# barlettacarmen/CrCNN

Measured on NVIDIA B200. Metric: encrypted MNIST images/sec, higher is better.
Workload: dtype u64

## Files before the change

crcnn_b200/csrc/engine.cu:

```cuda
#include <cuda_runtime.h>
#include <dlfcn.h>
#include <algorithm>
#include <cstdlib>
#include <cstring>
#include <map>
#include <unordered_map>
#include <string>
#include <vector>

#include "../../include/crcnn_b200.h"
#include "kernels.cuh"
#include "params.h"
#include "tc_mac.cuh"
#include "tcn_mac.cuh"
#include "relin32.cuh"
#include "reenc.cuh"

using namespace crcnn;

namespace {

enum KernelClass {
    KC_NTT_FWD = 0, KC_NTT_INV, KC_MAC, KC_PLAIN_EXPAND, KC_POOL, KC_BN, KC_PLAIN_OP,
    KC_BEHZ_LIFT, KC_SQ_TENSOR, KC_BEHZ_FLOOR, KC_RELIN, KC_PROBE, KC_TC_SPLIT, KC_TC_MAC, KC_TCN_SPLIT, KC_TCN_MAC, KC_RELIN32, KC_REENC, KC_COUNT
};
const char *kClassNames[KC_COUNT] = {"ntt_forward", "ntt_inverse", "weighted_sum_mac", "plain_expand_ntt", "pool_sum",
                                     "batch_norm", "plain_op", "behz_lift", "square_tensor", "behz_floor_sk",
                                     "relinearize", "imad_probe", "tc_plane_split", "weighted_sum_tc_i8", "tcn_plane_split",
                                     "weighted_sum_tcn_i8", "relinearize_u32", "reencrypt"};

thread_local std::string g_create_error;

}

struct crcnn_tensor {
    long count;
    int size;
    int ntt;
    uint64_t *d;
};

static long next_plain_serial() { static long s = 0; return ++s; }

struct crcnn_plain {
    long serial = next_plain_serial();
    long count;
    bool sparse_shape = false;
    std::vector<uint32_t> off, idx;
    std::vector<uint64_t> val;
    uint32_t *d_off = nullptr, *d_idx = nullptr;
    uint64_t *d_val = nullptr;
    uint64_t *ntt_mul = nullptr;
    uint64_t *ntt_mul_sh = nullptr;
    uint64_t *ntt_add = nullptr;
    uint64_t *coef_add = nullptr;
    int tap_state = 0;
    int tc_state = 0;
    int8_t *tc_A = nullptr;
    int tc_R = 0, tc_Kpad = 0;
    uint8_t *tcn_W = nullptr;
    int tcn_R = 0;
    uint64_t *fused_C = nullptr, *fused_Csh = nullptr, *fused_D = nullptr;
    long fused_scale = 0, fused_mean = 0;
    int add_mult = 1;
    bool dense_only = false;
    crcnn_plain *folded_w = nullptr, *folded_b = nullptr;
    long folded_key[9] = {0, 0, 0, 0, 0, 0, 0, 0, 0};
};

struct crcnn_evk {
    uint64_t *d = nullptr;
    long key_off[MAXK];
    int digits[MAXK];
    int dbc;
    bool has_r32 = false;
    Relin32 r32;
};

struct crcnn_keys {
    uint64_t *sk = nullptr;
    uint64_t *pk = nullptr;
    ReencConsts c;
};

struct crcnn_ctx {
    int device = 0;
    cudaStream_t stream = nullptr;
    HostParams hp;
    DeviceParams *dP = nullptr;
    std::vector<void *> owned;
    int n = 0, logn = 0, K = 0, S = 0;
    int chunk_terms = 1 << 30;
    size_t weight_cache_bytes = 24ull << 30;
    int sm_count = 148;
    int tc_mode = 1;
    int tc_min_fanin = 256;
    int tc_min_outputs = 32;
    int tap_mode = 1;
    int relin_mode = 1;
    int tcn_mode = 1;
    int sq_lean = 1;
    int tcn_fold = 1;
    size_t tc_scratch_bytes = 12ull << 30;
    std::string err;
    std::map<std::vector<int>, int *> index_cache;
    std::unordered_map<void *, size_t> big_size;
    std::multimap<size_t, void *> big_free;
    size_t big_cached = 0, big_cache_cap = 64ull << 30;
    long long st_big_malloc = 0, st_big_hit = 0, st_big_bypass = 0, st_flush = 0, st_small_malloc = 0;
    uint64_t *stage = nullptr;
    size_t stage_bytes = 0;
    bool prof_on = false;
    long launches[KC_COUNT] = {0};
    double ms[KC_COUNT] = {0};
    double work_bytes[KC_COUNT] = {0};
    double work_ops[KC_COUNT] = {0};
    struct Pending { int cls; cudaEvent_t a, b; };
    std::vector<Pending> pending;
    std::vector<cudaEvent_t> event_pool;
};

namespace {

int fail(crcnn_ctx *ctx, int code, const std::string &msg) {
    if (ctx) ctx->err = msg; else g_create_error = msg;
    return code;
}

#define CU(call)                                                                                       \
    do {                                                                                               \
        cudaError_t e__ = (call);                                                                      \
        if (e__ != cudaSuccess) {                                                                      \
            int code__ = (e__ == cudaErrorMemoryAllocation) ? CRCNN_ERR_OUT_OF_MEMORY : CRCNN_ERR_CUDA; \
            return fail(ctx, code__, std::string(#call) + ": " + cudaGetErrorString(e__));            \
        }                                                                                              \
    } while (0)

#define REQUIRE(cond, msg) \
    do { if (!(cond)) return fail(ctx, CRCNN_ERR_INVALID_ARGUMENT, msg); } while (0)

struct ProfScope {
    crcnn_ctx *c; int cls; cudaEvent_t a = nullptr, b = nullptr;
    ProfScope(crcnn_ctx *ctx, int k, double bytes = 0, double ops = 0) : c(ctx), cls(k) {
        c->launches[cls]++;
        c->work_bytes[cls] += bytes;
        c->work_ops[cls] += ops;
        if (!c->prof_on) return;
        auto get = [&]() { cudaEvent_t e; if (!c->event_pool.empty()) { e = c->event_pool.back(); c->event_pool.pop_back(); } else cudaEventCreate(&e); return e; };
        a = get(); b = get();
        cudaEventRecord(a, c->stream);
    }
    ~ProfScope() {
        if (!a) return;
        cudaEventRecord(b, c->stream);
        c->pending.push_back({cls, a, b});
    }
};

void prof_collect(crcnn_ctx *c) {
    for (auto &p : c->pending) {
        cudaEventSynchronize(p.b);
        float t = 0;
        cudaEventElapsedTime(&t, p.a, p.b);
        c->ms[p.cls] += t;
        c->event_pool.push_back(p.a);
        c->event_pool.push_back(p.b);
    }
    c->pending.clear();
}

inline size_t poly_words(const crcnn_ctx *c) { return (size_t)c->K * c->n; }
inline double lp_bytes(const crcnn_ctx *c, double polys) { return polys * c->n * 8.0; }
inline double lp_bfly(const crcnn_ctx *c, double polys) { return polys * (c->n / 2) * c->logn; }

constexpr size_t kBigBlock = 32ull << 20;
void big_cache_flush(crcnn_ctx *ctx) {
    for (auto &kv : ctx->big_free) { ctx->big_size.erase(kv.second); cudaFreeAsync(kv.second, ctx->stream); }
    ctx->big_free.clear();
    ctx->big_cached = 0;
}
int dev_alloc(crcnn_ctx *ctx, size_t bytes, void **out) {
    *out = nullptr;
    if (bytes == 0) return CRCNN_OK;
    if (bytes >= kBigBlock) {
        auto it = ctx->big_free.find(bytes);
        if (it != ctx->big_free.end()) {
            *out = it->second;
            ctx->big_cached -= bytes;
            ctx->big_free.erase(it);
            ctx->st_big_hit++;
            return CRCNN_OK;
        }
        ctx->st_big_malloc++;
    } else {
        ctx->st_small_malloc++;
    }
    cudaError_t e = cudaMallocAsync(out, bytes, ctx->stream);
    if (e == cudaErrorMemoryAllocation && !ctx->big_free.empty()) {
        cudaGetLastError();
        ctx->st_flush++;
        big_cache_flush(ctx);
        e = cudaMallocAsync(out, bytes, ctx->stream);
    }
    CU(e);
    if (bytes >= kBigBlock) ctx->big_size[*out] = bytes;
    return CRCNN_OK;
}
void dev_free(crcnn_ctx *ctx, void *p) {
    if (!p) return;
    auto it = ctx->big_size.find(p);
    if (it != ctx->big_size.end()) {
        if (ctx->big_cached + it->second <= ctx->big_cache_cap) {
            ctx->big_free.insert({it->second, p});
            ctx->big_cached += it->second;
            return;
        }
        ctx->big_size.erase(it);
        ctx->st_big_bypass++;
    }
    cudaFreeAsync(p, ctx->stream);
}

int new_tensor(crcnn_ctx *ctx, long count, int size, int ntt, crcnn_tensor **out) {
    auto *t = new crcnn_tensor{count, size, ntt, nullptr};
    int rc = dev_alloc(ctx, (size_t)count * size * poly_words(ctx) * 8, (void **)&t->d);
    if (rc) { delete t; return rc; }
    *out = t;
    return CRCNN_OK;
}

int ntt_inplace(crcnn_ctx *ctx, uint64_t *d, long npolys, int slot_base, int slot_count, bool inverse) {
    ProfScope ps(ctx, inverse ? KC_NTT_INV : KC_NTT_FWD, 2 * lp_bytes(ctx, npolys), lp_bfly(ctx, npolys));
    CU(launch_ntt(ctx->dP, ctx->logn, d, npolys, slot_base, slot_count, inverse, ctx->stream));
    return CRCNN_OK;
}

int ensure_domain(crcnn_ctx *ctx, crcnn_tensor *t, int want_ntt) {
    if (t->ntt == want_ntt) return CRCNN_OK;
    int rc = ntt_inplace(ctx, t->d, t->count * t->size * ctx->K, 0, ctx->K, !want_ntt);
    if (rc) return rc;
    t->ntt = want_ntt;
    return CRCNN_OK;
}

enum PlainForm { PF_NTT_MUL, PF_NTT_ADD, PF_COEF_ADD };

int expand_range(crcnn_ctx *ctx, crcnn_plain *p, long first, long count, PlainForm f, uint64_t *dst) {
    ProfScope ps(ctx, KC_PLAIN_EXPAND, lp_bytes(ctx, (double)count * ctx->K), f != PF_COEF_ADD ? lp_bfly(ctx, (double)count * ctx->K) : 0);
    CU(launch_plain_expand(ctx->dP, ctx->logn, ctx->K, p->d_off, p->d_idx, p->d_val, first, count,
                           (f == PF_NTT_MUL ? 0 : 1) | (p->sparse_shape ? 2 : 0), f != PF_COEF_ADD, dst, ctx->stream));
    return CRCNN_OK;
}

int ensure_form(crcnn_ctx *ctx, crcnn_plain *p, PlainForm f) {
    uint64_t **slot = f == PF_NTT_MUL ? &p->ntt_mul : (f == PF_NTT_ADD ? &p->ntt_add : &p->coef_add);
    if (*slot) return CRCNN_OK;
    if (p->dense_only) return fail(ctx, CRCNN_ERR_UNSUPPORTED, "this derived plaintext pack has no such form");
    int rc = dev_alloc(ctx, (size_t)p->count * poly_words(ctx) * 8, (void **)slot);
    if (rc) return rc;
    rc = expand_range(ctx, p, 0, p->count, f, *slot);
    if (!rc && f != PF_NTT_MUL && p->add_mult != 1)
        CU(launch_scale_small(ctx->dP, *slot, (long)((size_t)p->count * poly_words(ctx)), p->add_mult, ctx->stream));
    return rc;
}

int make_plain(crcnn_ctx *ctx, std::vector<uint32_t> &&off, std::vector<uint32_t> &&idx, std::vector<uint64_t> &&val,
               crcnn_plain **out) {
    auto *p = new crcnn_plain();
    p->count = (long)off.size() - 1;
    p->off = std::move(off); p->idx = std::move(idx); p->val = std::move(val);
    p->sparse_shape = true;
    for (uint32_t ix : p->idx)
        if (ix >= 64 && ix < (uint32_t)(ctx->n - 32)) { p->sparse_shape = false; break; }
    int rc = dev_alloc(ctx, p->off.size() * 4, (void **)&p->d_off);
    if (!rc) rc = dev_alloc(ctx, std::max<size_t>(p->idx.size(), 1) * 4, (void **)&p->d_idx);
    if (!rc) rc = dev_alloc(ctx, std::max<size_t>(p->val.size(), 1) * 8, (void **)&p->d_val);
    if (rc) { delete p; return rc; }
    CU(cudaMemcpyAsync(p->d_off, p->off.data(), p->off.size() * 4, cudaMemcpyHostToDevice, ctx->stream));
    if (!p->idx.empty()) {
        CU(cudaMemcpyAsync(p->d_idx, p->idx.data(), p->idx.size() * 4, cudaMemcpyHostToDevice, ctx->stream));
        CU(cudaMemcpyAsync(p->d_val, p->val.data(), p->val.size() * 8, cudaMemcpyHostToDevice, ctx->stream));
    }
    CU(cudaStreamSynchronize(ctx->stream));
    *out = p;
    return CRCNN_OK;
}

int ensure_shoup(crcnn_ctx *ctx, crcnn_plain *p) {
    int rc = ensure_form(ctx, p, PF_NTT_MUL);
    if (rc || p->ntt_mul_sh) return rc;
    const size_t words = (size_t)p->count * poly_words(ctx);
    rc = dev_alloc(ctx, words * 8, (void **)&p->ntt_mul_sh);
    if (rc) return rc;
    CU(launch_shoup_companion(ctx->dP, p->ntt_mul, (long)words, p->ntt_mul_sh, ctx->stream));
    return CRCNN_OK;
}

int ensure_pool_bn_consts(crcnn_ctx *ctx, crcnn_plain *scale, crcnn_plain *mean, crcnn_plain *invstd) {
    int rc = scale ? ensure_form(ctx, scale, PF_NTT_MUL) : CRCNN_OK;
    if (!rc) rc = ensure_form(ctx, mean, PF_NTT_ADD);
    if (!rc) rc = ensure_form(ctx, invstd, PF_NTT_MUL);
    if (rc) return rc;
    const long scale_id = scale ? scale->serial : -1;
    if (invstd->fused_C && invstd->fused_scale == scale_id && invstd->fused_mean == mean->serial) return CRCNN_OK;
    const size_t words = (size_t)invstd->count * poly_words(ctx);
    dev_free(ctx, invstd->fused_C); dev_free(ctx, invstd->fused_Csh); dev_free(ctx, invstd->fused_D);
    invstd->fused_C = invstd->fused_Csh = invstd->fused_D = nullptr;
    rc = dev_alloc(ctx, words * 8, (void **)&invstd->fused_C);
    if (!rc) rc = dev_alloc(ctx, words * 8, (void **)&invstd->fused_Csh);
    if (!rc) rc = dev_alloc(ctx, words * 8, (void **)&invstd->fused_D);
    if (rc) return rc;
    CU(launch_pool_bn_consts(ctx->dP, scale ? scale->ntt_mul : nullptr, invstd->ntt_mul, mean->ntt_add, (long)words, invstd->fused_C, invstd->fused_D, ctx->stream));
    CU(launch_shoup_companion(ctx->dP, invstd->fused_C, (long)words, invstd->fused_Csh, ctx->stream));
    invstd->fused_scale = scale_id; invstd->fused_mean = mean->serial;
    return CRCNN_OK;
}

int get_index_table(crcnn_ctx *ctx, const std::vector<int> &key, const std::vector<int> &table, const int **out) {
    auto it = ctx->index_cache.find(key);
    if (it != ctx->index_cache.end()) { *out = it->second; return CRCNN_OK; }
    int *d = nullptr;
    CU(cudaMalloc((void **)&d, std::max<size_t>(table.size(), 1) * sizeof(int)));
    CU(cudaMemcpyAsync(d, table.data(), table.size() * sizeof(int), cudaMemcpyHostToDevice, ctx->stream));
    CU(cudaStreamSynchronize(ctx->stream));
    ctx->index_cache[key] = d;
    *out = d;
    return CRCNN_OK;
}

bool tap_eligible(crcnn_ctx *ctx, crcnn_plain *p) {
    if (p->tap_state == 0) {
        p->tap_state = (p->sparse_shape && tcn_planes_for(ctx->hp.d) == 7 && ctx->n % 1024 == 0) ? 1 : -1;
        const uint64_t t = ctx->hp.d.t;
        for (size_t e = 0; e < p->val.size() && p->tap_state == 1; e++)
            if (p->val[e] != 1 && p->val[e] != t - 1) p->tap_state = -1;
        for (long i = 0; i < p->count && p->tap_state == 1; i++)
            if (p->off[i + 1] - p->off[i] > 96) p->tap_state = -1;
    }
    return p->tap_state == 1;
}

bool sum_fits_64(const crcnn_ctx *ctx, long R) {
    uint64_t maxq = 0;
    for (int j = 0; j < ctx->K; j++) maxq = std::max(maxq, ctx->hp.d.tab[j].mod.q);
    return R > 0 && (uint64_t)R <= UINT64_MAX / maxq;
}

void boundaries(int xd, int yd, int xs, int ys, int xf, int yf, int *xl, int *yl) {
    *xl = (xf > xs) ? xd - xf + 1 : xd - xs + 1;
    *yl = (yf > ys) ? yd - yf + 1 : yd - ys + 1;
}

int ensure_tc_form(crcnn_ctx *ctx, crcnn_plain *w, int R) {
    if (w->tc_state < 0) return CRCNN_OK;
    if (w->tc_state == 1 && w->tc_R == R) return CRCNN_OK;
    const uint32_t n = (uint32_t)ctx->n;
    const uint64_t t = ctx->hp.d.t;
    for (size_t e = 0; e < w->idx.size(); e++)
        if (w->idx[e] < n - TC_TAPS || (w->val[e] != 1 && w->val[e] != t - 1)) { w->tc_state = -1; return CRCNN_OK; }
    if (w->count % R) { w->tc_state = -1; return CRCNN_OK; }
    const long Mall = w->count / R;
    const int Kpad = ((R + 31) / 32 + 3) / 4 * TC_BK;
    const size_t rows = (size_t)Mall * TC_TAPS + TC_BM;
    std::vector<int8_t> A(rows * Kpad, 0);
    for (long wi = 0; wi < w->count; wi++) {
        const long m = wi / R, r = wi % R;
        for (uint32_t e = w->off[wi]; e < w->off[wi + 1]; e++) {
            const int tap = (int)(n - w->idx[e]);
            A[((size_t)m * TC_TAPS + tap - 1) * Kpad + r] = w->val[e] == 1 ? (int8_t)-1 : (int8_t)1;
        }
    }
    if (w->tc_A) { dev_free(ctx, w->tc_A); w->tc_A = nullptr; }
    int rc = dev_alloc(ctx, A.size(), (void **)&w->tc_A);
    if (rc) return rc;
    CU(cudaMemcpyAsync(w->tc_A, A.data(), A.size(), cudaMemcpyHostToDevice, ctx->stream));
    CU(cudaStreamSynchronize(ctx->stream));
    w->tc_state = 1; w->tc_R = R; w->tc_Kpad = Kpad;
    return CRCNN_OK;
}

int run_weighted_sum_tc(crcnn_ctx *ctx, crcnn_tensor *in, crcnn_plain *w, crcnn_plain *b, const int *d_index, int R,
                        int Npos, int Pimg, int m_first, int M, crcnn_tensor *out) {
    int rc = ensure_domain(ctx, in, 0);
    if (!rc) rc = ensure_form(ctx, b, PF_COEF_ADD);
    if (rc) return rc;
    const size_t pw = poly_words(ctx);
    TcMacArgs a{};
    a.A = w->tc_A + (size_t)m_first * TC_TAPS * w->tc_Kpad;
    a.x = in->d; a.bias = b->coef_add + (size_t)m_first * pw; a.out = out->d;
    a.M = M; a.Mpad = (M * TC_TAPS + TC_BM - 1) / TC_BM * TC_BM; a.R = R; a.Kpad = w->tc_Kpad;
    a.planes = tc_planes_for(ctx->hp.d);
    a.Pimg = Pimg; a.Mtotal = M; a.m0 = 0; a.n = ctx->n; a.K = ctx->K;
    a.npos = 1;
    const size_t per_pos = tc_b_bytes(a);
    long chunk = (long)std::max<size_t>(1, ctx->tc_scratch_bytes / per_pos);
    chunk = std::min<long>(std::min<long>(chunk, Npos), 65535 / (2 * ctx->K));
    uint8_t *scratch = nullptr;
    rc = dev_alloc(ctx, (size_t)chunk * per_pos, (void **)&scratch);
    if (rc) return rc;
    a.B = scratch;
    for (long p0 = 0; p0 < Npos && !rc; p0 += chunk) {
        a.npos = (int)std::min<long>(chunk, Npos - p0);
        a.p0 = (int)p0;
        a.in_index = d_index + p0 * R;
        cudaError_t e;
        const double bbytes = (double)a.npos * per_pos;
        { ProfScope ps(ctx, KC_TC_SPLIT, lp_bytes(ctx, (double)a.npos * R * 2 * ctx->K) + bbytes, 0); e = launch_tc_split(ctx->dP, a, ctx->stream); }
        if (e == cudaSuccess) {
            ProfScope ps(ctx, KC_TC_MAC, bbytes + lp_bytes(ctx, (double)a.npos * M * 2 * ctx->K),
                         (double)a.npos * 2 * ctx->K * ctx->n * a.planes * (double)M * TC_TAPS * R);
            e = launch_tc_mac(ctx->dP, a, ctx->sm_count, ctx->stream);
        }
        if (e != cudaSuccess) rc = fail(ctx, CRCNN_ERR_CUDA, std::string("tensor-core weighted sum: ") + cudaGetErrorString(e));
    }
    dev_free(ctx, scratch);
    if (!rc) out->ntt = 0;
    return rc;
}

int ensure_tcn_weights(crcnn_ctx *ctx, crcnn_plain *w, int R) {
    if (w->tcn_W && w->tcn_R == R) return CRCNN_OK;
    int rc = ensure_form(ctx, w, PF_NTT_MUL);
    if (rc) return rc;
    if (w->tcn_W) { dev_free(ctx, w->tcn_W); w->tcn_W = nullptr; }
    const int Mall = (int)(w->count / R), Kpad = tcn_kpad(R);
    rc = dev_alloc(ctx, tcn_w_bytes(7, Mall, Kpad, ctx->K, ctx->n), (void **)&w->tcn_W);
    if (rc) return rc;
    TcnSplitArgs s{};
    s.src = w->ntt_mul; s.index = nullptr; s.dst = w->tcn_W; s.item_polys = 1;
    s.R = R; s.Kpad = Kpad; s.planes = 7; s.ncols = Mall; s.slot0 = 0; s.nslots = ctx->K * ctx->n; s.n = ctx->n; s.K = ctx->K;
    {
        ProfScope ps(ctx, KC_TCN_SPLIT, lp_bytes(ctx, (double)w->count * ctx->K) + (double)tcn_w_bytes(7, Mall, Kpad, ctx->K, ctx->n), 0);
        CU(launch_tcn_split(s, ctx->stream));
    }
    dev_free(ctx, w->ntt_mul); w->ntt_mul = nullptr;
    if (w->ntt_mul_sh) { dev_free(ctx, w->ntt_mul_sh); w->ntt_mul_sh = nullptr; }
    w->tcn_R = R;
    return CRCNN_OK;
}

int run_weighted_sum_tcn(crcnn_ctx *ctx, crcnn_tensor *in, crcnn_plain *w, crcnn_plain *b, const int *d_index, int R,
                         int Npos, int Pimg, int m_first, int M, crcnn_tensor *out) {
    int rc = ensure_domain(ctx, in, 1);
    if (!rc) rc = ensure_form(ctx, b, PF_NTT_ADD);
    if (!rc) rc = ensure_tcn_weights(ctx, w, R);
    if (rc) return rc;
    const size_t pw = poly_words(ctx);
    const int Kpad = tcn_kpad(R), ncols = 2 * Npos, total = ctx->K * ctx->n;
    const size_t per_slot = tcn_x_bytes_per_slot(7, ncols, Kpad);
    long chunk = (long)(ctx->tc_scratch_bytes / per_slot) / 32 * 32;
    chunk = std::max<long>(32, std::min<long>(chunk, total));
    uint8_t *scratch = nullptr;
    rc = dev_alloc(ctx, (size_t)chunk * per_slot, (void **)&scratch);
    if (rc) return rc;
    TcnSplitArgs s{};
    s.src = in->d; s.index = d_index; s.dst = scratch; s.item_polys = 2;
    s.R = R; s.Kpad = Kpad; s.planes = 7; s.ncols = ncols; s.n = ctx->n; s.K = ctx->K;
    TcnMacArgs a{};
    a.W = w->tcn_W; a.X = scratch; a.bias = b->ntt_add + (size_t)m_first * pw; a.out = out->d;
    a.Mall = (int)(w->count / R); a.m_first = m_first; a.M = M;
    a.R = R; a.Kpad = Kpad; a.planes = 7; a.ncols = ncols;
    a.Pimg = Pimg; a.Mtotal = M; a.m0 = 0; a.n = ctx->n; a.K = ctx->K;
    a.variant = ctx->tcn_mode >= 2 ? ctx->tcn_mode - 1 : 0;
    a.use_fold = ctx->tcn_fold;
    for (int j = 0; j < ctx->K; j++) a.fold[j] = tcn_fold_make(ctx->hp.d.tab[j].mod.q);
    for (long s0 = 0; s0 < total && !rc; s0 += chunk) {
        const int ns = (int)std::min<long>(chunk, total - s0);
        s.slot0 = a.slot0 = (int)s0; s.nslots = a.nslots = ns;
        const double xbytes = (double)ns * per_slot;
        cudaError_t e;
        { ProfScope ps(ctx, KC_TCN_SPLIT, (double)ncols * R * ns * 8.0 + xbytes, 0); e = launch_tcn_split(s, ctx->stream); }
        if (e == cudaSuccess) {
            ProfScope ps(ctx, KC_TCN_MAC, xbytes + (double)ns * 7 * M * Kpad + (double)ncols * M * ns * 8.0, (double)ns * ncols * M * R * 49.0);
            e = launch_tcn_mac(ctx->dP, a, ctx->sm_count, ctx->stream);
        }
        if (e != cudaSuccess) rc = fail(ctx, CRCNN_ERR_CUDA, std::string("limb-split tensor-core weighted sum: ") + cudaGetErrorString(e));
    }
    dev_free(ctx, scratch);
    if (!rc) out->ntt = 1;
    return rc;
}

int run_weighted_sum(crcnn_ctx *ctx, crcnn_tensor *in, crcnn_plain *w, crcnn_plain *b, const int *d_index, int R,
                     int Npos, int Pimg, int Mall, int m_first, int M, crcnn_tensor *out) {
    if (ctx->tc_mode && R >= ctx->tc_min_fanin && (ctx->tc_mode == 2 || Mall >= ctx->tc_min_outputs) && w->sparse_shape && tc_mac_available() == cudaSuccess) {
        int rc = ensure_tc_form(ctx, w, R);
        if (rc) return rc;
        if (w->tc_state == 1) return run_weighted_sum_tc(ctx, in, w, b, d_index, R, Npos, Pimg, m_first, M, out);
    }
    if (ctx->tcn_mode && tcn_planes_for(ctx->hp.d) == 7 && R <= TCN_MAX_R && w->count % R == 0 && tc_mac_available() == cudaSuccess &&
        (w->tcn_W || tcn_w_bytes(7, (int)(w->count / R), tcn_kpad(R), ctx->K, ctx->n) <= ctx->weight_cache_bytes))
        return run_weighted_sum_tcn(ctx, in, w, b, d_index, R, Npos, Pimg, m_first, M, out);
    int rc = ensure_domain(ctx, in, 1);
    if (rc) return rc;
    rc = ensure_form(ctx, b, PF_NTT_ADD);
    if (rc) return rc;
    MacArgs a{};
    a.x = in->d; a.in_index = d_index; a.out = out->d;
    a.R = R; a.Npos = Npos; a.Pimg = Pimg; a.Mtotal = M; a.K = ctx->K; a.n = ctx->n;
    a.chunk_terms = ctx->chunk_terms;
    const size_t pw = poly_words(ctx);
    const size_t all_bytes = (size_t)w->count * pw * 8;
    if (w->ntt_mul || all_bytes <= ctx->weight_cache_bytes) {
        rc = ensure_form(ctx, w, PF_NTT_MUL);
        if (rc) return rc;
        a.w = w->ntt_mul + (size_t)m_first * R * pw;
        a.bias = b->ntt_add + (size_t)m_first * pw;
        a.M = M; a.m0 = 0;
        ProfScope ps(ctx, KC_MAC, lp_bytes(ctx, ((double)in->count + (double)M * Npos) * 2 * ctx->K + (double)M * R * ctx->K),
                     (double)M * Npos * R * 2 * ctx->K * ctx->n);
        CU(launch_mac(ctx->dP, a, ctx->stream));
        return CRCNN_OK;
    }
    long rows = (long)std::max<size_t>(1, ctx->weight_cache_bytes / ((size_t)R * pw * 8));
    rows = std::min<long>(rows, M);
    uint64_t *scratch = nullptr;
    rc = dev_alloc(ctx, (size_t)rows * R * pw * 8, (void **)&scratch);
    if (rc) return rc;
    for (long m0 = 0; m0 < M; m0 += rows) {
        long cur = std::min<long>(rows, M - m0);
        rc = expand_range(ctx, w, (long)(m_first + m0) * R, cur * R, PF_NTT_MUL, scratch);
        if (rc) break;
        a.w = scratch; a.bias = b->ntt_add + (size_t)(m_first + m0) * pw;
        a.M = (int)cur; a.m0 = (int)m0;
        ProfScope ps(ctx, KC_MAC, lp_bytes(ctx, ((double)in->count + (double)cur * Npos) * 2 * ctx->K + (double)cur * R * ctx->K),
                     (double)cur * Npos * R * 2 * ctx->K * ctx->n);
        cudaError_t e = launch_mac(ctx->dP, a, ctx->stream);
        if (e != cudaSuccess) { rc = fail(ctx, CRCNN_ERR_CUDA, cudaGetErrorString(e)); break; }
    }
    dev_free(ctx, scratch);
    return rc;
}

int upload_rows(crcnn_ctx *ctx, const uint64_t *host, size_t rows, uint64_t *dst, cudaStream_t s) {
    const size_t n = ctx->n;
    if (rows * n * 8 < (8u << 20)) {
        CU(cudaMemcpy2DAsync(dst, n * 8, host, (n + 1) * 8, n * 8, rows, cudaMemcpyHostToDevice, s));
        return CRCNN_OK;
    }
    uint64_t *stage = nullptr;
    CU(cudaMallocAsync((void **)&stage, rows * (n + 1) * 8, s));
    cudaError_t e = cudaMemcpyAsync(stage, host, rows * (n + 1) * 8, cudaMemcpyHostToDevice, s);
    if (e == cudaSuccess) e = launch_strip_pad(stage, dst, (long)rows, (int)n, s);
    cudaFreeAsync(stage, s);
    if (e != cudaSuccess) return fail(ctx, CRCNN_ERR_CUDA, std::string("upload: ") + cudaGetErrorString(e));
    return CRCNN_OK;
}

}

extern "C" {

const char *crcnn_last_error(const crcnn_ctx *ctx) { return ctx ? ctx->err.c_str() : g_create_error.c_str(); }

int crcnn_ctx_create(int n, int K, const uint64_t *q, uint64_t t, int device, crcnn_ctx **out) {
    crcnn_ctx *ctx = nullptr;
    if (!out || !q) return fail(nullptr, CRCNN_ERR_INVALID_ARGUMENT, "null argument");
    *out = nullptr;
    int ndev = 0;
    if (cudaGetDeviceCount(&ndev) != cudaSuccess || ndev == 0)
        return fail(nullptr, CRCNN_ERR_NO_DEVICE, "no CUDA device: crcnn_b200 has no CPU fallback");
    if (device < 0 || device >= ndev) return fail(nullptr, CRCNN_ERR_INVALID_ARGUMENT, "bad device ordinal");
    HostParams hp;
    try {
        hp = derive_params(n, K, q, t);
    } catch (const std::exception &e) {
        return fail(nullptr, CRCNN_ERR_INVALID_ARGUMENT, e.what());
    }
    CU(cudaSetDevice(device));
    auto *c = new crcnn_ctx();
    c->device = device; c->n = n; c->K = K; c->S = hp.d.S; c->logn = hp.d.logn;
    int maxbits = 0;
    for (int i = 0; i < K; i++) { int b = 0; for (uint64_t v = q[i]; v; v >>= 1) b++; maxbits = std::max(maxbits, b); }
    int spare = 128 - 2 * maxbits;
    c->chunk_terms = spare >= 30 ? (1 << 30) : (1 << spare);
    cudaDeviceGetAttribute(&c->sm_count, cudaDevAttrMultiProcessorCount, device);
    if (const char *e = getenv("CRCNN_TC")) c->tc_mode = atoi(e);
    if (const char *e = getenv("CRCNN_TCN")) c->tcn_mode = atoi(e);
    if (const char *e = getenv("CRCNN_TAP")) c->tap_mode = atoi(e);
    if (const char *e = getenv("CRCNN_TCN_FOLD")) c->tcn_fold = atoi(e);
    if (const char *e = getenv("CRCNN_SQ_LEAN")) c->sq_lean = atoi(e);
    cudaMemPool_t pool;
    if (cudaDeviceGetDefaultMemPool(&pool, device) == cudaSuccess) {
        uint64_t thr = UINT64_MAX;
        cudaMemPoolSetAttribute(pool, cudaMemPoolAttrReleaseThreshold, &thr);
    }
    {
        size_t fr = 0, tot = 0;
        if (cudaMemGetInfo(&fr, &tot) == cudaSuccess && tot) c->big_cache_cap = tot / 4 * 3;
    }
    int slots = K + hp.d.S;
    auto up = [&](const std::vector<uint64_t> &v, const uint64_t **dst) -> cudaError_t {
        void *d = nullptr;
        cudaError_t e = cudaMalloc(&d, v.size() * 8);
        if (e != cudaSuccess) return e;
        c->owned.push_back(d);
        *dst = (const uint64_t *)d;
        return cudaMemcpy(d, v.data(), v.size() * 8, cudaMemcpyHostToDevice);
    };
    cudaError_t e = cudaSuccess;
    for (int s = 0; s < slots && e == cudaSuccess; s++) {
        std::vector<uint64_t> fw(2 * (size_t)n), bw(2 * (size_t)n);
        for (int i = 0; i < n; i++) {
            fw[2 * i] = hp.w[s][i]; fw[2 * i + 1] = hp.wp[s][i];
            bw[2 * i] = hp.iwf[s][i]; bw[2 * i + 1] = hp.iwfp[s][i];
        }
        e = up(fw, &hp.d.tab[s].w);
        if (e == cudaSuccess) e = up(bw, &hp.d.tab[s].iw);
        const int NG = n >> 4;
        std::vector<uint64_t> fl(2 * (size_t)16 * NG, 0), bl(2 * (size_t)16 * NG, 0);
        for (int G = 0; G < NG; G++)
            for (int st = 0; st < 4; st++) {
                for (int lb = 0; lb < (1 << st); lb++) {
                    const size_t at = 2 * ((size_t)((1 << st) - 1 + lb) * NG + G), from = 2 * ((((size_t)NG + G) << st) + lb);
                    fl[at] = fw[from]; fl[at + 1] = fw[from + 1];
                }
                for (int lb = 0; lb < (1 << (3 - st)); lb++) {
                    const size_t at = 2 * ((size_t)(16 - (16 >> st) + lb) * NG + G);
                    const size_t from = 2 * ((size_t)((n >> 1) >> st) + ((size_t)G << (3 - st)) + lb);
                    bl[at] = bw[from]; bl[at + 1] = bw[from + 1];
                }
            }
        if (e == cudaSuccess) e = up(fl, &hp.d.tab[s].wl);
        if (e == cudaSuccess) e = up(bl, &hp.d.tab[s].iwl);
        hp.d.tab[s].tf = nullptr;
        if (e == cudaSuccess && s < K) e = up(hp.tf[s], &hp.d.tab[s].tf);
    }
    if (e == cudaSuccess) e = cudaMalloc((void **)&c->dP, sizeof(DeviceParams));
    if (e == cudaSuccess) e = cudaMemcpy(c->dP, &hp.d, sizeof(DeviceParams), cudaMemcpyHostToDevice);
    if (e != cudaSuccess) {
        std::string m = cudaGetErrorString(e);
        for (void *p : c->owned) cudaFree(p);
        if (c->dP) cudaFree(c->dP);
        delete c;
        return fail(nullptr, CRCNN_ERR_CUDA, "context setup: " + m);
    }
    c->hp = std::move(hp);
    *out = c;
    return CRCNN_OK;
}

int crcnn_ctx_destroy(crcnn_ctx *ctx) {
    if (!ctx) return CRCNN_OK;
    cudaSetDevice(ctx->device);
    big_cache_flush(ctx);
    cudaStreamSynchronize(ctx->stream);
    prof_collect(ctx);
    for (auto e : ctx->event_pool) cudaEventDestroy(e);
    for (auto &kv : ctx->index_cache) cudaFree(kv.second);
    if (ctx->stage) cudaFree(ctx->stage);
    for (void *p : ctx->owned) cudaFree(p);
    cudaFree(ctx->dP);
    delete ctx;
    return CRCNN_OK;
}

int crcnn_ctx_set_stream(crcnn_ctx *ctx, void *cuda_stream) {
    if (!ctx) return CRCNN_ERR_INVALID_ARGUMENT;
    CU(cudaStreamSynchronize(ctx->stream));
    ctx->stream = (cudaStream_t)cuda_stream;
    return CRCNN_OK;
}

int crcnn_ctx_sync(crcnn_ctx *ctx) {
    if (!ctx) return CRCNN_ERR_INVALID_ARGUMENT;
    CU(cudaStreamSynchronize(ctx->stream));
    prof_collect(ctx);
    return CRCNN_OK;
}

int crcnn_ctx_alloc_stats(crcnn_ctx *ctx, long long out[6]) {
    if (!ctx || !out) return CRCNN_ERR_INVALID_ARGUMENT;
    out[0] = ctx->st_big_malloc; out[1] = ctx->st_big_hit; out[2] = ctx->st_big_bypass; out[3] = ctx->st_flush;
    out[4] = ctx->st_small_malloc; out[5] = (long long)ctx->big_cached;
    return CRCNN_OK;
}

int crcnn_ctx_set_weight_cache_bytes(crcnn_ctx *ctx, size_t bytes) {
    if (!ctx) return CRCNN_ERR_INVALID_ARGUMENT;
    ctx->weight_cache_bytes = bytes;
    return CRCNN_OK;
}

int crcnn_ctx_set_tensor_core_mode(crcnn_ctx *ctx, int mode, int min_fanin, size_t scratch_bytes) {
    if (!ctx) return CRCNN_ERR_INVALID_ARGUMENT;
    REQUIRE(mode >= 0 && mode <= 2, "tensor-core mode must be 0, 1 or 2");
    ctx->tc_mode = mode;
    if (min_fanin > 0) ctx->tc_min_fanin = min_fanin;
    if (scratch_bytes > 0) ctx->tc_scratch_bytes = scratch_bytes;
    return CRCNN_OK;
}

int crcnn_ctx_set_limb_split_mode(crcnn_ctx *ctx, int mode) {
    if (!ctx) return CRCNN_ERR_INVALID_ARGUMENT;
    REQUIRE(mode >= 0 && mode <= 3, "limb-split mode must be 0 (off), 1 (on), 2 (row-major kernel) or 3 (column-major kernel)");
    ctx->tcn_mode = mode;
    return CRCNN_OK;
}

int crcnn_ctx_set_limb_split_reduction(crcnn_ctx *ctx, int mode) {
    if (!ctx) return CRCNN_ERR_INVALID_ARGUMENT;
    REQUIRE(mode == 0 || mode == 1, "limb-split reduction must be 0 (128-bit recombination + Barrett) or 1 (folded through 2^k - delta)");
    ctx->tcn_fold = mode;
    return CRCNN_OK;
}

int crcnn_ctx_set_relin_mode(crcnn_ctx *ctx, int mode) {
    if (!ctx) return CRCNN_ERR_INVALID_ARGUMENT;
    REQUIRE(mode == 0 || mode == 1, "relinearize mode must be 0 (64-bit transforms) or 1 (word-size auxiliary primes)");
    ctx->relin_mode = mode;
    return CRCNN_OK;
}

int crcnn_ctx_ntt_table(const crcnn_ctx *ctx_c, int slot, int which, uint64_t *out) {
    crcnn_ctx *ctx = const_cast<crcnn_ctx *>(ctx_c);
    if (!ctx) return CRCNN_ERR_INVALID_ARGUMENT;
    REQUIRE(out && slot >= 0 && slot < ctx->K + ctx->S && which >= 0 && which < 4, "bad table selector");
    const auto &v = which == 0 ? ctx->hp.w[slot] : which == 1 ? ctx->hp.wp[slot] : which == 2 ? ctx->hp.iw[slot] : ctx->hp.iwp[slot];
    memcpy(out, v.data(), v.size() * 8);
    return CRCNN_OK;
}

int crcnn_ctx_bsk_count(const crcnn_ctx *ctx) { return ctx ? ctx->S : CRCNN_ERR_INVALID_ARGUMENT; }

int crcnn_tensor_upload_ex(crcnn_ctx *ctx, const uint64_t *host, long count, int size, int ntt_form, crcnn_tensor **out) {
    if (!ctx) return CRCNN_ERR_INVALID_ARGUMENT;
    REQUIRE(host && out && count >= 0 && size >= 2 && size <= 3, "bad tensor upload arguments");
    CU(cudaSetDevice(ctx->device));
    crcnn_tensor *t = nullptr;
    int rc = new_tensor(ctx, count, size, ntt_form ? 1 : 0, &t);
    if (rc) return rc;
    const size_t n = ctx->n, rows = (size_t)count * size * ctx->K;
    if (rows) {
        int rc2 = upload_rows(ctx, host, rows, t->d, ctx->stream);
        if (rc2) { crcnn_tensor_free(ctx, t); return rc2; }
    }
    (void)n;
    *out = t;
    return CRCNN_OK;
}
int crcnn_tensor_upload_on(crcnn_ctx *ctx, const uint64_t *host, long count, int size, int ntt_form, void *copy_stream,
                           crcnn_tensor **out) {
    if (!ctx) return CRCNN_ERR_INVALID_ARGUMENT;
    REQUIRE(host && out && count >= 0 && size >= 2 && size <= 3, "bad tensor upload arguments");
    CU(cudaSetDevice(ctx->device));
    cudaStream_t cs = (cudaStream_t)copy_stream;
    auto *t = new crcnn_tensor{count, size, ntt_form ? 1 : 0, nullptr};
    const size_t n = ctx->n, rows = (size_t)count * size * ctx->K;
    if (rows) {
        cudaError_t e = cudaMallocAsync((void **)&t->d, rows * n * 8, cs);
        if (e != cudaSuccess) { delete t; return fail(ctx, e == cudaErrorMemoryAllocation ? CRCNN_ERR_OUT_OF_MEMORY : CRCNN_ERR_CUDA, cudaGetErrorString(e)); }
        int rc2 = upload_rows(ctx, host, rows, t->d, cs);
        if (rc2) { cudaFreeAsync(t->d, cs); delete t; return rc2; }
    }
    *out = t;
    return CRCNN_OK;
}

int crcnn_tensor_upload_into(crcnn_ctx *ctx, const uint64_t *host, crcnn_tensor *t, int ntt_form, void *copy_stream) {
    if (!ctx) return CRCNN_ERR_INVALID_ARGUMENT;
    REQUIRE(host && t, "null argument");
    CU(cudaSetDevice(ctx->device));
    cudaStream_t cs = copy_stream ? (cudaStream_t)copy_stream : ctx->stream;
    const size_t n = ctx->n, rows = (size_t)t->count * t->size * ctx->K;
    const size_t need = rows * (n + 1) * 8;
    if (need > ctx->stage_bytes) {
        if (ctx->stage) { CU(cudaStreamSynchronize(cs)); CU(cudaFree(ctx->stage)); ctx->stage = nullptr; ctx->stage_bytes = 0; }
        CU(cudaMalloc((void **)&ctx->stage, need));
        ctx->stage_bytes = need;
    }
    if (rows) {
        CU(cudaMemcpyAsync(ctx->stage, host, need, cudaMemcpyHostToDevice, cs));
        CU(launch_strip_pad(ctx->stage, t->d, (long)rows, (int)n, cs));
    }
    t->ntt = ntt_form ? 1 : 0;
    return CRCNN_OK;
}

int crcnn_ctx_wait_stream(crcnn_ctx *ctx, void *other_stream) {
    if (!ctx) return CRCNN_ERR_INVALID_ARGUMENT;
    cudaEvent_t ev;
    CU(cudaEventCreateWithFlags(&ev, cudaEventDisableTiming));
    CU(cudaEventRecord(ev, (cudaStream_t)other_stream));
    CU(cudaStreamWaitEvent(ctx->stream, ev, 0));
    CU(cudaEventDestroy(ev));
    return CRCNN_OK;
}

int crcnn_tensor_upload(crcnn_ctx *ctx, const uint64_t *host, long count, int size, crcnn_tensor **out) {
    return crcnn_tensor_upload_ex(ctx, host, count, size, 0, out);
}

int crcnn_tensor_download_ex(crcnn_ctx *ctx, crcnn_tensor *t, int want_ntt, uint64_t *host) {
    if (!ctx) return CRCNN_ERR_INVALID_ARGUMENT;
    REQUIRE(t && host, "null argument");
    CU(cudaSetDevice(ctx->device));
    const size_t n = ctx->n, rows = (size_t)t->count * t->size * ctx->K;
    const uint64_t *src = t->d;
    uint64_t *tmp = nullptr;
    if ((t->ntt != 0) != (want_ntt != 0)) {
        int rc = dev_alloc(ctx, rows * n * 8, (void **)&tmp);
        if (rc) return rc;
        CU(cudaMemcpyAsync(tmp, t->d, rows * n * 8, cudaMemcpyDeviceToDevice, ctx->stream));
        rc = ntt_inplace(ctx, tmp, (long)rows, 0, ctx->K, want_ntt == 0);
        if (rc) return rc;
        src = tmp;
    }
    if (rows) CU(cudaMemcpy2DAsync(host, (n + 1) * 8, src, n * 8, n * 8, rows, cudaMemcpyDeviceToHost, ctx->stream));
    CU(cudaStreamSynchronize(ctx->stream));
    dev_free(ctx, tmp);
    for (size_t r = 0; r < rows; r++) host[r * (n + 1) + n] = 0;
    prof_collect(ctx);
    return CRCNN_OK;
}
int crcnn_tensor_download(crcnn_ctx *ctx, crcnn_tensor *t, uint64_t *host) { return crcnn_tensor_download_ex(ctx, t, 0, host); }

int crcnn_tensor_free(crcnn_ctx *ctx, crcnn_tensor *t) {
    if (!ctx) return CRCNN_ERR_INVALID_ARGUMENT;
    if (!t) return CRCNN_OK;
    dev_free(ctx, t->d);
    delete t;
    return CRCNN_OK;
}
long crcnn_tensor_count(const crcnn_tensor *t) { return t ? t->count : -1; }
int crcnn_tensor_ct_size(const crcnn_tensor *t) { return t ? t->size : -1; }

int crcnn_tensor_slice(crcnn_ctx *ctx, crcnn_tensor *t, long first, long count, crcnn_tensor **out) {
    if (!ctx) return CRCNN_ERR_INVALID_ARGUMENT;
    REQUIRE(t && out && first >= 0 && count >= 0 && first + count <= t->count, "slice out of range");
    crcnn_tensor *s = nullptr;
    int rc = new_tensor(ctx, count, t->size, t->ntt, &s);
    if (rc) return rc;
    size_t ctw = (size_t)t->size * poly_words(ctx);
    if (count) CU(cudaMemcpyAsync(s->d, t->d + first * ctw, count * ctw * 8, cudaMemcpyDeviceToDevice, ctx->stream));
    *out = s;
    return CRCNN_OK;
}

int crcnn_tensor_device_ptr(crcnn_tensor *t, void **dev_ptr, int *ntt_form) {
    if (!t || !dev_ptr) return CRCNN_ERR_INVALID_ARGUMENT;
    *dev_ptr = t->d;
    if (ntt_form) *ntt_form = t->ntt;
    return CRCNN_OK;
}

int crcnn_tensor_wrap_alloc(crcnn_ctx *ctx, long count, int size, int ntt_form, crcnn_tensor **out) {
    if (!ctx) return CRCNN_ERR_INVALID_ARGUMENT;
    REQUIRE(out && count >= 0 && size >= 2 && size <= 3, "bad tensor shape");
    return new_tensor(ctx, count, size, ntt_form ? 1 : 0, out);
}

int crcnn_plain_upload(crcnn_ctx *ctx, const uint64_t *host, long count, int coeff_count, long stride, crcnn_plain **out) {
    if (!ctx) return CRCNN_ERR_INVALID_ARGUMENT;
    REQUIRE(host && out && count >= 0 && coeff_count >= 0 && stride >= coeff_count, "bad plaintext upload arguments");
    REQUIRE(coeff_count <= ctx->n + 1, "plain is not valid for encryption parameters");
    std::vector<uint32_t> off(count + 1, 0), idx;
    std::vector<uint64_t> val;
    for (long i = 0; i < count; i++) {
        const uint64_t *p = host + i * stride;
        for (int c = 0; c < coeff_count; c++)
            if (p[c]) {
                REQUIRE(c < ctx->n, "plain is not valid for encryption parameters");
                REQUIRE(p[c] < ctx->hp.d.t, "plaintext coefficient not below the plain modulus");
                idx.push_back((uint32_t)c); val.push_back(p[c]);
            }
        off[i + 1] = (uint32_t)idx.size();
    }
    return make_plain(ctx, std::move(off), std::move(idx), std::move(val), out);
}

int crcnn_plain_upload_sparse(crcnn_ctx *ctx, const uint32_t *idx, const uint64_t *val, const uint32_t *offsets, long count,
                              crcnn_plain **out) {
    if (!ctx) return CRCNN_ERR_INVALID_ARGUMENT;
    REQUIRE(offsets && out && count >= 0, "bad sparse plaintext arguments");
    std::vector<uint32_t> off(offsets, offsets + count + 1);
    size_t nnz = off[count];
    REQUIRE(nnz == 0 || (idx && val), "null sparse arrays");
    std::vector<uint32_t> vi(idx, idx + nnz);
    std::vector<uint64_t> vv(val, val + nnz);
    for (size_t e = 0; e < nnz; e++) {
        REQUIRE(vi[e] < (uint32_t)ctx->n, "plain is not valid for encryption parameters");
        REQUIRE(vv[e] < ctx->hp.d.t, "plaintext coefficient not below the plain modulus");
    }
    return make_plain(ctx, std::move(off), std::move(vi), std::move(vv), out);
}

int crcnn_plain_encode(crcnn_ctx *ctx, const float *values, long count, crcnn_plain **out) {
    if (!ctx) return CRCNN_ERR_INVALID_ARGUMENT;
    REQUIRE(values && out && count >= 0, "bad encode arguments");
    std::vector<uint32_t> off(count + 1, 0), idx;
    std::vector<uint64_t> val;
    idx.reserve(count * 24); val.reserve(count * 24);
    for (long i = 0; i < count; i++) {
        encode_fractional_sparse((double)values[i], ctx->n, ctx->hp.d.t, idx, val);
        off[i + 1] = (uint32_t)idx.size();
    }
    return make_plain(ctx, std::move(off), std::move(idx), std::move(val), out);
}

int crcnn_plain_encode_f64(crcnn_ctx *ctx, const double *values, long count, crcnn_plain **out) {
    if (!ctx) return CRCNN_ERR_INVALID_ARGUMENT;
    REQUIRE(values && out && count >= 0, "bad encode arguments");
    std::vector<uint32_t> off(count + 1, 0), idx;
    std::vector<uint64_t> val;
    for (long i = 0; i < count; i++) {
        encode_fractional_sparse(values[i], ctx->n, ctx->hp.d.t, idx, val);
        off[i + 1] = (uint32_t)idx.size();
    }
    return make_plain(ctx, std::move(off), std::move(idx), std::move(val), out);
}

int crcnn_plain_get(crcnn_ctx *ctx, const crcnn_plain *p, long index, uint64_t *out_words) {
    if (!ctx) return CRCNN_ERR_INVALID_ARGUMENT;
    REQUIRE(p && out_words && index >= 0 && index < p->count, "plaintext index out of range");
    REQUIRE(!p->dense_only, "derived plaintext pack: no host form");
    memset(out_words, 0, (size_t)(ctx->n + 1) * 8);
    for (uint32_t e = p->off[index]; e < p->off[index + 1]; e++) out_words[p->idx[e]] = p->val[e];
    return CRCNN_OK;
}

int crcnn_plain_get_ntt(crcnn_ctx *ctx, crcnn_plain *p, long index, uint64_t *out_words) {
    if (!ctx) return CRCNN_ERR_INVALID_ARGUMENT;
    REQUIRE(p && out_words && index >= 0 && index < p->count, "plaintext index out of range");
    REQUIRE(!p->dense_only, "derived plaintext pack: no host form");
    uint64_t *tmp = nullptr;
    int rc = dev_alloc(ctx, poly_words(ctx) * 8, (void **)&tmp);
    if (rc) return rc;
    rc = expand_range(ctx, p, index, 1, PF_NTT_MUL, tmp);
    if (rc) return rc;
    const size_t n = ctx->n;
    CU(cudaMemcpy2DAsync(out_words, (n + 1) * 8, tmp, n * 8, n * 8, ctx->K, cudaMemcpyDeviceToHost, ctx->stream));
    CU(cudaStreamSynchronize(ctx->stream));
    dev_free(ctx, tmp);
    for (int j = 0; j < ctx->K; j++) out_words[j * (n + 1) + n] = 0;
    return CRCNN_OK;
}

int crcnn_plain_free(crcnn_ctx *ctx, crcnn_plain *p) {
    if (!ctx) return CRCNN_ERR_INVALID_ARGUMENT;
    if (!p) return CRCNN_OK;
    dev_free(ctx, p->d_off); dev_free(ctx, p->d_idx); dev_free(ctx, p->d_val);
    dev_free(ctx, p->ntt_mul); dev_free(ctx, p->ntt_mul_sh); dev_free(ctx, p->ntt_add); dev_free(ctx, p->coef_add); dev_free(ctx, p->tc_A); dev_free(ctx, p->tcn_W);
    dev_free(ctx, p->fused_C); dev_free(ctx, p->fused_Csh); dev_free(ctx, p->fused_D);
    if (p->folded_w) crcnn_plain_free(ctx, p->folded_w);
    if (p->folded_b) crcnn_plain_free(ctx, p->folded_b);
    delete p;
    return CRCNN_OK;
}
long crcnn_plain_count(const crcnn_plain *p) { return p ? p->count : -1; }

int crcnn_evk_upload(crcnn_ctx *ctx, const uint64_t *host, int dbc, const int *sizes, crcnn_evk **out) {
    if (!ctx) return CRCNN_ERR_INVALID_ARGUMENT;
    REQUIRE(host && sizes && out && dbc >= 1 && dbc <= 60, "bad evaluation key arguments");
    CU(cudaSetDevice(ctx->device));
    auto *k = new crcnn_evk();
    k->dbc = dbc;
    long polys = 0;
    const size_t pw = poly_words(ctx);
    for (int i = 0; i < MAXK; i++) { k->key_off[i] = 0; k->digits[i] = 0; }
    for (int i = 0; i < ctx->K; i++) {
        if (sizes[i] < 2 || (sizes[i] & 1)) { delete k; return fail(ctx, CRCNN_ERR_INVALID_ARGUMENT, "evaluation key sizes must be even and >= 2"); }
        k->key_off[i] = polys * (long)pw;
        k->digits[i] = sizes[i] / 2;
        polys += sizes[i];
    }
    int rc = dev_alloc(ctx, (size_t)polys * pw * 8, (void **)&k->d);
    if (rc) { delete k; return rc; }
    const size_t n = ctx->n, rows = (size_t)polys * ctx->K;
    CU(cudaMemcpy2DAsync(k->d, n * 8, host, (n + 1) * 8, n * 8, rows, cudaMemcpyHostToDevice, ctx->stream));
    CU(launch_canonicalize(ctx->dP, k->d, (long)(rows * n), ctx->stream));
    {
        uint64_t q[MAXK];
        for (int i = 0; i < ctx->K; i++) q[i] = ctx->hp.d.tab[i].mod.q;
        if (relin32_applicable(ctx->n, ctx->K, q, k->digits, dbc, k->r32.c)) {
            cudaError_t e = relin32_build(ctx->dP, ctx->logn, ctx->K, q, k->d, k->key_off, polys, k->r32, ctx->stream);
            if (e != cudaSuccess) { relin32_free(k->r32); dev_free(ctx, k->d); delete k; return fail(ctx, CRCNN_ERR_CUDA, cudaGetErrorString(e)); }
            k->has_r32 = true;
        }
    }
    *out = k;
    return CRCNN_OK;
}
int crcnn_evk_free(crcnn_ctx *ctx, crcnn_evk *k) {
    if (!ctx) return CRCNN_ERR_INVALID_ARGUMENT;
    if (!k) return CRCNN_OK;
    CU(cudaSetDevice(ctx->device));
    CU(cudaStreamSynchronize(ctx->stream));
    relin32_free(k->r32);
    dev_free(ctx, k->d);
    delete k;
    return CRCNN_OK;
}

int crcnn_conv_forward_shard(crcnn_ctx *ctx, crcnn_tensor *in, crcnn_plain *w, crcnn_plain *b, int batch, int xd, int yd,
                             int zd, int xs, int ys, int xf, int yf, int nf, int k0, int kc, crcnn_tensor **out) {
    if (!ctx) return CRCNN_ERR_INVALID_ARGUMENT;
    REQUIRE(in && w && b && out, "null argument");
    REQUIRE(batch > 0 && xd > 0 && yd > 0 && zd > 0 && xs > 0 && ys > 0 && xf > 0 && yf > 0 && nf > 0 && xf <= xd && yf <= yd,
            "bad convolution geometry");
    REQUIRE(k0 >= 0 && kc >= 0 && k0 + kc <= nf, "bad output-channel shard");
    REQUIRE(in->size == 2 && in->count == (long)batch * zd * xd * yd, "input tensor does not match the layer geometry");
    const int R = zd * xf * yf;
    REQUIRE(w->count == (long)nf * R && b->count == nf, "kernel/bias count does not match the layer geometry");
    CU(cudaSetDevice(ctx->device));
    const int xo = (xd - xf) / xs + 1, yo = (yd - yf) / ys + 1;
    int xl, yl;
    boundaries(xd, yd, xs, ys, xf, yf, &xl, &yl);
    if ((xl + xs - 1) / xs != xo || (yl + ys - 1) / ys != yo)
        return fail(ctx, CRCNN_ERR_UNSUPPORTED, "stride larger than the filter leaves outputs the reference never computes");
    const int P = xo * yo, Npos = batch * P, nin = zd * xd * yd;
    std::vector<int> key = {1, batch, xd, yd, zd, xs, ys, xf, yf};
    const int *d_index = nullptr;
    if (ctx->index_cache.find(key) == ctx->index_cache.end()) {
        std::vector<int> table((size_t)Npos * R);
        for (int bi = 0; bi < batch; bi++)
            for (int i = 0; i < xo; i++)
                for (int j = 0; j < yo; j++) {
                    int *row = &table[((size_t)bi * P + i * yo + j) * R];
                    int r = 0;
                    for (int z = 0; z < zd; z++)
                        for (int kx = 0; kx < xf; kx++)
                            for (int ky = 0; ky < yf; ky++) row[r++] = bi * nin + (z * xd + i * xs + kx) * yd + j * ys + ky;
                }
        int rc = get_index_table(ctx, key, table, &d_index);
        if (rc) return rc;
    } else {
        d_index = ctx->index_cache[key];
    }
    crcnn_tensor *o = nullptr;
    int rc = new_tensor(ctx, (long)batch * kc * P, 2, 1, &o);
    if (rc) return rc;
    rc = run_weighted_sum(ctx, in, w, b, d_index, R, Npos, P, nf, k0, kc, o);
    if (rc) { crcnn_tensor_free(ctx, o); return rc; }
    *out = o;
    return CRCNN_OK;
}

int crcnn_conv_forward(crcnn_ctx *ctx, crcnn_tensor *in, crcnn_plain *w, crcnn_plain *b, int batch, int xd, int yd, int zd,
                       int xs, int ys, int xf, int yf, int nf, crcnn_tensor **out) {
    return crcnn_conv_forward_shard(ctx, in, w, b, batch, xd, yd, zd, xs, ys, xf, yf, nf, 0, nf, out);
}

int crcnn_fc_forward_shard(crcnn_ctx *ctx, crcnn_tensor *in, crcnn_plain *w, crcnn_plain *b, int batch, int in_dim,
                           int out_dim, int o0, int oc, crcnn_tensor **out) {
    if (!ctx) return CRCNN_ERR_INVALID_ARGUMENT;
    REQUIRE(in && w && b && out, "null argument");
    REQUIRE(batch > 0 && in_dim > 0 && out_dim > 0, "bad fully-connected geometry");
    REQUIRE(o0 >= 0 && oc >= 0 && o0 + oc <= out_dim, "bad output-row shard");
    REQUIRE(in->size == 2 && in->count == (long)batch * in_dim, "input tensor does not match the layer geometry");
    REQUIRE(w->count == (long)out_dim * in_dim && b->count == out_dim, "weight/bias count does not match the layer geometry");
    CU(cudaSetDevice(ctx->device));
    std::vector<int> key = {2, batch, in_dim};
    const int *d_index = nullptr;
    if (ctx->index_cache.find(key) == ctx->index_cache.end()) {
        std::vector<int> table((size_t)batch * in_dim);
        for (size_t i = 0; i < table.size(); i++) table[i] = (int)i;
        int rc = get_index_table(ctx, key, table, &d_index);
        if (rc) return rc;
    } else {
        d_index = ctx->index_cache[key];
    }
    crcnn_tensor *o = nullptr;
    int rc = new_tensor(ctx, (long)batch * oc, 2, 1, &o);
    if (rc) return rc;
    rc = run_weighted_sum(ctx, in, w, b, d_index, in_dim, batch, 1, out_dim, o0, oc, o);
    if (rc) { crcnn_tensor_free(ctx, o); return rc; }
    *out = o;
    return CRCNN_OK;
}

int crcnn_fc_forward(crcnn_ctx *ctx, crcnn_tensor *in, crcnn_plain *w, crcnn_plain *b, int batch, int in_dim, int out_dim,
                     crcnn_tensor **out) {
    return crcnn_fc_forward_shard(ctx, in, w, b, batch, in_dim, out_dim, 0, out_dim, out);
}

static int compose_fc(crcnn_ctx *ctx, crcnn_plain *w1, crcnn_plain *b1, crcnn_plain *w2, crcnn_plain *b2, int in_dim, int mid_dim, int out_dim,
                      const uint64_t *C = nullptr, const uint64_t *D = nullptr, int per_channel = 1) {
    const size_t pw = poly_words(ctx);
    const int saved_tc = ctx->tc_mode;
    const bool saved_prof = ctx->prof_on;
    ctx->tc_mode = 0;
    ctx->prof_on = false;
    crcnn_plain *zero = nullptr, *W = nullptr, *B = nullptr;
    crcnn_tensor *T = nullptr, *O = nullptr;
    uint64_t *dense = nullptr;
    int rc = CRCNN_OK;
    auto done = [&](int code) {
        if (T) crcnn_tensor_free(ctx, T);
        if (O) crcnn_tensor_free(ctx, O);
        if (zero) crcnn_plain_free(ctx, zero);
        dev_free(ctx, dense);
        if (code) { if (W) crcnn_plain_free(ctx, W); if (B) crcnn_plain_free(ctx, B); }
        ctx->tc_mode = saved_tc; ctx->prof_on = saved_prof;
        return code;
    };
    rc = make_plain(ctx, std::vector<uint32_t>((size_t)out_dim + 1, 0), {}, {}, &zero);
    if (rc) return done(rc);
    rc = dev_alloc(ctx, (size_t)out_dim * in_dim * pw * 8, (void **)&dense);
    if (rc) return done(rc);
    const int pairs_all = (in_dim + 1) / 2;
    int Bc = (int)std::max<size_t>(1, std::min<size_t>((size_t)pairs_all, (8ull << 30) / ((size_t)mid_dim * 2 * pw * 8)));
    if (const char *e = getenv("CRCNN_FC_COMPOSE_PAIRS")) Bc = std::max(1, std::min(Bc, atoi(e)));
    std::vector<int> table((size_t)Bc * mid_dim);
    for (int bi = 0; bi < Bc; bi++)
        for (int o = 0; o < mid_dim; o++) table[(size_t)bi * mid_dim + o] = o * Bc + bi;
    const int *d_index = nullptr;
    rc = get_index_table(ctx, {5, Bc, mid_dim}, table, &d_index);
    if (rc) return done(rc);
    rc = new_tensor(ctx, (long)mid_dim * Bc, 2, 1, &T);
    if (!rc) rc = new_tensor(ctx, (long)Bc * out_dim, 2, 1, &O);
    if (rc) return done(rc);
    CU(cudaMemsetAsync(T->d, 0, (size_t)T->count * 2 * pw * 8, ctx->stream));
    for (int r0 = 0; r0 < in_dim && !rc; r0 += 2 * Bc) {
        const int cols = std::min(2 * Bc, in_dim - r0);
        for (int o = 0; o < mid_dim && !rc; o++)
            rc = expand_range(ctx, w1, (long)o * in_dim + r0, cols, PF_NTT_MUL, T->d + (size_t)o * Bc * 2 * pw);
        if (rc) break;
        rc = run_weighted_sum(ctx, T, w2, zero, d_index, mid_dim, Bc, 1, out_dim, 0, out_dim, O);
        if (rc) break;
        for (int bi = 0; 2 * bi < cols; bi++) {
            const int polys = std::min(2, cols - 2 * bi);
            cudaError_t e = cudaMemcpy2DAsync(dense + ((size_t)r0 + 2 * bi) * pw, (size_t)in_dim * pw * 8, O->d + (size_t)bi * out_dim * 2 * pw,
                                              2 * pw * 8, (size_t)polys * pw * 8, out_dim, cudaMemcpyDeviceToDevice, ctx->stream);
            if (e != cudaSuccess) { rc = fail(ctx, CRCNN_ERR_CUDA, cudaGetErrorString(e)); break; }
        }
    }
    if (rc) return done(rc);
    W = new crcnn_plain();
    W->count = (long)out_dim * in_dim; W->dense_only = true; W->sparse_shape = false; W->tc_state = -1; W->tap_state = -1;
    W->ntt_mul = dense; dense = nullptr;
    rc = ensure_form(ctx, b1, PF_NTT_ADD);
    if (rc) return done(rc);
    crcnn_tensor_free(ctx, T); T = nullptr;
    crcnn_tensor_free(ctx, O); O = nullptr;
    rc = new_tensor(ctx, mid_dim, 2, 1, &T);
    if (!rc) rc = new_tensor(ctx, out_dim, 2, 1, &O);
    if (rc) return done(rc);
    CU(cudaMemsetAsync(T->d, 0, (size_t)mid_dim * 2 * pw * 8, ctx->stream));
    CU(cudaMemcpy2DAsync(T->d, 2 * pw * 8, b1->ntt_add, pw * 8, pw * 8, mid_dim, cudaMemcpyDeviceToDevice, ctx->stream));
    std::vector<int> ident(mid_dim);
    for (int o = 0; o < mid_dim; o++) ident[o] = o;
    rc = get_index_table(ctx, {2, 1, mid_dim}, ident, &d_index);
    if (!rc) rc = run_weighted_sum(ctx, T, w2, b2, d_index, mid_dim, 1, 1, out_dim, 0, out_dim, O);
    if (rc) return done(rc);
    B = new crcnn_plain();
    B->count = out_dim; B->dense_only = true; B->sparse_shape = false; B->tc_state = -1; B->tap_state = -1;
    rc = dev_alloc(ctx, (size_t)out_dim * pw * 8, (void **)&B->ntt_add);
    if (rc) return done(rc);
    CU(cudaMemcpy2DAsync(B->ntt_add, pw * 8, O->d, 2 * pw * 8, pw * 8, out_dim, cudaMemcpyDeviceToDevice, ctx->stream));
    if (C) CU(launch_fold_fc_input_affine(ctx->dP, W->ntt_mul, out_dim, in_dim, (long)pw, per_channel, C, D, B->ntt_add, ctx->stream));
    rc = ensure_tcn_weights(ctx, W, in_dim);
    if (rc) return done(rc);
    w1->folded_w = W; w1->folded_b = B;
    return done(CRCNN_OK);
}

int crcnn_fc_fc_forward(crcnn_ctx *ctx, crcnn_tensor *in, crcnn_plain *w1, crcnn_plain *b1, crcnn_plain *w2, crcnn_plain *b2, int batch,
                        int in_dim, int mid_dim, int out_dim, crcnn_tensor **out) {
    if (!ctx) return CRCNN_ERR_INVALID_ARGUMENT;
    REQUIRE(in && w1 && b1 && w2 && b2 && out, "null argument");
    REQUIRE(batch > 0 && in_dim > 0 && mid_dim > 0 && out_dim > 0, "bad fully-connected geometry");
    REQUIRE(in->size == 2 && in->count == (long)batch * in_dim, "input tensor does not match the layer geometry");
    REQUIRE(w1->count == (long)mid_dim * in_dim && b1->count == mid_dim && w2->count == (long)out_dim * mid_dim && b2->count == out_dim,
            "weight/bias count does not match the layer geometry");
    CU(cudaSetDevice(ctx->device));
    const bool composed = (double)out_dim * in_dim < (double)mid_dim * (in_dim + out_dim) && !w1->dense_only && !w2->dense_only &&
                          ctx->tcn_mode && tcn_planes_for(ctx->hp.d) == 7 && in_dim <= TCN_MAX_R && mid_dim <= TCN_MAX_R &&
                          tc_mac_available() == cudaSuccess && tcn_w_bytes(7, out_dim, tcn_kpad(in_dim), ctx->K, ctx->n) <= ctx->weight_cache_bytes &&
                          !getenv("CRCNN_NO_FC_COMPOSE");
    if (!composed) {
        crcnn_tensor *mid = nullptr;
        int rc = crcnn_fc_forward(ctx, in, w1, b1, batch, in_dim, mid_dim, &mid);
        if (rc) return rc;
        rc = crcnn_fc_forward(ctx, mid, w2, b2, batch, mid_dim, out_dim, out);
        crcnn_tensor_free(ctx, mid);
        return rc;
    }
    const long key[9] = {b1->serial, w2->serial, b2->serial, (long)mid_dim, (long)out_dim, 0, 0, 0, 0};
    if (!w1->folded_w || memcmp(key, w1->folded_key, sizeof(key)) != 0) {
        if (w1->folded_w) { crcnn_plain_free(ctx, w1->folded_w); w1->folded_w = nullptr; }
        if (w1->folded_b) { crcnn_plain_free(ctx, w1->folded_b); w1->folded_b = nullptr; }
        int rc = compose_fc(ctx, w1, b1, w2, b2, in_dim, mid_dim, out_dim);
        if (rc) return rc;
        memcpy(w1->folded_key, key, sizeof(key));
    }
    return crcnn_fc_forward(ctx, in, w1->folded_w, w1->folded_b, batch, in_dim, out_dim, out);
}

int crcnn_pool_bn_fc_fc_forward(crcnn_ctx *ctx, crcnn_tensor *in, int batch, int xd, int yd, int zd, int pxs, int pys, int pxf, int pyf,
                                crcnn_plain *scale, crcnn_plain *mean, crcnn_plain *invstd, crcnn_plain *w1, crcnn_plain *b1,
                                crcnn_plain *w2, crcnn_plain *b2, int mid_dim, int out_dim, crcnn_tensor **out) {
    if (!ctx) return CRCNN_ERR_INVALID_ARGUMENT;
    REQUIRE(in && mean && invstd && w1 && b1 && w2 && b2 && out, "null argument");
    REQUIRE(batch > 0 && xd > 0 && yd > 0 && zd > 0 && pxs > 0 && pys > 0 && pxf > 0 && pyf > 0 && pxf <= xd && pyf <= yd, "bad pooling geometry");
    REQUIRE(mid_dim > 0 && out_dim > 0, "bad fully-connected geometry");
    const int pxo = (xd - pxf) / pxs + 1, pyo = (yd - pyf) / pys + 1, Rp = pxf * pyf;
    const int in_dim = zd * pxo * pyo;
    REQUIRE(in->size == 2 && in->count == (long)batch * zd * xd * yd, "input tensor does not match the layer geometry");
    REQUIRE((!scale || scale->count >= 1) && mean->count == zd && invstd->count == zd, "mean/var count does not match the channel count");
    REQUIRE(w1->count == (long)mid_dim * in_dim && b1->count == mid_dim && w2->count == (long)out_dim * mid_dim && b2->count == out_dim,
            "weight/bias count does not match the layer geometry");
    CU(cudaSetDevice(ctx->device));
    const bool composed = pxs <= pxf && pys <= pyf && sum_fits_64(ctx, Rp) &&
                          (double)out_dim * in_dim < (double)mid_dim * (in_dim + out_dim) && !w1->dense_only && !w2->dense_only &&
                          ctx->tcn_mode && tcn_planes_for(ctx->hp.d) == 7 && in_dim <= TCN_MAX_R && mid_dim <= TCN_MAX_R &&
                          tc_mac_available() == cudaSuccess && tcn_w_bytes(7, out_dim, tcn_kpad(in_dim), ctx->K, ctx->n) <= ctx->weight_cache_bytes &&
                          !getenv("CRCNN_NO_FC_COMPOSE");
    if (!composed) {
        crcnn_tensor *mid = nullptr;
        int rc = crcnn_pool_bn_forward(ctx, in, batch, xd, yd, zd, pxs, pys, pxf, pyf, scale, mean, invstd, &mid);
        if (rc) return rc;
        rc = crcnn_fc_fc_forward(ctx, mid, w1, b1, w2, b2, batch, in_dim, mid_dim, out_dim, out);
        crcnn_tensor_free(ctx, mid);
        return rc;
    }
    int rc = ensure_pool_bn_consts(ctx, scale, mean, invstd);
    if (rc) return rc;
    const long key[9] = {b1->serial, w2->serial, b2->serial, (long)mid_dim, (long)out_dim, scale ? scale->serial : -1, mean->serial, invstd->serial, (long)(pxo * pyo)};
    if (!w1->folded_w || memcmp(key, w1->folded_key, sizeof(key)) != 0) {
        if (w1->folded_w) { crcnn_plain_free(ctx, w1->folded_w); w1->folded_w = nullptr; }
        if (w1->folded_b) { crcnn_plain_free(ctx, w1->folded_b); w1->folded_b = nullptr; }
        rc = compose_fc(ctx, w1, b1, w2, b2, in_dim, mid_dim, out_dim, invstd->fused_C, invstd->fused_D, pxo * pyo);
        if (rc) return rc;
        memcpy(w1->folded_key, key, sizeof(key));
    }
    crcnn_tensor *sums = nullptr;
    rc = crcnn_pool_forward(ctx, in, batch, xd, yd, zd, pxs, pys, pxf, pyf, nullptr, &sums);
    if (rc) return rc;
    rc = crcnn_fc_forward(ctx, sums, w1->folded_w, w1->folded_b, batch, in_dim, out_dim, out);
    crcnn_tensor_free(ctx, sums);
    return rc;
}

int crcnn_pool_forward(crcnn_ctx *ctx, crcnn_tensor *in, int batch, int xd, int yd, int zd, int xs, int ys, int xf, int yf,
                       crcnn_plain *scale, crcnn_tensor **out) {
    if (!ctx) return CRCNN_ERR_INVALID_ARGUMENT;
    REQUIRE(in && out, "null argument");
    REQUIRE(batch > 0 && xd > 0 && yd > 0 && zd > 0 && xs > 0 && ys > 0 && xf > 0 && yf > 0 && xf <= xd && yf <= yd, "bad pooling geometry");
    REQUIRE(in->size == 2 && in->count == (long)batch * zd * xd * yd, "input tensor does not match the layer geometry");
    REQUIRE(!scale || scale->count >= 1, "empty scale pack");
    CU(cudaSetDevice(ctx->device));
    const int xo = (xd - xf) / xs + 1, yo = (yd - yf) / ys + 1;
    int xl, yl;
    boundaries(xd, yd, xs, ys, xf, yf, &xl, &yl);
    if ((xl + xs - 1) / xs != xo || (yl + ys - 1) / ys != yo)
        return fail(ctx, CRCNN_ERR_UNSUPPORTED, "stride larger than the window leaves outputs the reference never computes");
    const int R = xf * yf, Nout = batch * zd * xo * yo;
    std::vector<int> key = {3, batch, xd, yd, zd, xs, ys, xf, yf};
    const int *d_index = nullptr;
    if (ctx->index_cache.find(key) == ctx->index_cache.end()) {
        std::vector<int> table((size_t)Nout * R);
        size_t o = 0;
        for (int bz = 0; bz < batch * zd; bz++)
            for (int i = 0; i < xo; i++)
                for (int j = 0; j < yo; j++)
                    for (int kx = 0; kx < xf; kx++)
                        for (int ky = 0; ky < yf; ky++) table[o++] = (bz * xd + i * xs + kx) * yd + j * ys + ky;
        int rc = get_index_table(ctx, key, table, &d_index);
        if (rc) return rc;
    } else {
        d_index = ctx->index_cache[key];
    }
    int rc = CRCNN_OK;
    if (scale && !in->ntt && ctx->tap_mode && tap_eligible(ctx, scale) && sum_fits_64(ctx, R)) {
        crcnn_tensor *o = nullptr;
        rc = new_tensor(ctx, Nout, 2, 0, &o);
        if (rc) return rc;
        TapMulArgs a{};
        a.in = in->d; a.in_index = d_index; a.R = R; a.sub = nullptr;
        a.t_off = scale->d_off; a.t_idx = scale->d_idx; a.t_val = scale->d_val; a.per_channel = 1; a.channels = 1;
        a.out = o->d; a.nout = Nout;
        ProfScope ps(ctx, KC_POOL, lp_bytes(ctx, ((double)in->count + Nout) * 2 * ctx->K), (double)Nout * R * 2 * ctx->K * ctx->n);
        cudaError_t e = launch_tapmul(ctx->dP, ctx->n, ctx->K, a, ctx->stream);
        if (e != cudaSuccess) { crcnn_tensor_free(ctx, o); return fail(ctx, CRCNN_ERR_CUDA, cudaGetErrorString(e)); }
        *out = o;
        return CRCNN_OK;
    }
    if (scale) {
        rc = ensure_domain(ctx, in, 1);
        if (!rc) rc = ensure_shoup(ctx, scale);
        if (rc) return rc;
    }
    crcnn_tensor *o = nullptr;
    rc = new_tensor(ctx, Nout, 2, in->ntt, &o);
    if (rc) return rc;
    {
        ProfScope ps(ctx, KC_POOL, lp_bytes(ctx, ((double)in->count + Nout) * 2 * ctx->K), (double)Nout * R * 2 * ctx->K * ctx->n);
        cudaError_t e = launch_pool(ctx->dP, ctx->n, ctx->K, in->d, d_index, Nout, R, scale ? scale->ntt_mul : nullptr,
                                    scale ? scale->ntt_mul_sh : nullptr, sum_fits_64(ctx, R), o->d, ctx->stream);
        if (e != cudaSuccess) { crcnn_tensor_free(ctx, o); return fail(ctx, CRCNN_ERR_CUDA, cudaGetErrorString(e)); }
    }
    *out = o;
    return CRCNN_OK;
}

int crcnn_pool_bn_forward(crcnn_ctx *ctx, crcnn_tensor *in, int batch, int xd, int yd, int zd, int xs, int ys, int xf, int yf,
                          crcnn_plain *scale, crcnn_plain *mean, crcnn_plain *invstd, crcnn_tensor **out) {
    if (!ctx) return CRCNN_ERR_INVALID_ARGUMENT;
    REQUIRE(in && mean && invstd && out, "null argument");
    REQUIRE((!scale || scale->count >= 1) && mean->count == zd && invstd->count == zd, "mean/var count does not match the channel count");
    const int xo = (xd - xf) / xs + 1, yo = (yd - yf) / ys + 1;
    const int R = xf * yf;
    if (!in->ntt || !sum_fits_64(ctx, R)) {
        crcnn_tensor *mid = nullptr;
        int rc = crcnn_pool_forward(ctx, in, batch, xd, yd, zd, xs, ys, xf, yf, scale, &mid);
        if (rc) return rc;
        rc = crcnn_bn_forward(ctx, mid, batch, zd, xo, yo, mean, invstd, out);
        crcnn_tensor_free(ctx, mid);
        return rc;
    }
    REQUIRE(batch > 0 && xd > 0 && yd > 0 && zd > 0 && xs > 0 && ys > 0 && xf > 0 && yf > 0 && xf <= xd && yf <= yd, "bad pooling geometry");
    REQUIRE(in->size == 2 && in->count == (long)batch * zd * xd * yd, "input tensor does not match the layer geometry");
    CU(cudaSetDevice(ctx->device));
    int xl, yl;
    boundaries(xd, yd, xs, ys, xf, yf, &xl, &yl);
    if ((xl + xs - 1) / xs != xo || (yl + ys - 1) / ys != yo)
        return fail(ctx, CRCNN_ERR_UNSUPPORTED, "stride larger than the window leaves outputs the reference never computes");
    const int Nout = batch * zd * xo * yo;
    std::vector<int> key = {3, batch, xd, yd, zd, xs, ys, xf, yf};
    const int *d_index = nullptr;
    if (ctx->index_cache.find(key) == ctx->index_cache.end()) {
        std::vector<int> table((size_t)Nout * R);
        size_t o = 0;
        for (int bz = 0; bz < batch * zd; bz++)
            for (int i = 0; i < xo; i++)
                for (int j = 0; j < yo; j++)
                    for (int kx = 0; kx < xf; kx++)
                        for (int ky = 0; ky < yf; ky++) table[o++] = (bz * xd + i * xs + kx) * yd + j * ys + ky;
        int rc = get_index_table(ctx, key, table, &d_index);
        if (rc) return rc;
    } else {
        d_index = ctx->index_cache[key];
    }
    int rc = ensure_pool_bn_consts(ctx, scale, mean, invstd);
    if (rc) return rc;
    crcnn_tensor *o = nullptr;
    rc = new_tensor(ctx, Nout, 2, 1, &o);
    if (rc) return rc;
    {
        ProfScope ps(ctx, KC_POOL, lp_bytes(ctx, ((double)in->count + Nout) * 2 * ctx->K), (double)Nout * (R + 1) * 2 * ctx->K * ctx->n);
        cudaError_t e = launch_pool(ctx->dP, ctx->n, ctx->K, in->d, d_index, Nout, R, invstd->fused_C, invstd->fused_Csh, true, o->d, ctx->stream,
                                    xo * yo, zd, invstd->fused_D);
        if (e != cudaSuccess) { crcnn_tensor_free(ctx, o); return fail(ctx, CRCNN_ERR_CUDA, cudaGetErrorString(e)); }
    }
    *out = o;
    return CRCNN_OK;
}

int crcnn_conv_pool_bn_forward_shard(crcnn_ctx *ctx, crcnn_tensor *in, crcnn_plain *w, crcnn_plain *b, int batch, int xd, int yd, int zd,
                                     int xs, int ys, int xf, int yf, int nf, int pxs, int pys, int pxf, int pyf, crcnn_plain *scale,
                                     crcnn_plain *mean, crcnn_plain *invstd, int k0, int kc, crcnn_tensor **out) {
    if (!ctx) return CRCNN_ERR_INVALID_ARGUMENT;
    REQUIRE(k0 >= 0 && kc >= 0 && k0 + kc <= nf, "bad output-channel shard");
    REQUIRE(in && w && b && mean && invstd && out, "null argument");
    REQUIRE(batch > 0 && xd > 0 && yd > 0 && zd > 0 && xs > 0 && ys > 0 && xf > 0 && yf > 0 && nf > 0 && xf <= xd && yf <= yd,
            "bad convolution geometry");
    const int cxo = (xd - xf) / xs + 1, cyo = (yd - yf) / ys + 1;
    REQUIRE(pxs > 0 && pys > 0 && pxf > 0 && pyf > 0 && pxf <= cxo && pyf <= cyo, "bad pooling geometry");
    const int pxo = (cxo - pxf) / pxs + 1, pyo = (cyo - pyf) / pys + 1;
    const int Rp = pxf * pyf, R = zd * xf * yf;
    REQUIRE(in->size == 2 && in->count == (long)batch * zd * xd * yd, "input tensor does not match the layer geometry");
    REQUIRE(w->count == (long)nf * R && b->count == nf, "kernel/bias count does not match the layer geometry");
    REQUIRE((!scale || scale->count >= 1) && mean->count == nf && invstd->count == nf, "mean/var count does not match the channel count");
    CU(cudaSetDevice(ctx->device));
    const bool pooled_grid = pxs <= pxf && pys <= pyf && xs <= xf && ys <= yf && pxs * xs <= xf && pys * ys <= yf && Rp <= 64 && sum_fits_64(ctx, Rp) &&
                             ctx->tcn_mode && tcn_planes_for(ctx->hp.d) == 7 && R <= TCN_MAX_R && tc_mac_available() == cudaSuccess &&
                             tcn_w_bytes(7, nf, tcn_kpad(R), ctx->K, ctx->n) <= ctx->weight_cache_bytes && !getenv("CRCNN_NO_POOLED_CONV");
    if (!pooled_grid) {
        if (k0 != 0 || kc != nf)
            return fail(ctx, CRCNN_ERR_UNSUPPORTED, "channel shards of conv + pool + batch-norm need the pooled-grid path");
        crcnn_tensor *mid = nullptr;
        int rc = crcnn_conv_forward(ctx, in, w, b, batch, xd, yd, zd, xs, ys, xf, yf, nf, &mid);
        if (rc) return rc;
        rc = crcnn_pool_bn_forward(ctx, mid, batch, cxo, cyo, nf, pxs, pys, pxf, pyf, scale, mean, invstd, out);
        crcnn_tensor_free(ctx, mid);
        return rc;
    }
    int rc = ensure_pool_bn_consts(ctx, scale, mean, invstd);
    if (rc) return rc;
    const long key[9] = {b->serial, scale ? scale->serial : -1, mean->serial, invstd->serial, (long)Rp, 0, 0, 0, 0};
    if (!w->folded_w || memcmp(key, w->folded_key, sizeof(key)) != 0) {
        if (w->folded_w) { crcnn_plain_free(ctx, w->folded_w); w->folded_w = nullptr; }
        if (w->folded_b) { crcnn_plain_free(ctx, w->folded_b); w->folded_b = nullptr; }
        const size_t pw = poly_words(ctx);
        rc = make_plain(ctx, std::vector<uint32_t>(w->off), std::vector<uint32_t>(w->idx), std::vector<uint64_t>(w->val), &w->folded_w);
        if (rc) return rc;
        w->folded_w->sparse_shape = false;
        w->folded_w->tc_state = -1; w->folded_w->tap_state = -1;
        rc = ensure_form(ctx, w->folded_w, PF_NTT_MUL);
        if (rc) return rc;
        CU(launch_fold_affine(ctx->dP, w->folded_w->ntt_mul, (long)nf * R, (long)pw, R, invstd->fused_C, nullptr, ctx->stream));
        rc = ensure_tcn_weights(ctx, w->folded_w, R);
        if (rc) return rc;
        rc = make_plain(ctx, std::vector<uint32_t>(b->off), std::vector<uint32_t>(b->idx), std::vector<uint64_t>(b->val), &w->folded_b);
        if (rc) return rc;
        w->folded_b->add_mult = Rp;
        rc = ensure_form(ctx, w->folded_b, PF_NTT_ADD);
        if (rc) return rc;
        CU(launch_fold_affine(ctx->dP, w->folded_b->ntt_add, (long)nf, (long)pw, 1, invstd->fused_C, invstd->fused_D, ctx->stream));
        memcpy(w->folded_key, key, sizeof(key));
    }
    const int sxd = xd - (pxf - 1) * xs, syd = yd - (pyf - 1) * ys;
    const int Nsum = batch * zd * sxd * syd;
    std::vector<int> skey = {4, batch, xd, yd, zd, xs, ys, pxf, pyf};
    const int *d_index = nullptr;
    if (ctx->index_cache.find(skey) == ctx->index_cache.end()) {
        std::vector<int> table((size_t)Nsum * Rp);
        size_t o = 0;
        for (int bz = 0; bz < batch * zd; bz++)
            for (int u = 0; u < sxd; u++)
                for (int v = 0; v < syd; v++)
                    for (int a = 0; a < pxf; a++)
                        for (int c = 0; c < pyf; c++) table[o++] = (bz * xd + u + a * xs) * yd + v + c * ys;
        rc = get_index_table(ctx, skey, table, &d_index);
        if (rc) return rc;
    } else {
        d_index = ctx->index_cache[skey];
    }
    crcnn_tensor *sums = nullptr, *pooled = nullptr;
    rc = new_tensor(ctx, Nsum, 2, in->ntt, &sums);
    if (rc) return rc;
    {
        ProfScope ps(ctx, KC_POOL, lp_bytes(ctx, ((double)in->count + Nsum) * 2 * ctx->K), (double)Nsum * Rp * 2 * ctx->K * ctx->n);
        cudaError_t e = launch_pool(ctx->dP, ctx->n, ctx->K, in->d, d_index, Nsum, Rp, nullptr, nullptr, true, sums->d, ctx->stream);
        if (e != cudaSuccess) { crcnn_tensor_free(ctx, sums); return fail(ctx, CRCNN_ERR_CUDA, cudaGetErrorString(e)); }
    }
    rc = crcnn_conv_forward_shard(ctx, sums, w->folded_w, w->folded_b, batch, sxd, syd, zd, pxs * xs, pys * ys, xf, yf, nf, k0, kc, &pooled);
    crcnn_tensor_free(ctx, sums);
    if (rc) return rc;
    if (pooled->count != (long)batch * kc * pxo * pyo || !pooled->ntt) {
        crcnn_tensor_free(ctx, pooled);
        return fail(ctx, CRCNN_ERR_UNSUPPORTED, "pooled-grid convolution produced an unexpected shape");
    }
    *out = pooled;
    return CRCNN_OK;
}

int crcnn_conv_pool_bn_forward(crcnn_ctx *ctx, crcnn_tensor *in, crcnn_plain *w, crcnn_plain *b, int batch, int xd, int yd, int zd,
                               int xs, int ys, int xf, int yf, int nf, int pxs, int pys, int pxf, int pyf, crcnn_plain *scale,
                               crcnn_plain *mean, crcnn_plain *invstd, crcnn_tensor **out) {
    return crcnn_conv_pool_bn_forward_shard(ctx, in, w, b, batch, xd, yd, zd, xs, ys, xf, yf, nf, pxs, pys, pxf, pyf, scale, mean, invstd, 0, nf, out);
}

int crcnn_bn_forward(crcnn_ctx *ctx, crcnn_tensor *in, int batch, int zd, int xd, int yd, crcnn_plain *mean,
                     crcnn_plain *invstd, crcnn_tensor **out) {
    if (!ctx) return CRCNN_ERR_INVALID_ARGUMENT;
    REQUIRE(in && mean && invstd && out, "null argument");
    REQUIRE(batch > 0 && zd > 0 && xd > 0 && yd > 0, "bad batch-norm geometry");
    REQUIRE(in->size == 2 && in->count == (long)batch * zd * xd * yd, "input tensor does not match the layer geometry");
    REQUIRE(mean->count == zd && invstd->count == zd, "mean/var count does not match the channel count");
    CU(cudaSetDevice(ctx->device));
    if (!in->ntt && ctx->tap_mode && tap_eligible(ctx, invstd)) {
        int rc = ensure_form(ctx, mean, PF_COEF_ADD);
        if (rc) return rc;
        crcnn_tensor *o = nullptr;
        rc = new_tensor(ctx, in->count, 2, 0, &o);
        if (rc) return rc;
        TapMulArgs a{};
        a.in = in->d; a.in_index = nullptr; a.R = 1; a.sub = mean->coef_add;
        a.t_off = invstd->d_off; a.t_idx = invstd->d_idx; a.t_val = invstd->d_val; a.per_channel = xd * yd; a.channels = zd;
        a.out = o->d; a.nout = in->count;
        ProfScope ps(ctx, KC_BN, lp_bytes(ctx, (double)in->count * 4 * ctx->K), (double)in->count * 2 * ctx->K * ctx->n);
        cudaError_t e = launch_tapmul(ctx->dP, ctx->n, ctx->K, a, ctx->stream);
        if (e != cudaSuccess) { crcnn_tensor_free(ctx, o); return fail(ctx, CRCNN_ERR_CUDA, cudaGetErrorString(e)); }
        *out = o;
        return CRCNN_OK;
    }
    int rc = ensure_domain(ctx, in, 1);
    if (!rc) rc = ensure_form(ctx, mean, PF_NTT_ADD);
    if (!rc) rc = ensure_shoup(ctx, invstd);
    if (rc) return rc;
    crcnn_tensor *o = nullptr;
    rc = new_tensor(ctx, in->count, 2, 1, &o);
    if (rc) return rc;
    {
        ProfScope ps(ctx, KC_BN, lp_bytes(ctx, (double)in->count * 4 * ctx->K), (double)in->count * 2 * ctx->K * ctx->n);
        cudaError_t e = launch_bn(ctx->dP, ctx->n, ctx->K, in->d, in->count, xd * yd, zd, mean->ntt_add, invstd->ntt_mul, invstd->ntt_mul_sh, o->d, ctx->stream);
        if (e != cudaSuccess) { crcnn_tensor_free(ctx, o); return fail(ctx, CRCNN_ERR_CUDA, cudaGetErrorString(e)); }
    }
    *out = o;
    return CRCNN_OK;
}

int crcnn_square(crcnn_ctx *ctx, crcnn_tensor *in, crcnn_tensor **out3) {
    if (!ctx) return CRCNN_ERR_INVALID_ARGUMENT;
    REQUIRE(in && out3, "null argument");
    REQUIRE(in->size == 2, "square expects size-2 ciphertexts");
    CU(cudaSetDevice(ctx->device));
    const bool have_ntt = in->ntt != 0;
    const bool lean = ctx->sq_lean != 0, fold = lean && behz_fold_ok(ctx->hp.d), copy_ninv = !(lean && have_ntt);
    crcnn_tensor *o = nullptr;
    int rc = new_tensor(ctx, in->count, 3, 0, &o);
    if (rc) return rc;
    const int KS = ctx->K + ctx->S;
    const size_t n = ctx->n, pw = poly_words(ctx);
    const long step = std::max<long>(1, std::min<long>(in->count, (long)((2ull << 30) / (5 * (size_t)KS * n * 8))));
    uint64_t *ext = nullptr, *prod = nullptr, *coef = nullptr;
    rc = dev_alloc(ctx, (size_t)step * 2 * KS * n * 8, (void **)&ext);
    if (!rc) rc = dev_alloc(ctx, (size_t)step * 3 * KS * n * 8, (void **)&prod);
    if (!rc && have_ntt) rc = dev_alloc(ctx, (size_t)step * 2 * pw * 8, (void **)&coef);
    if (rc) { crcnn_tensor_free(ctx, o); return rc; }
    for (long c0 = 0; c0 < in->count && !rc; c0 += step) {
        const long cur = std::min<long>(step, in->count - c0);
        const uint64_t *src = in->d + c0 * 2 * pw;
        cudaError_t e = cudaSuccess;
        if (have_ntt) {
            ProfScope ps(ctx, KC_NTT_INV, 2 * lp_bytes(ctx, (double)cur * 2 * ctx->K), lp_bfly(ctx, (double)cur * 2 * ctx->K));
            e = launch_ntt_grouped(ctx->dP, ctx->logn, coef, cur * 2 * ctx->K, 0, ctx->K, true, ctx->K, 0, ctx->stream, src,
                                   nullptr, 1, 1, copy_ninv);
        }
        if (e == cudaSuccess) { ProfScope ps(ctx, KC_BEHZ_LIFT, lp_bytes(ctx, (double)cur * 2 * (ctx->K + (have_ntt ? ctx->S : KS))), (double)cur * 2 * n * ctx->S * (ctx->K + 1)); e = launch_behz_lift(ctx->hp.d, ctx->n, have_ntt ? coef : src, have_ntt ? src : nullptr, cur, ext, ctx->stream, copy_ninv); }
        if (e == cudaSuccess) {
            if (have_ntt) {
                ProfScope ps(ctx, KC_NTT_FWD, 2 * lp_bytes(ctx, (double)cur * 2 * ctx->S), lp_bfly(ctx, (double)cur * 2 * ctx->S));
                e = launch_ntt_grouped(ctx->dP, ctx->logn, ext, cur * 2 * ctx->S, ctx->K, ctx->S, false, KS, ctx->K, ctx->stream);
            } else {
                ProfScope ps(ctx, KC_NTT_FWD, 2 * lp_bytes(ctx, (double)cur * 2 * KS), lp_bfly(ctx, (double)cur * 2 * KS));
                e = launch_ntt(ctx->dP, ctx->logn, ext, cur * 2 * KS, 0, KS, false, ctx->stream);
            }
        }
        if (e == cudaSuccess) {
            ProfScope ps(ctx, KC_SQ_TENSOR, lp_bytes(ctx, (double)cur * 5 * KS), lp_bfly(ctx, (double)cur * 3 * KS));
            e = launch_ntt_inv_tensor(ctx->dP, ctx->logn, ext, have_ntt ? src : nullptr, cur, KS, prod, fold, !lean, ctx->stream);
        }
        if (e == cudaSuccess) { ProfScope ps(ctx, KC_BEHZ_FLOOR, lp_bytes(ctx, (double)cur * 3 * (KS + ctx->K)),
                                                     (double)cur * 3 * n * (ctx->S * (ctx->K + 1) + ctx->S + ctx->K * ctx->S)); e = launch_behz_floor(ctx->hp.d, ctx->n, prod, cur, o->d + c0 * 3 * pw, ctx->stream, !lean); }
        if (e != cudaSuccess) rc = fail(ctx, CRCNN_ERR_CUDA, cudaGetErrorString(e));
    }
    dev_free(ctx, coef);
    dev_free(ctx, ext); dev_free(ctx, prod);
    if (rc) { crcnn_tensor_free(ctx, o); return rc; }
    *out3 = o;
    return CRCNN_OK;
}

int crcnn_relinearize(crcnn_ctx *ctx, crcnn_tensor *in3, crcnn_evk *evk, crcnn_tensor **out2) {
    if (!ctx) return CRCNN_ERR_INVALID_ARGUMENT;
    REQUIRE(in3 && evk && out2, "null argument");
    REQUIRE(in3->size == 3, "relinearize expects size-3 ciphertexts");
    int total_digits = 0;
    for (int i = 0; i < ctx->K; i++) {
        int bits = 0; for (uint64_t v = ctx->hp.d.tab[i].mod.q; v; v >>= 1) bits++;
        REQUIRE(evk->digits[i] * evk->dbc >= bits, "not enough evaluation keys");
        total_digits += evk->digits[i];
    }
    REQUIRE(total_digits <= 63, "too many key digits for 128-bit lazy accumulation");
    CU(cudaSetDevice(ctx->device));
    int rc = ensure_domain(ctx, in3, 0);
    if (rc) return rc;
    crcnn_tensor *o = nullptr;
    rc = new_tensor(ctx, in3->count, 2, 0, &o);
    if (rc) return rc;
    const size_t pw = poly_words(ctx);
    if (evk->has_r32 && ctx->relin_mode == 1) {
        const Relin32Consts &c = evk->r32.c;
        const size_t per_ct = relin32_scratch_bytes(ctx->n, ctx->K, c);
        const long step = std::max<long>(1, std::min<long>(std::min<long>(in3->count, 200000), (long)((2ull << 30) / per_ct)));
        void *scratch = nullptr;
        rc = dev_alloc(ctx, (size_t)step * per_ct, &scratch);
        if (rc) { crcnn_tensor_free(ctx, o); return rc; }
        for (long c0 = 0; c0 < in3->count && !rc; c0 += step) {
            const long cnt = std::min<long>(step, in3->count - c0);
            ProfScope ps(ctx, KC_RELIN32, lp_bytes(ctx, (double)cnt * 5 * ctx->K),
                         lp_bfly(ctx, (double)cnt * (c.D + 2 * ctx->K) * c.S3));
            cudaError_t e = relin32_run(ctx->dP, ctx->logn, ctx->K, evk->r32, in3->d + c0 * 3 * pw, o->d + c0 * 2 * pw, cnt, scratch, ctx->stream);
            if (e != cudaSuccess) rc = fail(ctx, CRCNN_ERR_CUDA, cudaGetErrorString(e));
        }
        dev_free(ctx, scratch);
        if (rc) { crcnn_tensor_free(ctx, o); return rc; }
        *out2 = o;
        return CRCNN_OK;
    }
    RelinArgs a{};
    a.evk = evk->d; a.dbc = evk->dbc;
    for (int i = 0; i < MAXK; i++) { a.key_off[i] = evk->key_off[i]; a.digits[i] = evk->digits[i]; }
    const size_t per_ct = (size_t)(1 + total_digits + 2) * pw * 8;
    const long step = std::max<long>(1, std::min<long>(in3->count, (long)((2ull << 30) / per_ct)));
    uint64_t *scratch = nullptr;
    rc = dev_alloc(ctx, (size_t)step * per_ct, (void **)&scratch);
    if (rc) { crcnn_tensor_free(ctx, o); return rc; }
    a.dsc = scratch;
    a.dig = scratch + (size_t)step * pw;
    a.acc = a.dig + (size_t)step * total_digits * pw;
    for (long c0 = 0; c0 < in3->count && !rc; c0 += step) {
        a.count = std::min<long>(step, in3->count - c0);
        a.in3 = in3->d + c0 * 3 * pw;
        a.out = o->d + c0 * 2 * pw;
        cudaError_t e;
        { ProfScope ps(ctx, KC_RELIN, lp_bytes(ctx, (double)a.count * 3 * ctx->K), lp_bfly(ctx, (double)a.count * total_digits * ctx->K)); e = launch_relin(ctx->dP, ctx->logn, ctx->K, a, ctx->stream); }
        if (e == cudaSuccess) {
            ProfScope ps(ctx, KC_NTT_INV, 2 * lp_bytes(ctx, (double)a.count * 2 * ctx->K) + lp_bytes(ctx, (double)a.count * 2 * ctx->K), lp_bfly(ctx, (double)a.count * 2 * ctx->K));
            e = launch_ntt_grouped(ctx->dP, ctx->logn, a.out, a.count * 2 * ctx->K, 0, ctx->K, true, ctx->K, 0, ctx->stream, a.acc, a.in3,
                                   2 * ctx->K, 3 * ctx->K);
        }
        if (e != cudaSuccess) rc = fail(ctx, CRCNN_ERR_CUDA, cudaGetErrorString(e));
    }
    dev_free(ctx, scratch);
    if (rc) { crcnn_tensor_free(ctx, o); return rc; }
    *out2 = o;
    return CRCNN_OK;
}

int crcnn_square_forward(crcnn_ctx *ctx, crcnn_tensor *in, crcnn_evk *evk, crcnn_tensor **out) {
    if (!ctx) return CRCNN_ERR_INVALID_ARGUMENT;
    crcnn_tensor *t3 = nullptr;
    int rc = crcnn_square(ctx, in, &t3);
    if (rc) return rc;
    rc = crcnn_relinearize(ctx, t3, evk, out);
    crcnn_tensor_free(ctx, t3);
    return rc;
}

int crcnn_transform_to_ntt(crcnn_ctx *ctx, crcnn_tensor *t) {
    if (!ctx) return CRCNN_ERR_INVALID_ARGUMENT;
    REQUIRE(t, "null argument");
    REQUIRE(!t->ntt, "tensor is already in NTT form");
    CU(cudaSetDevice(ctx->device));
    return ensure_domain(ctx, t, 1);
}
int crcnn_transform_from_ntt(crcnn_ctx *ctx, crcnn_tensor *t) {
    if (!ctx) return CRCNN_ERR_INVALID_ARGUMENT;
    REQUIRE(t, "null argument");
    REQUIRE(t->ntt, "tensor is not in NTT form");
    CU(cudaSetDevice(ctx->device));
    return ensure_domain(ctx, t, 0);
}

int crcnn_plain_op(crcnn_ctx *ctx, crcnn_tensor *t, crcnn_plain *p, long index, int op) {
    if (!ctx) return CRCNN_ERR_INVALID_ARGUMENT;
    REQUIRE(t && p && index >= 0 && index < p->count && op >= 0 && op <= 2, "bad plain_op arguments");
    CU(cudaSetDevice(ctx->device));
    int rc;
    const uint64_t *pl, *pl_sh = nullptr;
    if (op == 0) {
        rc = ensure_domain(ctx, t, 1);
        if (!rc) rc = ensure_shoup(ctx, p);
        if (rc) return rc;
        pl = p->ntt_mul + index * poly_words(ctx);
        pl_sh = p->ntt_mul_sh + index * poly_words(ctx);
    } else {
        rc = ensure_form(ctx, p, t->ntt ? PF_NTT_ADD : PF_COEF_ADD);
        if (rc) return rc;
        pl = (t->ntt ? p->ntt_add : p->coef_add) + index * poly_words(ctx);
    }
    ProfScope ps(ctx, KC_PLAIN_OP, lp_bytes(ctx, (double)t->count * (op == 0 ? t->size : 1) * 2 * ctx->K), (double)t->count * (op == 0 ? t->size : 1) * ctx->K * ctx->n);
    CU(launch_plain_op(ctx->dP, ctx->n, ctx->K, t->d, t->count, t->size, pl, pl_sh, op, ctx->stream));
    return CRCNN_OK;
}

int crcnn_add_many(crcnn_ctx *ctx, crcnn_tensor *t, crcnn_tensor **out) {
    if (!ctx) return CRCNN_ERR_INVALID_ARGUMENT;
    REQUIRE(t && out, "null argument");
    REQUIRE(t->count >= 1, "encrypteds cannot be empty");
    REQUIRE(t->size == 2, "add_many is implemented for size-2 ciphertexts");
    CU(cudaSetDevice(ctx->device));
    auto pass = [&](const uint64_t *src, long first, int nout, int g, uint64_t *dst) -> int {
        std::vector<int> key = {4, (int)first, nout, g};
        const int *d_index = nullptr;
        auto it = ctx->index_cache.find(key);
        if (it == ctx->index_cache.end()) {
            std::vector<int> table((size_t)nout * g);
            for (size_t i = 0; i < table.size(); i++) table[i] = (int)(first + (long)i);
            int rc = get_index_table(ctx, key, table, &d_index);
            if (rc) return rc;
        } else d_index = it->second;
        ProfScope ps(ctx, KC_POOL, lp_bytes(ctx, ((double)nout * g + nout) * 2 * ctx->K), (double)nout * g * 2 * ctx->K * ctx->n);
        CU(launch_pool(ctx->dP, ctx->n, ctx->K, src, d_index, nout, g, nullptr, nullptr, sum_fits_64(ctx, g), dst, ctx->stream));
        return CRCNN_OK;
    };
    crcnn_tensor *o = nullptr;
    int rc = new_tensor(ctx, 1, 2, t->ntt, &o);
    if (rc) return rc;
    if (t->count <= 128) {
        rc = pass(t->d, 0, 1, (int)t->count, o->d);
    } else {
        int g = 1;
        while ((long)g * g < t->count) g++;
        const long full = t->count / g, tail = t->count % g, groups = full + (tail ? 1 : 0);
        crcnn_tensor *part = nullptr;
        rc = new_tensor(ctx, groups, 2, t->ntt, &part);
        if (!rc) rc = pass(t->d, 0, (int)full, g, part->d);
        if (!rc && tail) rc = pass(t->d, full * g, 1, (int)tail, part->d + full * 2 * poly_words(ctx));
        if (!rc) rc = pass(part->d, 0, 1, (int)groups, o->d);
        crcnn_tensor_free(ctx, part);
    }
    if (rc) { crcnn_tensor_free(ctx, o); return rc; }
    *out = o;
    return CRCNN_OK;
}

int crcnn_prof_enable(crcnn_ctx *ctx, int on) {
    if (!ctx) return CRCNN_ERR_INVALID_ARGUMENT;
    ctx->prof_on = on != 0;
    return CRCNN_OK;
}
int crcnn_prof_reset(crcnn_ctx *ctx) {
// ... 378 lines not shown
```

crcnn_b200/csrc/host_selftest.cpp:

```cpp
#include <cinttypes>
#include <cstdio>
#include <cstdlib>
#include <vector>
#include "params.h"

using namespace crcnn;

static uint64_t fnv(const std::vector<uint64_t> &v) {
    uint64_t h = 1469598103934665603ULL;
    for (uint64_t x : v) { h ^= x; h *= 1099511628211ULL; }
    return h;
}

int main(int argc, char **argv) {
    if (argc < 4) { fprintf(stderr, "usage: host_selftest n t q...\n"); return 2; }
    int n = atoi(argv[1]);
    uint64_t t = strtoull(argv[2], nullptr, 0);
    std::vector<uint64_t> q;
    for (int i = 3; i < argc; i++) q.push_back(strtoull(argv[i], nullptr, 0));
    try {
        HostParams hp = derive_params(n, (int)q.size(), q.data(), t);
        const DeviceParams &d = hp.d;
        printf("K %d L %d S %d half %" PRIu64 "\n", d.K, d.L, d.S, d.half);
        for (int s = 0; s < d.K + d.S; s++) {
            printf("slot %d q %" PRIu64 " r0 %" PRIu64 " r1 %" PRIu64 " root %" PRIu64 " w %" PRIu64 " wp %" PRIu64 " iw %" PRIu64 " iwp %" PRIu64 "\n",
                   s, d.tab[s].mod.q, d.tab[s].mod.r0, d.tab[s].mod.r1, hp.roots[s], fnv(hp.w[s]), fnv(hp.wp[s]), fnv(hp.iw[s]), fnv(hp.iwp[s]));
        }
        for (int j = 0; j < d.K; j++)
            printf("prime %d delta %" PRIu64 " rho %" PRIu64 " lift %" PRIu64 "\n", j, d.delta[j], d.rho[j], d.lift_inc[j]);
        uint64_t x = 0x123456789abcdef1ULL, y = 0xfedcba9876543211ULL;
        for (int s = 0; s < d.K + d.S; s++) {
            const Mod &m = d.tab[s].mod;
            for (int it = 0; it < 1000; it++) {
                x = x * 6364136223846793005ULL + 1442695040888963407ULL;
                y = y * 2862933555777941757ULL + 3037000493ULL;
                uint64_t a = x % (4 * m.q), b = y % m.q;
                uint64_t want = (uint64_t)(((unsigned __int128)a * b) % m.q);
                if (mulmod(a, b, m) != want) { printf("MULMOD MISMATCH\n"); return 1; }
                uint64_t wp = (uint64_t)((((unsigned __int128)b) << 64) / m.q);
                uint64_t lazy = mulshoup_lazy(a, b, wp, m.q);
                if (lazy >= 2 * m.q || lazy % m.q != want) { printf("SHOUP MISMATCH\n"); return 1; }
            }
        }
        for (int j = 0; j < d.K; j++) {
            const Mod &m = d.tab[j].mod;
            const TcnFold f = tcn_fold_make(m.q);
            printf("fold %d ok %u T %u delta %u\n", j, f.ok, f.T, f.delta);
            if (!f.ok) continue;
            for (int it = 0; it < 200000; it++) {
                uint32_t s[13];
                const int mode = it % 8;
                for (int w = 0; w < 13; w++) {
                    x = x * 6364136223846793005ULL + 1442695040888963407ULL;
                    const uint32_t r = (uint32_t)(x >> 33);
                    s[w] = mode == 0 ? 0x7fffffffu : mode == 1 ? 0u : mode == 2 ? ((x >> 20) & 1 ? 0x7fffffffu : 0u)
                         : mode == 3 ? 7u * 4096u * 255u * 255u - (r & 3) : mode == 4 ? (r >> (x & 31)) : r;
                }
                y = y * 2862933555777941757ULL + 3037000493ULL;
                const uint64_t bias = mode == 0 ? m.q - 1 : (it & 1) ? y % m.q : 0;
                unsigned __int128 z = 0;
                for (int w = 12; w >= 0; w--) z = (z << 8) + s[w];
                const uint64_t want = (uint64_t)((z + bias) % m.q);
                if (tcn_fold_reduce(s, bias, f, m.q) != want) { printf("FOLD MISMATCH\n"); return 1; }
            }
        }
        for (int sidx = 0; sidx < d.K + d.S; sidx++) {
            const Mod &m = d.tab[sidx].mod;
            const Fold128 f = fold128_make(m.q);
            printf("fold128 %d ok %u delta %u\n", sidx, f.ok, f.delta);
            if (!f.ok) continue;
            for (int it = 0; it < 200000; it++) {
                x = x * 6364136223846793005ULL + 1442695040888963407ULL;
                y = y * 2862933555777941757ULL + 3037000493ULL;
                U128 z;
                const int mode = it % 8;
                z.lo = mode == 0 ? ~0ull : mode == 1 ? 0 : mode == 2 ? m.q - 1 : mode == 3 ? m.q : x;
                z.hi = mode == 0 ? ~0ull : mode == 1 ? 0 : mode == 2 ? 0 : mode == 3 ? (y >> (y & 63)) : mode == 4 ? (y >> 40) : y;
                const uint64_t want = (uint64_t)(((((unsigned __int128)z.hi) << 64) | z.lo) % m.q);
                if (reduce128_fold(z, f) != want || barrett128(z, m) != want) { printf("FOLD128 MISMATCH\n"); return 1; }
            }
        }
        typedef unsigned __int128 u128;
        for (int s = 0; s < d.K + d.S; s++) {
            const uint64_t q = d.tab[s].mod.q;
            const bool ok_ninv = (u128)d.tab[s].ninv * (uint64_t)n % q == 1;
            bool ok = ok_ninv;
            if (s < d.K) {
                ok = ok && d.mt_inv_qhat_n[s] < q && (u128)d.mt_inv_qhat_n[s] * (uint64_t)n % q == d.mt_inv_qhat[s];
                ok = ok && d.fl_c_n[s] < q && (u128)d.fl_c_n[s] * (uint64_t)n % q == d.fl_c[s];
            } else {
                ok = ok && d.fl_T_n[s - d.K] < q && (u128)d.fl_T_n[s - d.K] * (uint64_t)n % q == d.fl_T[s - d.K];
            }
            printf("ninv %d ok %d\n", s, ok ? 1 : 0);
            if (!ok) { printf("NINV CONSTANT MISMATCH\n"); return 1; }
        }
        for (int s = 0; s < d.K + d.S; s++) {
            const uint64_t q = d.tab[s].mod.q, nq = 0 - q;
            const uint64_t ws[] = {0, 1, q - 1, q / 2, 0x5555555555555555ULL % q, 0};
            long checked = 0;
            for (int wi = 0; wi < 6; wi++) {
                uint64_t w = ws[wi];
                for (int it = 0; it < 20000; it++) {
                    x = x * 6364136223846793005ULL + 1442695040888963407ULL;
                    y = y * 2862933555777941757ULL + 3037000493ULL;
                    if (wi == 5) w = y % q;
                    const uint64_t wp = (uint64_t)(((u128)w << 64) / q);
                    const int mode = it % 8;
                    const uint64_t yv = mode == 0 ? 0 : mode == 1 ? ~0ull : mode == 2 ? (x % (~0ull / q + 1)) * q
                                      : mode == 3 ? (~0ull / q) * q : mode == 4 ? q - 1 : mode == 5 ? 8 * q - 1 - (x & 7) : x;
                    const uint64_t r = mulshoup_lazy4(yv, w, wp, nq);
                    if (r >= 4 * q || r % q != (uint64_t)((u128)w * yv % q)) { printf("SHOUP4 MISMATCH\n"); return 1; }
                    const uint64_t a = x % q;
                    const U128 z = sqr128(a);
                    if (((u128)z.hi << 64 | z.lo) != (u128)a * a) { printf("SQR128 MISMATCH\n"); return 1; }
                    checked++;
                }
            }
            printf("shoup4 %d checked %ld\n", s, checked);
            const int k = reduce64_shape_k(q);
            if (k) {
                for (int it = 0; it < 200000; it++) {
                    x = x * 6364136223846793005ULL + 1442695040888963407ULL;
                    const int mode = it % 6;
                    const uint64_t v = mode == 0 ? ~0ull : mode == 1 ? 0 : mode == 2 ? q : mode == 3 ? q - 1 : mode == 4 ? (x % 16) * q + (x >> 60) : x;
                    if (reduce64_shape(v, q, k) != v % q || reduce64(v, d.tab[s].mod) != v % q) { printf("REDUCE64 MISMATCH\n"); return 1; }
                }
            }
            printf("reduce64_shape %d k %d\n", s, k);
        }
        for (int i = 4; i >= 0; i--) {
            double vals[] = {0.0867, -3.25, 0.0, 1.0, 2.8215};
            std::vector<uint32_t> idx; std::vector<uint64_t> val;
            encode_fractional_sparse(vals[i], n, t, idx, val);
            printf("enc %.4f nnz %zu", vals[i], idx.size());
            for (size_t e = 0; e < idx.size(); e++) printf(" %u:%" PRIu64, idx[e], val[e]);
            printf("\n");
        }
        printf("OK\n");
    } catch (const std::exception &e) {
        printf("ERROR %s\n", e.what());
        return 1;
    }
    return 0;
}
```

crcnn_b200/csrc/modarith.cuh:

```cuda
#pragma once
#include <cstdint>

#if defined(__CUDACC__)
#define CRCNN_HD __host__ __device__ __forceinline__
#else
#define CRCNN_HD inline
#endif

namespace crcnn {

struct Mod {
    uint64_t q;
    uint64_t r0;
    uint64_t r1;
};

CRCNN_HD uint64_t mulhi64(uint64_t a, uint64_t b) {
#if defined(__CUDA_ARCH__)
    return __umul64hi(a, b);
#else
    return (uint64_t)(((unsigned __int128)a * b) >> 64);
#endif
}

struct U128 {
    uint64_t lo, hi;
};

CRCNN_HD U128 mul128(uint64_t a, uint64_t b) {
    U128 r;
    r.lo = a * b;
    r.hi = mulhi64(a, b);
    return r;
}

CRCNN_HD U128 sqr128(uint64_t a) {
    const uint64_t a0 = (uint32_t)a, a1 = a >> 32;
    const uint64_t lo = a0 * a0, mid = (a0 * a1) << 1, hi = a1 * a1;
    U128 r;
    r.lo = lo + (mid << 32);
    r.hi = hi + (mid >> 32) + (r.lo < lo);
    return r;
}

CRCNN_HD void mac128(U128 &acc, uint64_t a, uint64_t b) {
    uint64_t lo = a * b;
    uint64_t hi = mulhi64(a, b);
    acc.lo += lo;
    acc.hi += hi + (acc.lo < lo);
}

struct Acc7 {
    uint32_t a0, a1, a2, a3;
    uint32_t b0, b1, b2;
};

CRCNN_HD Acc7 acc7_zero() { return Acc7{0, 0, 0, 0, 0, 0, 0}; }

CRCNN_HD void mac7(Acc7 &c, uint64_t x, uint64_t w) {
#if defined(__CUDA_ARCH__)
    uint32_t x0 = (uint32_t)x, x1 = (uint32_t)(x >> 32), w0 = (uint32_t)w, w1 = (uint32_t)(w >> 32);
    asm("mad.lo.cc.u32 %0, %7, %9, %0;\n\t"
        "madc.hi.cc.u32 %1, %7, %9, %1;\n\t"
        "madc.lo.cc.u32 %2, %8, %10, %2;\n\t"
        "madc.hi.u32 %3, %8, %10, %3;\n\t"
        "mad.lo.cc.u32 %4, %7, %10, %4;\n\t"
        "madc.hi.cc.u32 %5, %7, %10, %5;\n\t"
        "addc.u32 %6, %6, 0;\n\t"
        "mad.lo.cc.u32 %4, %8, %9, %4;\n\t"
        "madc.hi.cc.u32 %5, %8, %9, %5;\n\t"
        "addc.u32 %6, %6, 0;\n\t"
        : "+r"(c.a0), "+r"(c.a1), "+r"(c.a2), "+r"(c.a3), "+r"(c.b0), "+r"(c.b1), "+r"(c.b2)
        : "r"(x0), "r"(x1), "r"(w0), "r"(w1));
#else
    typedef unsigned __int128 u128;
    uint64_t x0 = (uint32_t)x, x1 = x >> 32, w0 = (uint32_t)w, w1 = w >> 32;
    u128 even = ((u128)(((uint64_t)c.a3 << 32) | c.a2) << 64) | (((uint64_t)c.a1 << 32) | c.a0);
    even += (u128)(x0 * w0) + ((u128)(x1 * w1) << 64);
    u128 odd = ((u128)c.b2 << 64) | (((uint64_t)c.b1 << 32) | c.b0);
    odd += (u128)(x0 * w1) + (u128)(x1 * w0);
    c.a0 = (uint32_t)even; c.a1 = (uint32_t)(even >> 32); c.a2 = (uint32_t)(even >> 64); c.a3 = (uint32_t)(even >> 96);
    c.b0 = (uint32_t)odd; c.b1 = (uint32_t)(odd >> 32); c.b2 = (uint32_t)(odd >> 64);
#endif
}

CRCNN_HD U128 acc7_value(const Acc7 &c) {
    uint64_t lo = ((uint64_t)c.a1 << 32) | c.a0, hi = ((uint64_t)c.a3 << 32) | c.a2;
    uint64_t add_lo = (uint64_t)c.b0 << 32, add_hi = ((uint64_t)c.b2 << 32) | c.b1;
    U128 r;
    r.lo = lo + add_lo;
    r.hi = hi + add_hi + (r.lo < lo);
    return r;
}

CRCNN_HD Acc7 acc7_from(uint64_t v) { return Acc7{(uint32_t)v, (uint32_t)(v >> 32), 0, 0, 0, 0, 0}; }

CRCNN_HD void add128_64(U128 &acc, uint64_t v) {
    acc.lo += v;
    acc.hi += (acc.lo < v);
}

CRCNN_HD uint64_t barrett128(U128 z, const Mod &m) {
    uint64_t carry = mulhi64(z.lo, m.r0);
    uint64_t t_lo = z.lo * m.r1;
    uint64_t t_hi = mulhi64(z.lo, m.r1);
    uint64_t s1 = t_lo + carry;
    uint64_t c1 = t_hi + (s1 < carry);
    uint64_t u_lo = z.hi * m.r0;
    uint64_t u_hi = mulhi64(z.hi, m.r0);
    uint64_t s2 = s1 + u_lo;
    uint64_t c2 = u_hi + (s2 < u_lo);
    uint64_t qest = z.hi * m.r1 + c1 + c2;
    uint64_t r = z.lo - qest * m.q;
    return r >= m.q ? r - m.q : r;
}

CRCNN_HD uint64_t reduce64(uint64_t x, const Mod &m) {
    uint64_t r = x - mulhi64(x, m.r1) * m.q;
    return r >= m.q ? r - m.q : r;
}

CRCNN_HD int reduce64_shape_k(uint64_t q) {
    int k = 0;
    for (uint64_t v = q; v; v >>= 1) k++;
    return (k >= 48 && k <= 63 && ((1ull << k) - q) < (1ull << 27)) ? k : 0;
}
CRCNN_HD uint64_t reduce64_shape(uint64_t x, uint64_t q, int k) {
    const uint32_t delta = (uint32_t)((1ull << k) - q), hi = (uint32_t)(x >> k);
    const uint64_t r = (x & ((1ull << k) - 1)) + (uint64_t)hi * delta;
    return r >= q ? r - q : r;
}

CRCNN_HD uint64_t mulmod(uint64_t a, uint64_t b, const Mod &m) { return barrett128(mul128(a, b), m); }

CRCNN_HD uint64_t addmod(uint64_t a, uint64_t b, uint64_t q) {
    uint64_t s = a + b;
    return s >= q ? s - q : s;
}
CRCNN_HD uint64_t submod(uint64_t a, uint64_t b, uint64_t q) { return a >= b ? a - b : a + q - b; }
CRCNN_HD uint64_t negmod(uint64_t a, uint64_t q) { return a ? q - a : 0; }

CRCNN_HD uint64_t mulshoup_lazy(uint64_t y, uint64_t w, uint64_t wp, uint64_t q) {
    uint64_t h = mulhi64(wp, y);
    return y * w - h * q;
}

CRCNN_HD uint64_t mulshoup_lazy4(uint64_t y, uint64_t w, uint64_t wp, uint64_t nq) {
#if defined(__CUDA_ARCH__)
    uint32_t y0 = (uint32_t)y, y1 = (uint32_t)(y >> 32), p0 = (uint32_t)wp, p1 = (uint32_t)(wp >> 32);
    uint32_t w0 = (uint32_t)w, w1 = (uint32_t)(w >> 32), n0 = (uint32_t)nq, n1 = (uint32_t)(nq >> 32);
    uint32_t a, b, h0, h1, r0, r1;
    uint64_t wa, wb;
    asm("mul.wide.u32 %0, %2, %3;\n\t"
        "mul.wide.u32 %1, %4, %5;\n\t"
        : "=l"(wa), "=l"(wb) : "r"(p1), "r"(y0), "r"(p0), "r"(y1));
    a = (uint32_t)(wa >> 32);
    b = (uint32_t)(wb >> 32);
    asm("mad.lo.cc.u32 %0, %2, %3, %4;\n\t"
        "madc.hi.u32 %1, %2, %3, 0;\n\t"
        "add.cc.u32 %0, %0, %5;\n\t"
        "addc.u32 %1, %1, 0;\n\t"
        : "=r"(h0), "=r"(h1) : "r"(p1), "r"(y1), "r"(a), "r"(b));
    asm("mul.lo.u32 %0, %2, %3;\n\t"
        "mul.hi.u32 %1, %2, %3;\n\t"
        "mad.lo.cc.u32 %0, %4, %5, %0;\n\t"
        "madc.hi.u32 %1, %4, %5, %1;\n\t"
        "mad.lo.u32 %1, %2, %6, %1;\n\t"
        "mad.lo.u32 %1, %7, %3, %1;\n\t"
        "mad.lo.u32 %1, %4, %8, %1;\n\t"
        "mad.lo.u32 %1, %9, %5, %1;\n\t"
        : "=&r"(r0), "=&r"(r1) : "r"(y0), "r"(w0), "r"(h0), "r"(n0), "r"(w1), "r"(y1), "r"(n1), "r"(h1));
    return ((uint64_t)r1 << 32) | r0;
#else
    uint64_t y0 = (uint32_t)y, y1 = y >> 32, p0 = (uint32_t)wp, p1 = wp >> 32;
    uint64_t h = p1 * y1 + ((p1 * y0) >> 32) + ((p0 * y1) >> 32);
    return y * w + h * nq;
#endif
}

struct TcnFold {
    uint32_t T;
    uint32_t delta;
    uint32_t sh, mask;
    uint32_t c8, c16, c24;
    uint32_t ok;
};

inline TcnFold tcn_fold_make(uint64_t q) {
    typedef unsigned __int128 u128;
    TcnFold f{};
    int k = 0;
    for (uint64_t v = q; v; v >>= 1) k++;
    if (k < 48 || k > 56) return f;
    const uint64_t delta = (1ull << k) - q;
    if (delta == 0 || delta >> 28) return f;
    const u128 T = (u128)delta << (56 - k);
    if (T >> 32 || T >= q) return f;
    const u128 one = 1, smax = 0x7fffffffu, w32 = 0xffffffffu;
    const u128 La = smax * (1 + (one << 8) + (one << 16) + (one << 24)), Lb = smax * (1 + (one << 8) + (one << 16));
    const u128 Ha = La, Hb = smax * (1 + (one << 8));
    const u128 a = w32 * T + La, b = (Ha >> 32) * T + Lb + w32 * T, e = (Hb >> 32) * T;
    if (a >> 64 || b >> 64 || e >> 60) return f;
    const u128 y = a + (b << 32) + (e << 64);
    const u128 h1 = (y >> k) >> 32;
    const u128 v = w32 * delta + ((one << k) - 1) + (q - 1), w = h1 * delta;
    if (h1 >> 32 || v >> 64 || w >> 62) return f;
    const u128 V = v + (w << 32);
    const u128 g = V >> k;
    if (V >> 96 || g >> 32) return f;
    if (g * delta + ((one << k) - 1) >= 2 * (u128)q) return f;
    f.T = (uint32_t)T; f.delta = (uint32_t)delta; f.sh = (uint32_t)(k - 32); f.mask = (1u << (k - 32)) - 1;
    f.c8 = 1u << 8; f.c16 = 1u << 16; f.c24 = 1u << 24; f.ok = 1;
    return f;
}

CRCNN_HD uint32_t tcn_shr64(uint32_t lo, uint32_t hi, uint32_t sh) {
#if defined(__CUDA_ARCH__)
    return __funnelshift_r(lo, hi, sh);
#else
    return (lo >> sh) | (hi << (32 - sh));
#endif
}

CRCNN_HD uint64_t tcn_fold_reduce(const uint32_t (&s)[13], uint64_t bias, const TcnFold &f, uint64_t q) {
    const uint64_t La = (uint64_t)s[3] * f.c24 + ((uint64_t)s[2] * f.c16 + ((uint64_t)s[1] * f.c8 + s[0]));
    const uint64_t Lb = (uint64_t)s[6] * f.c16 + ((uint64_t)s[5] * f.c8 + s[4]);
    const uint64_t Ha = (uint64_t)s[10] * f.c24 + ((uint64_t)s[9] * f.c16 + ((uint64_t)s[8] * f.c8 + s[7]));
    const uint64_t Hb = (uint64_t)s[12] * f.c8 + s[11];
    const uint64_t a = (uint64_t)(uint32_t)Ha * f.T + La;
    const uint64_t b = (uint64_t)(uint32_t)Hb * f.T + ((Ha >> 32) * f.T + Lb);
    const uint64_t e = (Hb >> 32) * f.T;
    const uint32_t y0 = (uint32_t)a;
    const uint64_t m1 = (a >> 32) + (uint32_t)b;
    const uint32_t y1 = (uint32_t)m1;
    const uint64_t m2 = (b >> 32) + (uint64_t)(uint32_t)e + (m1 >> 32);
    const uint32_t y2 = (uint32_t)m2;
    const uint32_t y3 = (uint32_t)(e >> 32) + (uint32_t)(m2 >> 32);
    const uint32_t h0 = tcn_shr64(y1, y2, f.sh), h1 = tcn_shr64(y2, y3, f.sh);
    const uint64_t l = ((uint64_t)(y1 & f.mask) << 32) | y0;
    const uint64_t v = (uint64_t)h0 * f.delta + l + bias;
    const uint64_t w = (uint64_t)h1 * f.delta;
    const uint64_t m3 = (v >> 32) + (uint32_t)w;
    const uint32_t V1 = (uint32_t)m3, V2 = (uint32_t)(w >> 32) + (uint32_t)(m3 >> 32);
    const uint32_t g = tcn_shr64(V1, V2, f.sh);
    const uint64_t lo = ((uint64_t)(V1 & f.mask) << 32) | (uint32_t)v;
    const uint64_t r = (uint64_t)g * f.delta + lo;
    return r >= q ? r - q : r;
}

struct Fold128 {
    uint64_t q;
    uint32_t delta, sh, mask, ok;
};

inline Fold128 fold128_make(uint64_t q) {
    typedef unsigned __int128 u128;
    Fold128 f{};
    f.q = q;
    int k = 0;
    for (uint64_t v = q; v; v >>= 1) k++;
    if (k < 54 || k > 61) return f;
    const uint64_t delta = (1ull << k) - q;
    if (delta == 0 || delta >> 27) return f;
    const u128 one = 1, zmax = ~(u128)0;
    const u128 y = ((one << k) - 1) + (zmax >> k) * delta;
    const u128 V = ((one << k) - 1) + (y >> k) * delta;
    const u128 g = V >> k;
    if (y >> 112 || (y >> k) >> 64 || V >> 96 || g >> 32) return f;
    if (g * delta + ((one << k) - 1) >= 2 * (u128)q) return f;
    f.delta = (uint32_t)delta; f.sh = (uint32_t)(k - 32); f.mask = (1u << (k - 32)) - 1; f.ok = 1;
    return f;
}

CRCNN_HD uint64_t reduce128_fold(U128 z, const Fold128 &f) {
    const uint32_t z0 = (uint32_t)z.lo, z1 = (uint32_t)(z.lo >> 32), z2 = (uint32_t)z.hi, z3 = (uint32_t)(z.hi >> 32);
    const uint32_t h0 = tcn_shr64(z1, z2, f.sh), h1 = tcn_shr64(z2, z3, f.sh), h2 = z3 >> f.sh;
    const uint64_t l = ((uint64_t)(z1 & f.mask) << 32) | z0;
    const uint64_t t0 = (uint64_t)h0 * f.delta + l;
    const uint64_t u = (uint64_t)h1 * f.delta + (t0 >> 32);
    const uint64_t u2 = (uint64_t)h2 * f.delta + (u >> 32);
    const uint32_t y0 = (uint32_t)t0, y1 = (uint32_t)u, y2 = (uint32_t)u2, y3 = (uint32_t)(u2 >> 32);
    const uint32_t g0 = tcn_shr64(y1, y2, f.sh), g1 = tcn_shr64(y2, y3, f.sh);
    const uint64_t l2 = ((uint64_t)(y1 & f.mask) << 32) | y0;
    const uint64_t v = (uint64_t)g0 * f.delta + l2;
    const uint64_t w = (uint64_t)g1 * f.delta + (v >> 32);
    const uint32_t V0 = (uint32_t)v, V1 = (uint32_t)w, V2 = (uint32_t)(w >> 32);
    const uint32_t g = tcn_shr64(V1, V2, f.sh);
    const uint64_t l3 = ((uint64_t)(V1 & f.mask) << 32) | V0;
    const uint64_t r = (uint64_t)g * f.delta + l3;
    return r >= f.q ? r - f.q : r;
}

}
```

crcnn_b200/csrc/tc_ptx.cuh:

```cuda
#pragma once
#include <cuda.h>
#include <cuda_runtime.h>
#include <cstdint>
#include <cstdio>

namespace crcnn {
namespace tcptx {

__device__ __forceinline__ uint32_t smem_u32(const void *p) { return (uint32_t)__cvta_generic_to_shared(p); }

__device__ __forceinline__ void mbar_init(uint32_t bar, uint32_t count) {
    asm volatile("mbarrier.init.shared::cta.b64 [%0], %1;" ::"r"(bar), "r"(count));
}
__device__ __forceinline__ void mbar_expect_tx(uint32_t bar, uint32_t bytes) {
    asm volatile("mbarrier.arrive.expect_tx.shared::cta.b64 _, [%0], %1;" ::"r"(bar), "r"(bytes) : "memory");
}
__device__ __forceinline__ void mbar_arrive(uint32_t bar) {
    asm volatile("mbarrier.arrive.shared::cta.b64 _, [%0];" ::"r"(bar) : "memory");
}
__device__ __forceinline__ bool mbar_try_wait(uint32_t bar, uint32_t parity) {
    uint32_t ok;
    asm volatile(
        "{\n\t.reg .pred p;\n\t"
        "mbarrier.try_wait.parity.shared::cta.b64 p, [%1], %2;\n\t"
        "selp.u32 %0, 1, 0, p;\n\t}"
        : "=r"(ok)
        : "r"(bar), "r"(parity)
        : "memory");
    return ok != 0;
}
__device__ __forceinline__ void mbar_wait(uint32_t bar, uint32_t parity) {
    uint32_t spins = 0;
    while (!mbar_try_wait(bar, parity)) {
        if (++spins > (1u << 28)) {
            printf("tcgen05 kernel: mbarrier wait timed out (block %d thread %d)\n", blockIdx.x, threadIdx.x);
            __trap();
        }
    }
}
__device__ __forceinline__ void fence_barrier_init() { asm volatile("fence.mbarrier_init.release.cluster;" ::: "memory"); }
__device__ __forceinline__ void fence_proxy_async() { asm volatile("fence.proxy.async.shared::cta;" ::: "memory"); }

__device__ __forceinline__ void tma_load_2d(uint32_t dst, const CUtensorMap *map, uint32_t bar, int c0, int c1) {
    asm volatile(
        "cp.async.bulk.tensor.2d.shared::cluster.global.tile.mbarrier::complete_tx::bytes [%0], [%1, {%3, %4}], [%2];" ::"r"(dst),
        "l"(map), "r"(bar), "r"(c0), "r"(c1)
        : "memory");
}
__device__ __forceinline__ void tma_load_4d(uint32_t dst, const CUtensorMap *map, uint32_t bar, int c0, int c1, int c2, int c3) {
    asm volatile(
        "cp.async.bulk.tensor.4d.shared::cluster.global.tile.mbarrier::complete_tx::bytes [%0], [%1, {%3, %4, %5, %6}], [%2];" ::"r"(dst),
        "l"(map), "r"(bar), "r"(c0), "r"(c1), "r"(c2), "r"(c3)
        : "memory");
}
__device__ __forceinline__ void prefetch_tmap(const CUtensorMap *map) {
    asm volatile("prefetch.tensormap [%0];" ::"l"(map) : "memory");
}

__device__ __forceinline__ void tc_fence_before() { asm volatile("tcgen05.fence::before_thread_sync;" ::: "memory"); }
__device__ __forceinline__ void tc_fence_after() { asm volatile("tcgen05.fence::after_thread_sync;" ::: "memory"); }
__device__ __forceinline__ void tmem_alloc(uint32_t dst_smem, uint32_t cols) {
    asm volatile("tcgen05.alloc.cta_group::1.sync.aligned.shared::cta.b32 [%0], %1;" ::"r"(dst_smem), "r"(cols) : "memory");
    asm volatile("tcgen05.relinquish_alloc_permit.cta_group::1.sync.aligned;" ::: "memory");
}
__device__ __forceinline__ void tmem_dealloc(uint32_t taddr, uint32_t cols) {
    asm volatile("tcgen05.dealloc.cta_group::1.sync.aligned.b32 %0, %1;" ::"r"(taddr), "r"(cols) : "memory");
}
__device__ __forceinline__ void umma_i8(uint32_t tmem_d, uint64_t desc_a, uint64_t desc_b, uint32_t idesc, uint32_t accumulate) {
    asm volatile(
        "{\n\t.reg .pred p;\n\t"
        "setp.ne.b32 p, %4, 0;\n\t"
        "tcgen05.mma.cta_group::1.kind::i8 [%0], %1, %2, %3, p;\n\t}" ::"r"(tmem_d),
        "l"(desc_a), "l"(desc_b), "r"(idesc), "r"(accumulate)
        : "memory");
}
__device__ __forceinline__ void umma_commit(uint32_t bar) {
    asm volatile("tcgen05.commit.cta_group::1.mbarrier::arrive::one.shared::cluster.b64 [%0];" ::"r"(bar) : "memory");
}
__device__ __forceinline__ void tmem_ld32(uint32_t taddr, int (&v)[32]) {
    asm volatile(
        "tcgen05.ld.sync.aligned.32x32b.x32.b32 "
        "{%0, %1, %2, %3, %4, %5, %6, %7, %8, %9, %10, %11, %12, %13, %14, %15, "
        "%16, %17, %18, %19, %20, %21, %22, %23, %24, %25, %26, %27, %28, %29, %30, %31}, [%32];"
        : "=r"(v[0]), "=r"(v[1]), "=r"(v[2]), "=r"(v[3]), "=r"(v[4]), "=r"(v[5]), "=r"(v[6]), "=r"(v[7]), "=r"(v[8]),
          "=r"(v[9]), "=r"(v[10]), "=r"(v[11]), "=r"(v[12]), "=r"(v[13]), "=r"(v[14]), "=r"(v[15]), "=r"(v[16]),
          "=r"(v[17]), "=r"(v[18]), "=r"(v[19]), "=r"(v[20]), "=r"(v[21]), "=r"(v[22]), "=r"(v[23]), "=r"(v[24]),
          "=r"(v[25]), "=r"(v[26]), "=r"(v[27]), "=r"(v[28]), "=r"(v[29]), "=r"(v[30]), "=r"(v[31])
        : "r"(taddr)
        : "memory");
    asm volatile("tcgen05.wait::ld.sync.aligned;" ::: "memory");
}


__device__ __forceinline__ void tmem_ld16_nowait(uint32_t taddr, int *v) {
    asm volatile(
        "tcgen05.ld.sync.aligned.32x32b.x16.b32 "
        "{%0, %1, %2, %3, %4, %5, %6, %7, %8, %9, %10, %11, %12, %13, %14, %15}, [%16];"
        : "=r"(v[0]), "=r"(v[1]), "=r"(v[2]), "=r"(v[3]), "=r"(v[4]), "=r"(v[5]), "=r"(v[6]), "=r"(v[7]), "=r"(v[8]),
          "=r"(v[9]), "=r"(v[10]), "=r"(v[11]), "=r"(v[12]), "=r"(v[13]), "=r"(v[14]), "=r"(v[15])
        : "r"(taddr)
        : "memory");
}

__device__ __forceinline__ uint32_t cluster_ctarank() {
    uint32_t r;
    asm volatile("mov.u32 %0, %%cluster_ctarank;" : "=r"(r));
    return r;
}
__device__ __forceinline__ void cluster_sync_all() {
    asm volatile("barrier.cluster.arrive.release.aligned;" ::: "memory");
    asm volatile("barrier.cluster.wait.acquire.aligned;" ::: "memory");
}
constexpr uint32_t PAIR_LEADER_MASK = 0xFEFFFFFFu;
__device__ __forceinline__ void tma_load_2d_pair(uint32_t dst, const CUtensorMap *map, uint32_t bar, int c0, int c1) {
    asm volatile(
        "cp.async.bulk.tensor.2d.cta_group::2.shared::cluster.global.mbarrier::complete_tx::bytes [%0], [%1, {%3, %4}], [%2];" ::"r"(dst),
        "l"(map), "r"(bar & PAIR_LEADER_MASK), "r"(c0), "r"(c1)
        : "memory");
}
__device__ __forceinline__ void tma_load_4d_pair(uint32_t dst, const CUtensorMap *map, uint32_t bar, int c0, int c1, int c2, int c3) {
    asm volatile(
        "cp.async.bulk.tensor.4d.cta_group::2.shared::cluster.global.mbarrier::complete_tx::bytes [%0], [%1, {%3, %4, %5, %6}], [%2];" ::"r"(dst),
        "l"(map), "r"(bar & PAIR_LEADER_MASK), "r"(c0), "r"(c1), "r"(c2), "r"(c3)
        : "memory");
}
__device__ __forceinline__ void tmem_alloc_pair(uint32_t dst_smem, uint32_t cols) {
    asm volatile("tcgen05.alloc.cta_group::2.sync.aligned.shared::cta.b32 [%0], %1;" ::"r"(dst_smem), "r"(cols) : "memory");
    asm volatile("tcgen05.relinquish_alloc_permit.cta_group::2.sync.aligned;" ::: "memory");
}
__device__ __forceinline__ void tmem_dealloc_pair(uint32_t taddr, uint32_t cols) {
    asm volatile("tcgen05.dealloc.cta_group::2.sync.aligned.b32 %0, %1;" ::"r"(taddr), "r"(cols) : "memory");
}
__device__ __forceinline__ void umma_i8_pair(uint32_t tmem_d, uint64_t desc_a, uint64_t desc_b, uint32_t idesc, uint32_t accumulate) {
    asm volatile(
        "{\n\t.reg .pred p;\n\t"
        "setp.ne.b32 p, %4, 0;\n\t"
        "tcgen05.mma.cta_group::2.kind::i8 [%0], %1, %2, %3, p;\n\t}" ::"r"(tmem_d),
        "l"(desc_a), "l"(desc_b), "r"(idesc), "r"(accumulate)
        : "memory");
}
__device__ __forceinline__ void umma_commit_pair(uint32_t bar) {
    asm volatile("tcgen05.commit.cta_group::2.mbarrier::arrive::one.shared::cluster.multicast::cluster.b64 [%0], %1;" ::"r"(bar),
                 "h"((uint16_t)3)
                 : "memory");
}
__device__ __forceinline__ void mbar_arrive_remote(uint32_t bar, uint32_t rank) {
    asm volatile(
        "{\n\t.reg .b32 ra;\n\t"
        "mapa.shared::cluster.u32 ra, %0, %1;\n\t"
        "mbarrier.arrive.release.cluster.shared::cluster.b64 _, [ra];\n\t}" ::"r"(bar),
        "r"(rank)
        : "memory");
}

__device__ __forceinline__ void tmem_ld4(uint32_t taddr, uint32_t (&v)[4]) {
    asm volatile("tcgen05.ld.sync.aligned.32x32b.x4.b32 {%0, %1, %2, %3}, [%4];"
                 : "=r"(v[0]), "=r"(v[1]), "=r"(v[2]), "=r"(v[3])
                 : "r"(taddr)
                 : "memory");
}
__device__ __forceinline__ void tmem_ld_wait() { asm volatile("tcgen05.wait::ld.sync.aligned;" ::: "memory"); }

__device__ __forceinline__ uint64_t umma_desc_sw128(uint32_t smem_addr) {
    return (uint64_t)((smem_addr & 0x3FFFF) >> 4) | (1ull << 16) | (64ull << 32) | (1ull << 46) | (2ull << 61);
}
__device__ __forceinline__ uint64_t umma_desc_sw64(uint32_t smem_addr) {
    return (uint64_t)((smem_addr & 0x3FFFF) >> 4) | (1ull << 16) | (32ull << 32) | (1ull << 46) | (4ull << 61);
}
__device__ __forceinline__ uint64_t umma_desc_sw32(uint32_t smem_addr) {
    return (uint64_t)((smem_addr & 0x3FFFF) >> 4) | (1ull << 16) | (16ull << 32) | (1ull << 46) | (6ull << 61);
}

typedef CUresult (*EncodeTiledFn)(CUtensorMap *, CUtensorMapDataType, cuuint32_t, void *, const cuuint64_t *, const cuuint64_t *,
                                  const cuuint32_t *, const cuuint32_t *, CUtensorMapInterleave, CUtensorMapSwizzle,
                                  CUtensorMapL2promotion, CUtensorMapFloatOOBfill);

inline EncodeTiledFn encode_tiled() {
    static EncodeTiledFn fn = [] {
        void *p = nullptr;
        cudaDriverEntryPointQueryResult qres;
        if (cudaGetDriverEntryPoint("cuTensorMapEncodeTiled", &p, cudaEnableDefault, &qres) != cudaSuccess ||
            qres != cudaDriverEntryPointSuccess)
            p = nullptr;
        return (EncodeTiledFn)p;
    }();
    return fn;
}

}
}
```

crcnn_b200/csrc/tcn_mac.cu:

```cuda
#include <cuda.h>
#include <cuda_runtime.h>
#include <cstdio>
#include <cstdlib>
#include "devcfg.cuh"
#include "modarith.cuh"
#include "tc_ptx.cuh"
#include "tcn_mac.cuh"

namespace crcnn {

namespace {

using namespace tcptx;

constexpr int TCN_PLANES = 7;
constexpr int TCN_CLASSES = 2 * TCN_PLANES - 1;
constexpr int TCN_EPI_WARPS = 8;
constexpr int TCN_THREADS = 32 * (2 + TCN_EPI_WARPS);
constexpr int TCN_TMEM_COLS = 512;

__device__ __forceinline__ U128 tcn_combine(const uint32_t (&S)[TCN_CLASSES][4], int i) {
    uint32_t z0 = S[0][i], z1 = S[4][i], z2 = S[8][i], z3 = S[12][i];
#define CRCNN_ADD4(a0, a1, a2, a3)                                                                                     \
    asm("add.cc.u32 %0, %0, %4;\n\taddc.cc.u32 %1, %1, %5;\n\taddc.cc.u32 %2, %2, %6;\n\taddc.u32 %3, %3, %7;"          \
        : "+r"(z0), "+r"(z1), "+r"(z2), "+r"(z3)                                                                       \
        : "r"(a0), "r"(a1), "r"(a2), "r"(a3))
    CRCNN_ADD4(S[1][i] << 8, __funnelshift_l(S[1][i], S[5][i], 8), __funnelshift_l(S[5][i], S[9][i], 8), S[9][i] >> 24);
    CRCNN_ADD4(S[2][i] << 16, __funnelshift_l(S[2][i], S[6][i], 16), __funnelshift_l(S[6][i], S[10][i], 16), S[10][i] >> 16);
    CRCNN_ADD4(S[3][i] << 24, __funnelshift_l(S[3][i], S[7][i], 24), __funnelshift_l(S[7][i], S[11][i], 24), S[11][i] >> 8);
#undef CRCNN_ADD4
    U128 z;
    z.lo = ((uint64_t)z1 << 32) | z0;
    z.hi = ((uint64_t)z3 << 32) | z2;
    return z;
}

__device__ __forceinline__ uint64_t tcn_fold_out(const uint32_t (&S)[TCN_CLASSES][4], int i, uint64_t bias, const TcnFold &f, uint64_t q) {
    uint32_t s[TCN_CLASSES];
#pragma unroll
    for (int w = 0; w < TCN_CLASSES; w++) s[w] = S[w][i];
    return tcn_fold_reduce(s, bias, f, q);
}

template <int BK> struct TcnCfg {
    static constexpr int A_STAGE = TCN_PLANES * TCN_BM * BK;
    static constexpr int B_STAGE = TCN_PLANES * TCN_NB * BK;
    static constexpr int STAGES = BK == 128 ? 2 : 4;
    static constexpr size_t SMEM = 1024 + (size_t)STAGES * (A_STAGE + B_STAGE) + 8 * (2 * STAGES + 2) + 16;
};

template <int BK, bool FOLD>
__global__ void __launch_bounds__(TCN_THREADS, 1)
tcn_mac_kernel(const __grid_constant__ CUtensorMap tmW, const __grid_constant__ CUtensorMap tmX,
               const DeviceParams *__restrict__ P, TcnMacArgs a) {
    using Cfg = TcnCfg<BK>;
    constexpr int STAGES = Cfg::STAGES, A_STAGE = Cfg::A_STAGE, B_STAGE = Cfg::B_STAGE;
    constexpr uint32_t IDESC_BASE = (2u << 4)
                                    | ((uint32_t)(TCN_BM >> 4) << 24);

    extern __shared__ uint8_t smem_raw[];
    const uint32_t base = (smem_u32(smem_raw) + 1023u) & ~1023u;
    uint8_t *base_ptr = smem_raw + (base - smem_u32(smem_raw));
    const uint32_t sA = base, sB = base + STAGES * A_STAGE;
    const uint32_t off_bar = STAGES * (A_STAGE + B_STAGE);
    const uint32_t bar_full = base + off_bar, bar_empty = bar_full + 8 * STAGES;
    const uint32_t bar_tfull = bar_empty + 8 * STAGES, bar_tempty = bar_tfull + 8;
    const uint32_t tmem_slot = bar_tempty + 8;
    volatile uint32_t *tmem_slot_ptr = reinterpret_cast<volatile uint32_t *>(base_ptr + off_bar + 8 * (2 * STAGES + 2));

    const int warp = threadIdx.x >> 5, lane = threadIdx.x & 31;
    const int n = a.n;
    const int m_tiles = (a.M + TCN_BM - 1) / TCN_BM;
    const long items = (long)a.nslots * m_tiles;
    const int chunks = (a.ncols + TCN_NB - 1) / TCN_NB;
    const int ksteps = (a.R + 31) / 32;
    const int KB = (ksteps * 32 + BK - 1) / BK;

    if (threadIdx.x == 0) {
        for (int s = 0; s < STAGES; s++) { mbar_init(bar_full + 8 * s, 1); mbar_init(bar_empty + 8 * s, 1); }
        mbar_init(bar_tfull, 1);
        mbar_init(bar_tempty, TCN_EPI_WARPS);
        fence_barrier_init();
        prefetch_tmap(&tmW);
        prefetch_tmap(&tmX);
    }
    if (warp == 0) tmem_alloc(tmem_slot, TCN_TMEM_COLS);
    tc_fence_before();
    __syncthreads();
    tc_fence_after();
    const uint32_t tmem_base = *tmem_slot_ptr;

    if (warp == 0) {
        if (lane == 0) {
            int stage = 0;
            uint32_t phase = 0;
            for (long item = blockIdx.x; item < items; item += gridDim.x) {
                const int sl = (int)(item / m_tiles), mt = (int)(item % m_tiles);
                for (int ch = 0; ch < chunks; ch++)
                    for (int kb = 0; kb < KB; kb++) {
                        mbar_wait(bar_empty + 8 * stage, phase ^ 1);
                        mbar_expect_tx(bar_full + 8 * stage, A_STAGE + B_STAGE);
                        tma_load_4d(sA + stage * A_STAGE, &tmW, bar_full + 8 * stage, kb * BK, mt * TCN_BM, 0, a.slot0 + sl);
                        tma_load_4d(sB + stage * B_STAGE, &tmX, bar_full + 8 * stage, kb * BK, ch * TCN_NB, 0, sl);
                        if (++stage == STAGES) { stage = 0; phase ^= 1; }
                    }
            }
        }
        __syncwarp();
    } else if (warp == 1) {
        if (lane == 0) {
            int stage = 0;
            uint32_t phase = 0, acc_phase = 0;
            for (long item = blockIdx.x; item < items; item += gridDim.x)
                for (int ch = 0; ch < chunks; ch++) {
                    mbar_wait(bar_tempty, acc_phase ^ 1);
                    tc_fence_after();
                    for (int kb = 0; kb < KB; kb++) {
                        mbar_wait(bar_full + 8 * stage, phase);
                        tc_fence_after();
                        const uint32_t aS = sA + stage * A_STAGE, bS = sB + stage * B_STAGE;
                        const int nks = BK == 128 ? min(4, ksteps - kb * 4) : 1;
                        for (int ks = 0; ks < nks; ks++) {
                            const bool fresh = (kb | ks) == 0;
                            auto descA = [&](int pa) { return (BK == 128 ? umma_desc_sw128(aS + pa * (TCN_BM * BK)) : umma_desc_sw32(aS + pa * (TCN_BM * BK))) + 2 * ks; };
                            auto descB = [&](int pb) { return (BK == 128 ? umma_desc_sw128(bS + pb * (TCN_NB * BK)) : umma_desc_sw32(bS + pb * (TCN_NB * BK))) + 2 * ks; };
                            constexpr uint32_t ID_ALL = IDESC_BASE | ((uint32_t)((TCN_PLANES * TCN_NB) >> 3) << 17);
                            constexpr uint32_t ID_HI = IDESC_BASE | ((uint32_t)(((TCN_PLANES - 1) * TCN_NB) >> 3) << 17);
                            constexpr uint32_t ID_ONE = IDESC_BASE | ((uint32_t)(TCN_NB >> 3) << 17);
                            if (fresh) {
                                umma_i8(tmem_base, descA(0), descB(0), ID_ALL, 0u);
                                umma_i8(tmem_base + TCN_PLANES * TCN_NB, descA(TCN_PLANES - 1), descB(1), ID_HI, 0u);
                                umma_i8(tmem_base + (TCN_PLANES - 1) * TCN_NB, descA(TCN_PLANES - 1), descB(0), ID_ONE, 1u);
#pragma unroll
                                for (int pa = 1; pa < TCN_PLANES - 1; pa++) umma_i8(tmem_base + pa * TCN_NB, descA(pa), descB(0), ID_ALL, 1u);
                            } else {
#pragma unroll
                                for (int pa = 0; pa < TCN_PLANES; pa++) umma_i8(tmem_base + pa * TCN_NB, descA(pa), descB(0), ID_ALL, 1u);
                            }
                        }
                        umma_commit(bar_empty + 8 * stage);
                        if (++stage == STAGES) { stage = 0; phase ^= 1; }
                    }
                    umma_commit(bar_tfull);
                    acc_phase ^= 1;
                }
        }
        __syncwarp();
    } else {
        const int qd = warp & 3, half = (warp - 2) >> 2;
        const long pw = (long)a.K * n;
        uint32_t acc_phase = 0;
        for (long item = blockIdx.x; item < items; item += gridDim.x) {
            const int sl = (int)(item / m_tiles), mt = (int)(item % m_tiles);
            const int slot = a.slot0 + sl, j = slot / n, c = slot - j * n;
            const Mod mod = P->tab[j].mod;
            const TcnFold fold = a.fold[FOLD ? j : 0];
            const int m = mt * TCN_BM + qd * 16 + lane;
            const bool valid = lane < 16 && m < a.M;
            const uint64_t bias = (a.bias && valid) ? __ldg(a.bias + (long)m * pw + (long)j * n + c) : 0;
            const long row_off = (long)(a.m0 + m) * a.Pimg;
            for (int ch = 0; ch < chunks; ch++) {
                mbar_wait(bar_tfull, acc_phase);
                tc_fence_after();
#pragma unroll 1
                for (int g = 0; g < 4; g++) {
                    const int col0 = ch * TCN_NB + (half * 4 + g) * 4;
                    uint32_t S[TCN_CLASSES][4];
#pragma unroll
                    for (int w = 0; w < TCN_CLASSES; w++)
                        tmem_ld4(tmem_base + ((uint32_t)(qd * 32) << 16) + w * TCN_NB + (half * 4 + g) * 4, S[w]);
                    tmem_ld_wait();
#pragma unroll
                    for (int i = 0; i < 4; i++) {
                        const int col = col0 + i;
                        if (!valid || col >= a.ncols) continue;
                        const int p = col >> 1, poly = col & 1;
                        uint64_t r;
                        if constexpr (FOLD) {
                            r = tcn_fold_out(S, i, poly == 0 ? bias : 0, fold, mod.q);
                        } else {
                            r = barrett128(tcn_combine(S, i), mod);
                            if (poly == 0 && a.bias) r = addmod(r, bias, mod.q);
                        }
                        const long oct = (long)(p / a.Pimg) * ((long)a.Mtotal * a.Pimg) + row_off + p % a.Pimg;
                        a.out[((oct * 2 + poly) * a.K + j) * (long)n + c] = r;
                    }
                }
                tc_fence_before();
                __syncwarp();
                if (lane == 0) mbar_arrive(bar_tempty);
                acc_phase ^= 1;
            }
        }
    }
    tc_fence_before();
    __syncthreads();
    if (warp == 0) tmem_dealloc(tmem_base, TCN_TMEM_COLS);
}

constexpr int TCN2_CB = 128;
constexpr int TCN2_MT = 32;
constexpr int TCN2_KBMAX = 2;
constexpr int TCN2_EPI_WARPS = 12;
constexpr int TCN2_THREADS = 32 * (2 + TCN2_EPI_WARPS);

#ifdef CRCNN_TCN2_TRACE
constexpr int TCN2_TRACE_N = 8192;
__device__ unsigned long long g_tcn2_trace[3][TCN2_TRACE_N];
__device__ int g_tcn2_trace_n[3];
#define TCN2_TR(role, tag)                                                                                    \
    do {                                                                                                      \
        if (blockIdx.x == 0) {                                                                                \
            const int i_ = g_tcn2_trace_n[role];                                                              \
            if (i_ < TCN2_TRACE_N) { g_tcn2_trace[role][i_] = ((unsigned long long)(tag) << 56) | (clock64() & 0xffffffffffffffull); g_tcn2_trace_n[role] = i_ + 1; } \
        }                                                                                                     \
    } while (0)
#else
#define TCN2_TR(role, tag) do { } while (0)
#endif

template <int BK> struct Tcn2Cfg {
    static constexpr int W_BLOCK = TCN_PLANES * TCN2_MT * BK;
    static constexpr int X_STAGE = TCN2_CB * BK;
#ifndef TCN2_STAGES_SMALL
#define TCN2_STAGES_SMALL 8
#define TCN2_STAGES_BIG 6
#endif
    static constexpr int STAGES = BK == 128 ? TCN2_STAGES_BIG : TCN2_STAGES_SMALL;
    static constexpr size_t BARS = (8 * (2 * STAGES + 4) + 16 + 127) / 128 * 128;
    static constexpr size_t smem(int ns, bool staged) {
        const size_t ops = 1024 + (size_t)ns * TCN2_KBMAX * W_BLOCK + (size_t)STAGES * X_STAGE;
        return staged ? ops + BARS + (size_t)(ns - 1) * TCN2_MT * TCN2_CB * 8 : ops + 8 * (2 * STAGES + 4) + 16;
    }
};

__device__ __forceinline__ void tcn_store_sector(uint64_t *p, uint64_t a, uint64_t b, uint64_t c, uint64_t d) {
    asm volatile("st.global.v4.u64 [%0], {%1, %2, %3, %4};" ::"l"(p), "l"(a), "l"(b), "l"(c), "l"(d) : "memory");
}

template <int BK, bool FOLD, int BIAS, int NS, bool STAGED = false>
__global__ void __launch_bounds__(TCN2_THREADS, 1)
tcn2_mac_kernel(const __grid_constant__ CUtensorMap tmW, const __grid_constant__ CUtensorMap tmX,
                const DeviceParams *__restrict__ P, TcnMacArgs a) {
    using Cfg = Tcn2Cfg<BK>;
    constexpr int STAGES = Cfg::STAGES, W_BLOCK = Cfg::W_BLOCK, X_STAGE = Cfg::X_STAGE;
    constexpr uint32_t IDESC_BASE = (2u << 4) | ((uint32_t)(TCN2_CB >> 4) << 24);
    constexpr uint32_t ID_ALL = IDESC_BASE | ((uint32_t)((TCN_PLANES * TCN2_MT) >> 3) << 17);
    constexpr uint32_t ID_HI = IDESC_BASE | ((uint32_t)(((TCN_PLANES - 1) * TCN2_MT) >> 3) << 17);
    constexpr uint32_t ID_ONE = IDESC_BASE | ((uint32_t)(TCN2_MT >> 3) << 17);

    extern __shared__ uint8_t smem_raw[];
    const uint32_t base = (smem_u32(smem_raw) + 1023u) & ~1023u;
    uint8_t *base_ptr = smem_raw + (base - smem_u32(smem_raw));
    const uint32_t sW = base, sX = base + NS * TCN2_KBMAX * W_BLOCK;
    const uint32_t off_bar = NS * TCN2_KBMAX * W_BLOCK + STAGES * X_STAGE;
    const uint32_t bar_full = base + off_bar, bar_empty = bar_full + 8 * STAGES;
    const uint32_t bar_wfull = bar_empty + 8 * STAGES, bar_wempty = bar_wfull + 8;
    const uint32_t bar_tfull = bar_wempty + 8, bar_tempty = bar_tfull + 8;
    const uint32_t tmem_slot = bar_tempty + 8;
    volatile uint32_t *tmem_slot_ptr = reinterpret_cast<volatile uint32_t *>(base_ptr + off_bar + 8 * (2 * STAGES + 4));
    uint64_t *out_stage = reinterpret_cast<uint64_t *>(base_ptr + off_bar + Cfg::BARS);

    const int warp = threadIdx.x >> 5, lane = threadIdx.x & 31;
    const int n = a.n;
    const int m_tiles = (a.M + TCN2_MT - 1) / TCN2_MT;
    const long groups = a.nslots / NS;
    const long items = (groups > blockIdx.x ? (groups - blockIdx.x + gridDim.x - 1) / gridDim.x : 0) * m_tiles;
    auto item_group = [&](long it) { return (long)blockIdx.x + (it / m_tiles) * gridDim.x; };
    const int chunks = (a.ncols + TCN2_CB - 1) / TCN2_CB;
    const int ksteps = (a.R + 31) / 32;
    const int KB = (ksteps * 32 + BK - 1) / BK;

    if (threadIdx.x == 0) {
        for (int s = 0; s < STAGES; s++) { mbar_init(bar_full + 8 * s, 1); mbar_init(bar_empty + 8 * s, 1); }
        mbar_init(bar_wfull, 1);
        mbar_init(bar_wempty, 1);
        mbar_init(bar_tfull, 1);
        mbar_init(bar_tempty, TCN2_EPI_WARPS);
        fence_barrier_init();
        prefetch_tmap(&tmW);
        prefetch_tmap(&tmX);
    }
    if (warp == 0) tmem_alloc(tmem_slot, TCN_TMEM_COLS);
    tc_fence_before();
    __syncthreads();
    tc_fence_after();
    const uint32_t tmem_base = *tmem_slot_ptr;

    auto plane_of = [](int bi) { return bi == 0 ? 0 : (bi == 1 ? TCN_PLANES - 1 : bi - 1); };

    if (warp == 0) {
        if (lane == 0) {
            int stage = 0;
            uint32_t phase = 0, wphase = 0;
            for (long item = 0; item < items; item++) {
                const int sl = (int)item_group(item) * NS, mt = (int)(item % m_tiles);
                mbar_wait(bar_wempty, wphase ^ 1);
                mbar_expect_tx(bar_wfull, NS * KB * W_BLOCK);
                for (int s = 0; s < NS; s++)
                    for (int kb = 0; kb < KB; kb++)
                        tma_load_4d(sW + (s * TCN2_KBMAX + kb) * W_BLOCK, &tmW, bar_wfull, kb * BK, mt * TCN2_MT, 0, a.slot0 + sl + s);
                wphase ^= 1;
                for (int ch = 0; ch < chunks; ch++)
                    for (int s = 0; s < NS; s++)
                        for (int kb = 0; kb < KB; kb++)
                            for (int bi = 0; bi < TCN_PLANES; bi++) {
                                mbar_wait(bar_empty + 8 * stage, phase ^ 1);
                                TCN2_TR(0, bi);
                                mbar_expect_tx(bar_full + 8 * stage, X_STAGE);
                                tma_load_4d(sX + stage * X_STAGE, &tmX, bar_full + 8 * stage, kb * BK, ch * TCN2_CB, plane_of(bi), sl + s);
                                if (++stage == STAGES) { stage = 0; phase ^= 1; }
                            }
            }
        }
        __syncwarp();
    } else if (warp == 1) {
        if (lane == 0) {
            int stage = 0;
            uint32_t phase = 0, acc_phase = 0, wphase = 0;
            for (long item = 0; item < items; item++) {
                mbar_wait(bar_wfull, wphase);
                wphase ^= 1;
                tc_fence_after();
                for (int chs = 0; chs < chunks * NS; chs++) {
                    const int s = NS == 1 ? 0 : chs % NS;
                    TCN2_TR(1, 100);
                    mbar_wait(bar_tempty, acc_phase ^ 1);
                    TCN2_TR(1, 101);
                    tc_fence_after();
                    for (int kb = 0; kb < KB; kb++) {
                        const uint32_t wS = sW + (s * TCN2_KBMAX + kb) * W_BLOCK;
                        const int nks = BK == 128 ? min(4, ksteps - kb * 4) : 1;
                        for (int bi = 0; bi < TCN_PLANES; bi++) {
                            const int pb = plane_of(bi);
                            mbar_wait(bar_full + 8 * stage, phase);
                            TCN2_TR(1, kb * 8 + bi);
                            tc_fence_after();
                            const uint32_t xS = sX + stage * X_STAGE;
                            for (int ks = 0; ks < nks; ks++) {
                                const uint64_t dx = (BK == 128 ? umma_desc_sw128(xS) : umma_desc_sw32(xS)) + 2 * ks;
                                auto descW = [&](int pa) { return (BK == 128 ? umma_desc_sw128(wS + pa * (TCN2_MT * BK)) : umma_desc_sw32(wS + pa * (TCN2_MT * BK))) + 2 * ks; };
                                if ((kb | ks) == 0 && pb == 0) {
                                    umma_i8(tmem_base, dx, descW(0), ID_ALL, 0u);
                                } else if ((kb | ks) == 0 && pb == TCN_PLANES - 1) {
                                    umma_i8(tmem_base + TCN_PLANES * TCN2_MT, dx, descW(1), ID_HI, 0u);
                                    umma_i8(tmem_base + (TCN_PLANES - 1) * TCN2_MT, dx, descW(0), ID_ONE, 1u);
                                } else {
                                    umma_i8(tmem_base + pb * TCN2_MT, dx, descW(0), ID_ALL, 1u);
                                }
                            }
                            umma_commit(bar_empty + 8 * stage);
                            if (++stage == STAGES) { stage = 0; phase ^= 1; }
                        }
                    }
                    umma_commit(bar_tfull);
                    TCN2_TR(1, 102);
                    acc_phase ^= 1;
                }
                umma_commit(bar_wempty);
            }
        }
        __syncwarp();
    } else {
        const int qd = warp & 3, sub = (warp - 2) >> 2;
        const long pw = (long)a.K * n;
        const long m_stride = 2L * a.Pimg * pw;
        uint32_t acc_phase = 0;
        for (long item = 0; item < items; item++) {
            const int sl = (int)item_group(item) * NS, mt = (int)(item % m_tiles);
            const int slot = a.slot0 + sl, j = slot / n, c = slot - j * n;
            const Mod mod = P->tab[j].mod;
            const TcnFold fold = a.fold[FOLD ? j : 0];
            const long slot_off = (long)j * n + c;
            const int m_valid = min(TCN2_MT, a.M - mt * TCN2_MT);
            const int groups = (m_valid + 3) >> 2;
            uint64_t bias_lane[NS];
#pragma unroll
            for (int s = 0; s < NS; s++)
                bias_lane[s] = (BIAS != 0 && a.bias && lane < m_valid) ? __ldg(a.bias + (long)(mt * TCN2_MT + lane) * pw + slot_off + s) : 0;
            const uint64_t *bias_p = a.bias ? a.bias + (long)(mt * TCN2_MT) * pw + slot_off : nullptr;
            for (int ch = 0; ch < chunks; ch++) {
                const int col = ch * TCN2_CB + qd * 32 + lane;
                const bool valid = col < a.ncols;
                const int p = col >> 1, poly = col & 1;
                const long colbase = (long)(p / a.Pimg) * ((long)a.Mtotal * a.Pimg) + p % a.Pimg;
                uint64_t *out_col = a.out + (colbase * 2 + poly) * pw + slot_off + (long)(a.m0 + mt * TCN2_MT) * m_stride;
                const bool add_bias = poly == 0 && (BIAS != 0 || bias_p != nullptr);
#pragma unroll
              for (int s = 0; s < NS; s++) {
                if (warp == 2 && lane == 0) TCN2_TR(2, 200);
                mbar_wait(bar_tfull, acc_phase);
                if (warp == 2 && lane == 0) TCN2_TR(2, 201);
                tc_fence_after();
#pragma unroll 1
                for (int g = sub; g < groups; g += TCN2_EPI_WARPS / 4) {
                    const int mloc = g * 4;
                    uint32_t S[TCN_CLASSES][4];
#pragma unroll
                    for (int w = 0; w < TCN_CLASSES; w++)
                        tmem_ld4(tmem_base + ((uint32_t)(qd * 32) << 16) + w * TCN2_MT + mloc, S[w]);
                    tmem_ld_wait();
                    uint64_t *op = out_col + (long)mloc * m_stride + s;
                    const uint64_t *bp = bias_p + (long)mloc * pw + s;
#pragma unroll
                    for (int i = 0; i < 4; i++) {
                        if (mloc + i < m_valid) {
                            uint64_t bias_m = 0;
                            if constexpr (BIAS != 0) bias_m = __shfl_sync(0xffffffffu, bias_lane[s], mloc + i);
                            else if (add_bias) bias_m = __ldg(bp);
                            uint64_t r;
                            if constexpr (FOLD) {
                                r = tcn_fold_out(S, i, add_bias ? bias_m : 0, fold, mod.q);
                            } else {
                                r = barrett128(tcn_combine(S, i), mod);
                                if (add_bias) r = addmod(r, bias_m, mod.q);
                            }
                            if constexpr (BIAS == 2) { if (valid && r == ~0ull) *op = r; }
                            else if constexpr (STAGED && NS == 4) {
                                uint64_t *st = out_stage + (mloc + i) * TCN2_CB + qd * 32 + lane;
                                if (s < NS - 1) st[s * (TCN2_MT * TCN2_CB)] = r;
                                else if (valid) tcn_store_sector(op - (NS - 1), st[0], st[TCN2_MT * TCN2_CB], st[2 * TCN2_MT * TCN2_CB], r);
                            } else if (valid) *op = r;
                        }
                        op += m_stride;
                        bp += pw;
                    }
                }
                tc_fence_before();
                __syncwarp();
                if (lane == 0) mbar_arrive(bar_tempty);
                if (warp == 2 && lane == 0) TCN2_TR(2, 202);
                acc_phase ^= 1;
              }
            }
        }
    }
    tc_fence_before();
    __syncthreads();
    if (warp == 0) tmem_dealloc(tmem_base, TCN_TMEM_COLS);
}

__global__ void __launch_bounds__(256)
tcn_split_kernel(TcnSplitArgs a) {
    __shared__ uint64_t tile[32][133];
    __shared__ long src_off[128];
    const int n = a.n, K = a.K;
    const int rows_per = a.Kpad < 128 ? 128 / a.Kpad : 1;
    const int col0 = blockIdx.x * rows_per;
    const int st = blockIdx.y;
    const int r0 = blockIdx.z * 128;
    const int slot = a.slot0 + st * 32;
    const int j = slot / n, c0 = slot - j * n;
    const int warp = threadIdx.x >> 5, lane = threadIdx.x & 31;
    if (threadIdx.x < 128) {
        const int e = threadIdx.x;
        const int col = col0 + (rows_per > 1 ? e / a.Kpad : 0);
        const int r = rows_per > 1 ? e % a.Kpad : r0 + e;
        long off = -1;
        if (r < a.R && col < a.ncols) {
            const int group = col / a.item_polys, poly = col - group * a.item_polys;
            const long item = a.index ? (long)__ldg(a.index + (long)group * a.R + r) : (long)group * a.R + r;
            off = ((item * a.item_polys + poly) * K + j) * (long)n + c0;
        }
        src_off[e] = off;
    }
    __syncthreads();
#pragma unroll 4
    for (int e = warp; e < 128; e += 8) {
        const long off = src_off[e];
        tile[lane][(e & 3) * 33 + (e >> 2)] = off >= 0 ? __ldg(a.src + off + lane) : 0;
    }
    __syncthreads();
    const long plane_stride = (long)a.ncols * a.Kpad;
    const long row_bytes = plane_stride - (long)col0 * a.Kpad - r0;
    uint8_t *dst = a.dst + ((long)st * 32 * a.planes) * plane_stride + (long)col0 * a.Kpad + r0;
#pragma unroll
    for (int it = 0; it < 4; it++) {
        const int w = threadIdx.x + 256 * it;
        const int c = w >> 5, rw = w & 31;
        if (rows_per > 1 ? 4 * rw >= row_bytes : r0 + 4 * rw >= a.Kpad) continue;
        const uint64_t x0 = tile[c][rw], x1 = tile[c][33 + rw], x2 = tile[c][66 + rw], x3 = tile[c][99 + rw];
        uint8_t *d = dst + (long)c * a.planes * plane_stride + 4 * rw;
#pragma unroll
        for (int l = 0; l < 7; l++) {
            const uint32_t a0 = l < 4 ? (uint32_t)x0 : (uint32_t)(x0 >> 32), a1 = l < 4 ? (uint32_t)x1 : (uint32_t)(x1 >> 32);
            const uint32_t a2 = l < 4 ? (uint32_t)x2 : (uint32_t)(x2 >> 32), a3 = l < 4 ? (uint32_t)x3 : (uint32_t)(x3 >> 32);
            const uint32_t sel = (uint32_t)(l & 3) | ((uint32_t)(4 + (l & 3)) << 4);
            const uint32_t w01 = __byte_perm(a0, a1, sel), w23 = __byte_perm(a2, a3, sel);
            *reinterpret_cast<uint32_t *>(d + (long)l * plane_stride) = __byte_perm(w01, w23, 0x5410);
        }
    }
}

template <int BK, bool FOLD>
cudaError_t launch_tcn_mac_t(const DeviceParams *P, const TcnMacArgs &a, int sm_count, cudaStream_t stream) {
    EncodeTiledFn enc = encode_tiled();
    if (!enc) return cudaErrorNotSupported;
    const CUtensorMapSwizzle sw = BK == 128 ? CU_TENSOR_MAP_SWIZZLE_128B : CU_TENSOR_MAP_SWIZZLE_32B;
    CUtensorMap tmW, tmX;
    {
        const cuuint64_t rowsW = (cuuint64_t)a.Mall * a.Kpad;
        cuuint64_t dims[4] = {(cuuint64_t)a.Kpad, (cuuint64_t)a.M, (cuuint64_t)TCN_PLANES, (cuuint64_t)a.K * a.n};
        cuuint64_t strides[3] = {(cuuint64_t)a.Kpad, rowsW, rowsW * TCN_PLANES};
        cuuint32_t box[4] = {BK, TCN_BM, TCN_PLANES, 1}, es[4] = {1, 1, 1, 1};
        if (enc(&tmW, CU_TENSOR_MAP_DATA_TYPE_UINT8, 4, (void *)(a.W + (size_t)a.m_first * a.Kpad), dims, strides, box, es,
                CU_TENSOR_MAP_INTERLEAVE_NONE, sw, CU_TENSOR_MAP_L2_PROMOTION_L2_256B, CU_TENSOR_MAP_FLOAT_OOB_FILL_NONE) != CUDA_SUCCESS)
            return cudaErrorInvalidValue;
    }
    {
        const cuuint64_t rowsX = (cuuint64_t)a.ncols * a.Kpad;
        cuuint64_t dims[4] = {(cuuint64_t)a.Kpad, (cuuint64_t)a.ncols, (cuuint64_t)TCN_PLANES, (cuuint64_t)a.nslots};
        cuuint64_t strides[3] = {(cuuint64_t)a.Kpad, rowsX, rowsX * TCN_PLANES};
        cuuint32_t box[4] = {BK, TCN_NB, TCN_PLANES, 1}, es[4] = {1, 1, 1, 1};
        if (enc(&tmX, CU_TENSOR_MAP_DATA_TYPE_UINT8, 4, (void *)a.X, dims, strides, box, es, CU_TENSOR_MAP_INTERLEAVE_NONE, sw,
                CU_TENSOR_MAP_L2_PROMOTION_L2_256B, CU_TENSOR_MAP_FLOAT_OOB_FILL_NONE) != CUDA_SUCCESS)
            return cudaErrorInvalidValue;
    }
    auto k = tcn_mac_kernel<BK, FOLD>;
    const size_t smem = TcnCfg<BK>::SMEM;
    static DeviceOnce once;
    if (once.first()) {
        cudaError_t e = cudaFuncSetAttribute(k, cudaFuncAttributeMaxDynamicSharedMemorySize, (int)smem);
        if (e != cudaSuccess) return e;
    }
    const long items = (long)a.nslots * ((a.M + TCN_BM - 1) / TCN_BM);
    const unsigned grid = (unsigned)(items < sm_count ? items : sm_count);
    k<<<grid, TCN_THREADS, smem, stream>>>(tmW, tmX, P, a);
    return cudaGetLastError();
}

template <int BK, bool FOLD, int BIAS, int NS = 1, bool STAGED = false>
cudaError_t launch_tcn2_mac_t(const DeviceParams *P, const TcnMacArgs &a, int sm_count, cudaStream_t stream) {
    EncodeTiledFn enc = encode_tiled();
    if (!enc) return cudaErrorNotSupported;
    const CUtensorMapSwizzle sw = BK == 128 ? CU_TENSOR_MAP_SWIZZLE_128B : CU_TENSOR_MAP_SWIZZLE_32B;
    CUtensorMap tmW, tmX;
    {
        const cuuint64_t rowsW = (cuuint64_t)a.Mall * a.Kpad;
        cuuint64_t dims[4] = {(cuuint64_t)a.Kpad, (cuuint64_t)a.M, (cuuint64_t)TCN_PLANES, (cuuint64_t)a.K * a.n};
        cuuint64_t strides[3] = {(cuuint64_t)a.Kpad, rowsW, rowsW * TCN_PLANES};
        cuuint32_t box[4] = {BK, TCN2_MT, TCN_PLANES, 1}, es[4] = {1, 1, 1, 1};
        if (enc(&tmW, CU_TENSOR_MAP_DATA_TYPE_UINT8, 4, (void *)(a.W + (size_t)a.m_first * a.Kpad), dims, strides, box, es,
                CU_TENSOR_MAP_INTERLEAVE_NONE, sw, CU_TENSOR_MAP_L2_PROMOTION_L2_256B, CU_TENSOR_MAP_FLOAT_OOB_FILL_NONE) != CUDA_SUCCESS)
            return cudaErrorInvalidValue;
    }
    {
        const cuuint64_t rowsX = (cuuint64_t)a.ncols * a.Kpad;
        cuuint64_t dims[4] = {(cuuint64_t)a.Kpad, (cuuint64_t)a.ncols, (cuuint64_t)TCN_PLANES, (cuuint64_t)a.nslots};
        cuuint64_t strides[3] = {(cuuint64_t)a.Kpad, rowsX, rowsX * TCN_PLANES};
        cuuint32_t box[4] = {BK, TCN2_CB, 1, 1}, es[4] = {1, 1, 1, 1};
        if (enc(&tmX, CU_TENSOR_MAP_DATA_TYPE_UINT8, 4, (void *)a.X, dims, strides, box, es, CU_TENSOR_MAP_INTERLEAVE_NONE, sw,
                CU_TENSOR_MAP_L2_PROMOTION_L2_256B, CU_TENSOR_MAP_FLOAT_OOB_FILL_NONE) != CUDA_SUCCESS)
            return cudaErrorInvalidValue;
    }
    auto k = tcn2_mac_kernel<BK, FOLD, BIAS, NS, STAGED>;
    const size_t smem = Tcn2Cfg<BK>::smem(NS, STAGED);
    static DeviceOnce once;
    if (once.first()) {
        cudaError_t e = cudaFuncSetAttribute(k, cudaFuncAttributeMaxDynamicSharedMemorySize, (int)smem);
        if (e != cudaSuccess) return e;
    }
    const long groups = a.nslots / NS;
    const unsigned grid = (unsigned)(groups < sm_count ? groups : sm_count);
    k<<<grid, TCN2_THREADS, smem, stream>>>(tmW, tmX, P, a);
    return cudaGetLastError();
}

}

size_t tcn_x_bytes_per_slot(int planes, int ncols, int Kpad) { return (size_t)planes * ncols * Kpad; }
size_t tcn_w_bytes(int planes, int Mall, int Kpad, int K, int n) { return (size_t)K * n * planes * Mall * Kpad; }

cudaError_t launch_tcn_split(const TcnSplitArgs &a, cudaStream_t stream) {
    if (a.ncols <= 0 || a.nslots <= 0) return cudaSuccess;
    if (a.nslots % 32 || a.slot0 % 32 || a.Kpad % 32 || a.planes != TCN_PLANES || a.nslots / 32 > 65535) return cudaErrorInvalidValue;
    const int rows_per = a.Kpad < 128 ? 128 / a.Kpad : 1;
    dim3 grid((unsigned)((a.ncols + rows_per - 1) / rows_per), (unsigned)(a.nslots / 32), (unsigned)((a.Kpad + 127) / 128));
    tcn_split_kernel<<<grid, 256, 0, stream>>>(a);
    return cudaGetLastError();
}

cudaError_t launch_tcn_mac(const DeviceParams *P, const TcnMacArgs &a, int sm_count, cudaStream_t stream) {
    if (a.nslots <= 0 || a.M <= 0 || a.ncols <= 0) return cudaSuccess;
    if (a.planes != TCN_PLANES || a.R > TCN_MAX_R || a.Kpad != tcn_kpad(a.R)) return cudaErrorInvalidValue;
    const int forced = a.variant;
    const int bk = tcn_bk(a.R);
    const bool fits2 = ((a.R + 31) / 32 * 32 + bk - 1) / bk <= TCN2_KBMAX;
    const bool use2 = fits2 && (forced == 2 || (forced != 1 && a.ncols >= 4 * a.M));
    bool fold = a.use_fold != 0;
    for (int j = 0; j < a.K && fold; j++) fold = a.fold[j].ok != 0;
    static const int bias_env = [] { const char *e = getenv("CRCNN_TCN2_BIAS"); return e ? atoi(e) : -1; }();
    static const int ns_env = [] { const char *e = getenv("CRCNN_TCN2_NS"); return e ? atoi(e) : 4; }();
    static const int stage_env = [] { const char *e = getenv("CRCNN_TCN2_STAGE"); return e ? atoi(e) : 1; }();
    if (use2 && ns_env == 4 && bk == 32 && a.nslots % 4 == 0 && a.slot0 % 4 == 0 && a.n % 4 == 0) {
        if (stage_env && (reinterpret_cast<uintptr_t>(a.out) & 31) == 0)
            return fold ? launch_tcn2_mac_t<32, true, 1, 4, true>(P, a, sm_count, stream) : launch_tcn2_mac_t<32, false, 1, 4, true>(P, a, sm_count, stream);
        return fold ? launch_tcn2_mac_t<32, true, 1, 4>(P, a, sm_count, stream) : launch_tcn2_mac_t<32, false, 1, 4>(P, a, sm_count, stream);
    }
    if (use2) {
        const int bias_var = bias_env >= 0 ? bias_env : (bk == 128 ? 1 : 0);
#ifdef CRCNN_TCN2_TIMING
        if (bias_var == 2) return bk == 128 ? launch_tcn2_mac_t<128, false, 2>(P, a, sm_count, stream) : launch_tcn2_mac_t<32, false, 2>(P, a, sm_count, stream);
#endif
        if (fold) {
            if (bias_var) return bk == 128 ? launch_tcn2_mac_t<128, true, 1>(P, a, sm_count, stream) : launch_tcn2_mac_t<32, true, 1>(P, a, sm_count, stream);
            return bk == 128 ? launch_tcn2_mac_t<128, true, 0>(P, a, sm_count, stream) : launch_tcn2_mac_t<32, true, 0>(P, a, sm_count, stream);
        }
        if (bias_var) return bk == 128 ? launch_tcn2_mac_t<128, false, 1>(P, a, sm_count, stream) : launch_tcn2_mac_t<32, false, 1>(P, a, sm_count, stream);
        return bk == 128 ? launch_tcn2_mac_t<128, false, 0>(P, a, sm_count, stream) : launch_tcn2_mac_t<32, false, 0>(P, a, sm_count, stream);
    }
    if (fold) return bk == 128 ? launch_tcn_mac_t<128, true>(P, a, sm_count, stream) : launch_tcn_mac_t<32, true>(P, a, sm_count, stream);
    return bk == 128 ? launch_tcn_mac_t<128, false>(P, a, sm_count, stream) : launch_tcn_mac_t<32, false>(P, a, sm_count, stream);
}

}

#ifdef CRCNN_TCN2_TRACE
extern "C" int crcnn_debug_tcn2_trace_reset() {
    int z[3] = {0, 0, 0};
    return (int)cudaMemcpyToSymbol(crcnn::g_tcn2_trace_n, z, sizeof(z));
}
extern "C" int crcnn_debug_tcn2_trace_read(int role, unsigned long long *out, int cap) {
    int n[3];
    if (cudaMemcpyFromSymbol(n, crcnn::g_tcn2_trace_n, sizeof(n)) != cudaSuccess) return -1;
    const int cnt = n[role] < cap ? n[role] : cap;
    if (cudaMemcpyFromSymbol(out, crcnn::g_tcn2_trace, (size_t)cnt * 8, (size_t)role * crcnn::TCN2_TRACE_N * 8) != cudaSuccess) return -1;
    return cnt;
}
#endif
```

crcnn_b200/csrc/tcn_mac.cuh:

```cuda
#pragma once
#include <cuda_runtime.h>
#include <cstdint>
#include "params.h"

namespace crcnn {

constexpr int TCN_BM = 64;
constexpr int TCN_NB = 32;
constexpr int TCN_MAX_R = 4096;

inline int tcn_planes_for(const DeviceParams &d) {
    int maxbits = 0;
    for (int j = 0; j < d.K; j++) {
        int b = 0;
        for (uint64_t v = d.tab[j].mod.q; v; v >>= 1) b++;
        maxbits = b > maxbits ? b : maxbits;
    }
    return maxbits <= 56 ? 7 : 8;
}

inline int tcn_kpad(int R) { return R <= 32 ? 32 : ((R + 31) / 32 * 32 < 128 ? 128 : (R + 31) / 32 * 32); }
inline int tcn_bk(int R) { return R <= 32 ? 32 : 128; }

struct TcnSplitArgs {
    const uint64_t *src;
    const int *index;
    uint8_t *dst;
    int item_polys;
    int R, Kpad, planes, ncols;
    int slot0, nslots;
    int n, K;
};

struct TcnMacArgs {
    const uint8_t *W;
    const uint8_t *X;
    const uint64_t *bias;
    uint64_t *out;
    int Mall, m_first, M;
    int R, Kpad, planes, ncols;
    int slot0, nslots;
    int Pimg, Mtotal, m0;
    int n, K;
    int use_fold;
    TcnFold fold[MAXK];
    int variant;
};

size_t tcn_x_bytes_per_slot(int planes, int ncols, int Kpad);
size_t tcn_w_bytes(int planes, int Mall, int Kpad, int K, int n);
cudaError_t launch_tcn_split(const TcnSplitArgs &a, cudaStream_t stream);
cudaError_t launch_tcn_mac(const DeviceParams *P, const TcnMacArgs &a, int sm_count, cudaStream_t stream);

}
```

Baseline: 39.14.

## Add pre-shifted weight planes so tensor-core MAC accumulates seven classes

Adds an optional preshift mode that stores seven copies of the byte-split weights, each first multiplied by 2^(8b) mod q. The MAC kernel can then collect the 49 byte-plane products into 7 accumulator classes instead of 13 diagonals, which shrinks the epilogue recombination and allows a new 7-term fold reduction. A new TMA-based kernel with a 5D weight tensor map implements this. In exchange, weight storage and weight traffic grow sevenfold, with a one-time preshift cost. It also removes an eager weight-split call in the BN fold path and caps the staged epilogue by M.

```diff
diff --git a/crcnn_b200/csrc/engine.cu b/crcnn_b200/csrc/engine.cu
--- a/crcnn_b200/csrc/engine.cu
+++ b/crcnn_b200/csrc/engine.cu
@@ -60,6 +60,7 @@
     int tc_R = 0, tc_Kpad = 0;
     uint8_t *tcn_W = nullptr;
     int tcn_R = 0;
+    bool tcn_pre = false;
     uint64_t *fused_C = nullptr, *fused_Csh = nullptr, *fused_D = nullptr;
     long fused_scale = 0, fused_mean = 0;
     int add_mult = 1;
@@ -100,6 +101,7 @@
     int relin_mode = 1;
     int tcn_mode = 1;
     int sq_lean = 1;
+    int tcn_preshift = 1;
     int tcn_fold = 1;
     size_t tc_scratch_bytes = 12ull << 30;
     std::string err;
@@ -418,35 +420,53 @@
     return rc;
 }
 
-int ensure_tcn_weights(crcnn_ctx *ctx, crcnn_plain *w, int R) {
+int ensure_tcn_weights(crcnn_ctx *ctx, crcnn_plain *w, int R, bool preshift) {
     if (w->tcn_W && w->tcn_R == R) return CRCNN_OK;
     int rc = ensure_form(ctx, w, PF_NTT_MUL);
     if (rc) return rc;
     if (w->tcn_W) { dev_free(ctx, w->tcn_W); w->tcn_W = nullptr; }
     const int Mall = (int)(w->count / R), Kpad = tcn_kpad(R);
-    rc = dev_alloc(ctx, tcn_w_bytes(7, Mall, Kpad, ctx->K, ctx->n), (void **)&w->tcn_W);
-    if (rc) return rc;
+    const size_t block = tcn_w_bytes(7, Mall, Kpad, ctx->K, ctx->n);
+    const int blocks = preshift ? 7 : 1;
+    rc = dev_alloc(ctx, block * blocks, (void **)&w->tcn_W);
+    if (rc) return rc;
+    const long words = (long)w->count * (long)poly_words(ctx);
+    uint64_t *shifted = nullptr;
+    if (preshift) {
+        rc = dev_alloc(ctx, (size_t)words * 8, (void **)&shifted);
+        if (rc) { dev_free(ctx, w->tcn_W); w->tcn_W = nullptr; return rc; }
+    }
+    uint64_t q[MAXK];
+    for (int j = 0; j < ctx->K; j++) q[j] = ctx->hp.d.tab[j].mod.q;
     TcnSplitArgs s{};
-    s.src = w->ntt_mul; s.index = nullptr; s.dst = w->tcn_W; s.item_polys = 1;
+    s.index = nullptr; s.item_polys = 1;
     s.R = R; s.Kpad = Kpad; s.planes = 7; s.ncols = Mall; s.slot0 = 0; s.nslots = ctx->K * ctx->n; s.n = ctx->n; s.K = ctx->K;
-    {
-        ProfScope ps(ctx, KC_TCN_SPLIT, lp_bytes(ctx, (double)w->count * ctx->K) + (double)tcn_w_bytes(7, Mall, Kpad, ctx->K, ctx->n), 0);
+    for (int b = 0; b < blocks; b++) {
+        if (b) CU(launch_tcn_preshift(q, w->ntt_mul, shifted, words, b, ctx->n, ctx->K, ctx->stream));
+        s.src = b ? shifted : w->ntt_mul;
+        s.dst = w->tcn_W + block * b;
+        ProfScope ps(ctx, KC_TCN_SPLIT, lp_bytes(ctx, (double)w->count * ctx->K) + (double)block, 0);
         CU(launch_tcn_split(s, ctx->stream));
     }
+    if (shifted) dev_free(ctx, shifted);
     dev_free(ctx, w->ntt_mul); w->ntt_mul = nullptr;
     if (w->ntt_mul_sh) { dev_free(ctx, w->ntt_mul_sh); w->ntt_mul_sh = nullptr; }
     w->tcn_R = R;
+    w->tcn_pre = preshift;
     return CRCNN_OK;
 }
 
 int run_weighted_sum_tcn(crcnn_ctx *ctx, crcnn_tensor *in, crcnn_plain *w, crcnn_plain *b, const int *d_index, int R,
                          int Npos, int Pimg, int m_first, int M, crcnn_tensor *out) {
+    const int Kpad = tcn_kpad(R), ncols = 2 * Npos, total = ctx->K * ctx->n;
+    const int variant = ctx->tcn_mode >= 2 ? ctx->tcn_mode - 1 : 0;
+    const bool want_pre = ctx->tcn_preshift && tcn_preshift_shape(R, ncols, M, variant) &&
+                          7 * tcn_w_bytes(7, (int)(w->count / R), Kpad, ctx->K, ctx->n) <= ctx->weight_cache_bytes;
     int rc = ensure_domain(ctx, in, 1);
     if (!rc) rc = ensure_form(ctx, b, PF_NTT_ADD);
-    if (!rc) rc = ensure_tcn_weights(ctx, w, R);
+    if (!rc) rc = ensure_tcn_weights(ctx, w, R, want_pre);
     if (rc) return rc;
     const size_t pw = poly_words(ctx);
-    const int Kpad = tcn_kpad(R), ncols = 2 * Npos, total = ctx->K * ctx->n;
     const size_t per_slot = tcn_x_bytes_per_slot(7, ncols, Kpad);
     long chunk = (long)(ctx->tc_scratch_bytes / per_slot) / 32 * 32;
     chunk = std::max<long>(32, std::min<long>(chunk, total));
@@ -461,7 +481,8 @@
     a.Mall = (int)(w->count / R); a.m_first = m_first; a.M = M;
     a.R = R; a.Kpad = Kpad; a.planes = 7; a.ncols = ncols;
     a.Pimg = Pimg; a.Mtotal = M; a.m0 = 0; a.n = ctx->n; a.K = ctx->K;
-    a.variant = ctx->tcn_mode >= 2 ? ctx->tcn_mode - 1 : 0;
+    a.variant = variant;
+    a.preshift = want_pre && w->tcn_pre;
     a.use_fold = ctx->tcn_fold;
     for (int j = 0; j < ctx->K; j++) a.fold[j] = tcn_fold_make(ctx->hp.d.tab[j].mod.q);
     for (long s0 = 0; s0 < total && !rc; s0 += chunk) {
@@ -471,7 +492,7 @@
         cudaError_t e;
         { ProfScope ps(ctx, KC_TCN_SPLIT, (double)ncols * R * ns * 8.0 + xbytes, 0); e = launch_tcn_split(s, ctx->stream); }
         if (e == cudaSuccess) {
-            ProfScope ps(ctx, KC_TCN_MAC, xbytes + (double)ns * 7 * M * Kpad + (double)ncols * M * ns * 8.0, (double)ns * ncols * M * R * 49.0);
+            ProfScope ps(ctx, KC_TCN_MAC, xbytes + (double)ns * 7 * M * Kpad * (a.preshift ? 7 : 1) + (double)ncols * M * ns * 8.0, (double)ns * ncols * M * R * 49.0);
             e = launch_tcn_mac(ctx->dP, a, ctx->sm_count, ctx->stream);
         }
         if (e != cudaSuccess) rc = fail(ctx, CRCNN_ERR_CUDA, std::string("limb-split tensor-core weighted sum: ") + cudaGetErrorString(e));
@@ -579,6 +600,7 @@
     if (const char *e = getenv("CRCNN_TCN")) c->tcn_mode = atoi(e);
     if (const char *e = getenv("CRCNN_TAP")) c->tap_mode = atoi(e);
     if (const char *e = getenv("CRCNN_TCN_FOLD")) c->tcn_fold = atoi(e);
+    if (const char *e = getenv("CRCNN_TCN2_PRESHIFT")) c->tcn_preshift = atoi(e);
     if (const char *e = getenv("CRCNN_SQ_LEAN")) c->sq_lean = atoi(e);
     cudaMemPool_t pool;
     if (cudaDeviceGetDefaultMemPool(&pool, device) == cudaSuccess) {
@@ -1149,7 +1171,7 @@
     if (rc) return done(rc);
     CU(cudaMemcpy2DAsync(B->ntt_add, pw * 8, O->d, 2 * pw * 8, pw * 8, out_dim, cudaMemcpyDeviceToDevice, ctx->stream));
     if (C) CU(launch_fold_fc_input_affine(ctx->dP, W->ntt_mul, out_dim, in_dim, (long)pw, per_channel, C, D, B->ntt_add, ctx->stream));
-    rc = ensure_tcn_weights(ctx, W, in_dim);
+    rc = ensure_tcn_weights(ctx, W, in_dim, false);
     if (rc) return done(rc);
     w1->folded_w = W; w1->folded_b = B;
     return done(CRCNN_OK);
@@ -1390,8 +1412,6 @@
         rc = ensure_form(ctx, w->folded_w, PF_NTT_MUL);
         if (rc) return rc;
         CU(launch_fold_affine(ctx->dP, w->folded_w->ntt_mul, (long)nf * R, (long)pw, R, invstd->fused_C, nullptr, ctx->stream));
-        rc = ensure_tcn_weights(ctx, w->folded_w, R);
-        if (rc) return rc;
         rc = make_plain(ctx, std::vector<uint32_t>(b->off), std::vector<uint32_t>(b->idx), std::vector<uint64_t>(b->val), &w->folded_b);
         if (rc) return rc;
         w->folded_b->add_mult = Rp;
diff --git a/crcnn_b200/csrc/host_selftest.cpp b/crcnn_b200/csrc/host_selftest.cpp
--- a/crcnn_b200/csrc/host_selftest.cpp
+++ b/crcnn_b200/csrc/host_selftest.cpp
@@ -63,6 +63,47 @@
                 const uint64_t want = (uint64_t)((z + bias) % m.q);
                 if (tcn_fold_reduce(s, bias, f, m.q) != want) { printf("FOLD MISMATCH\n"); return 1; }
             }
+        }
+        for (int j = 0; j < d.K; j++) {
+            const Mod &m = d.tab[j].mod;
+            const TcnFold f = tcn_fold_make(m.q);
+            long checked = 0;
+            for (int it = 0; it < 20000; it++) {
+                x = x * 6364136223846793005ULL + 1442695040888963407ULL;
+                y = y * 2862933555777941757ULL + 3037000493ULL;
+                const uint64_t W = it < 2 ? m.q - 1 : x % m.q, X = it < 2 ? m.q - 1 : y % m.q;
+                uint32_t C[7] = {0, 0, 0, 0, 0, 0, 0};
+                for (int b = 0; b < 7; b++) {
+                    const uint64_t wb = (uint64_t)(((unsigned __int128)1 << (8 * b)) % m.q);
+                    const uint64_t wbp = (uint64_t)(((unsigned __int128)wb << 64) / m.q);
+                    uint64_t Wb = mulshoup_lazy(W, wb, wbp, m.q);
+                    Wb = Wb >= m.q ? Wb - m.q : Wb;
+                    if (Wb != (uint64_t)(((unsigned __int128)W << (8 * b)) % m.q)) { printf("PRESHIFT MISMATCH\n"); return 1; }
+                    uint64_t back = 0;
+                    for (int a = 6; a >= 0; a--) back = (back << 8) | ((Wb >> (8 * a)) & 0xff);
+                    if (back != Wb) { printf("PLANE MISMATCH\n"); return 1; }
+                    for (int a = 0; a < 7; a++) C[a] += (uint32_t)(((X >> (8 * b)) & 0xff) * ((Wb >> (8 * a)) & 0xff));
+                }
+                const uint64_t bias = (it & 1) ? y % m.q : 0;
+                const uint64_t want = (uint64_t)(((unsigned __int128)W * X + bias) % m.q);
+                const U128 z = tcn7_combine(C);
+                if (addmod(barrett128(z, m), bias, m.q) != want) { printf("SEVEN-CLASS MISMATCH\n"); return 1; }
+                if (f.ok7 && tcn7_fold_reduce(C, bias, f, m.q) != want) { printf("FOLD7 MISMATCH\n"); return 1; }
+                checked++;
+            }
+            const uint32_t cmax = 7u * 4096u * 255u * 255u;
+            for (int it = 0; it < 2000 && f.ok7; it++) {
+                uint32_t C[7];
+                x = x * 6364136223846793005ULL + 1442695040888963407ULL;
+                for (int a = 0; a < 7; a++) C[a] = it == 0 ? cmax : cmax - (uint32_t)((x >> (4 * a)) % 4096);
+                const uint64_t bias = it == 0 ? m.q - 1 : x % m.q;
+                unsigned __int128 z = 0;
+                for (int a = 6; a >= 0; a--) z = (z << 8) + C[a];
+                if (z >> 80) { printf("FOLD7 BOUND\n"); return 1; }
+                if (tcn7_fold_reduce(C, bias, f, m.q) != (uint64_t)((z + bias) % m.q)) { printf("FOLD7 MISMATCH\n"); return 1; }
+                checked++;
+            }
+            printf("fold7 %d ok7 %u checked %ld\n", j, f.ok7, checked);
         }
         for (int sidx = 0; sidx < d.K + d.S; sidx++) {
             const Mod &m = d.tab[sidx].mod;
diff --git a/crcnn_b200/csrc/modarith.cuh b/crcnn_b200/csrc/modarith.cuh
--- a/crcnn_b200/csrc/modarith.cuh
+++ b/crcnn_b200/csrc/modarith.cuh
@@ -184,7 +184,19 @@
     uint32_t sh, mask;
     uint32_t c8, c16, c24;
     uint32_t ok;
-};
+    uint32_t ok7;
+};
+
+inline bool tcn7_fold_bound(uint64_t q, int k, uint64_t delta) {
+    typedef unsigned __int128 u128;
+    const u128 one = 1, cmax = 0x7fffffffu;
+    u128 z = 0;
+    for (int a = 6; a >= 0; a--) z = (z << 8) + cmax;
+    const u128 h = z >> k;
+    const u128 v = h * delta + ((one << k) - 1) + (q - 1);
+    if (h >> 32 || v >> 64) return false;
+    return (v >> k) * delta + ((one << k) - 1) < 2 * (u128)q;
+}
 
 inline TcnFold tcn_fold_make(uint64_t q) {
     typedef unsigned __int128 u128;
@@ -211,6 +223,7 @@
     if (g * delta + ((one << k) - 1) >= 2 * (u128)q) return f;
     f.T = (uint32_t)T; f.delta = (uint32_t)delta; f.sh = (uint32_t)(k - 32); f.mask = (1u << (k - 32)) - 1;
     f.c8 = 1u << 8; f.c16 = 1u << 16; f.c24 = 1u << 24; f.ok = 1;
+    f.ok7 = tcn7_fold_bound(q, k, delta) ? 1 : 0;
     return f;
 }
 
@@ -248,6 +261,28 @@
     return r >= q ? r - q : r;
 }
 
+CRCNN_HD uint64_t tcn7_fold_reduce(const uint32_t (&C)[7], uint64_t bias, const TcnFold &f, uint64_t q) {
+    const uint64_t La = (uint64_t)C[3] * f.c24 + ((uint64_t)C[2] * f.c16 + ((uint64_t)C[1] * f.c8 + C[0]));
+    const uint64_t Lb = (uint64_t)C[6] * f.c16 + ((uint64_t)C[5] * f.c8 + C[4]);
+    const uint64_t m1 = (La >> 32) + (uint32_t)Lb;
+    const uint32_t y0 = (uint32_t)La, y1 = (uint32_t)m1, y2 = (uint32_t)(Lb >> 32) + (uint32_t)(m1 >> 32);
+    const uint32_t h = tcn_shr64(y1, y2, f.sh);
+    const uint64_t v = (uint64_t)h * f.delta + ((((uint64_t)(y1 & f.mask)) << 32) | y0) + bias;
+    const uint32_t vh = (uint32_t)(v >> 32);
+    const uint64_t r = (uint64_t)(vh >> f.sh) * f.delta + ((((uint64_t)(vh & f.mask)) << 32) | (uint32_t)v);
+    return r >= q ? r - q : r;
+}
+
+CRCNN_HD U128 tcn7_combine(const uint32_t (&C)[7]) {
+    const uint64_t La = ((uint64_t)C[3] << 24) + (((uint64_t)C[2] << 16) + (((uint64_t)C[1] << 8) + C[0]));
+    const uint64_t Lb = ((uint64_t)C[6] << 16) + (((uint64_t)C[5] << 8) + C[4]);
+    const uint64_t m1 = (La >> 32) + (uint32_t)Lb;
+    U128 z;
+    z.lo = (m1 << 32) | (uint32_t)La;
+    z.hi = (Lb >> 32) + (m1 >> 32);
+    return z;
+}
+
 struct Fold128 {
     uint64_t q;
     uint32_t delta, sh, mask, ok;
diff --git a/crcnn_b200/csrc/tc_ptx.cuh b/crcnn_b200/csrc/tc_ptx.cuh
--- a/crcnn_b200/csrc/tc_ptx.cuh
+++ b/crcnn_b200/csrc/tc_ptx.cuh
@@ -51,6 +51,12 @@
     asm volatile(
         "cp.async.bulk.tensor.4d.shared::cluster.global.tile.mbarrier::complete_tx::bytes [%0], [%1, {%3, %4, %5, %6}], [%2];" ::"r"(dst),
         "l"(map), "r"(bar), "r"(c0), "r"(c1), "r"(c2), "r"(c3)
+        : "memory");
+}
+__device__ __forceinline__ void tma_load_5d(uint32_t dst, const CUtensorMap *map, uint32_t bar, int c0, int c1, int c2, int c3, int c4) {
+    asm volatile(
+        "cp.async.bulk.tensor.5d.shared::cluster.global.tile.mbarrier::complete_tx::bytes [%0], [%1, {%3, %4, %5, %6, %7}], [%2];" ::"r"(dst),
+        "l"(map), "r"(bar), "r"(c0), "r"(c1), "r"(c2), "r"(c3), "r"(c4)
         : "memory");
 }
 __device__ __forceinline__ void prefetch_tmap(const CUtensorMap *map) {
diff --git a/crcnn_b200/csrc/tcn_mac.cu b/crcnn_b200/csrc/tcn_mac.cu
--- a/crcnn_b200/csrc/tcn_mac.cu
+++ b/crcnn_b200/csrc/tcn_mac.cu
@@ -1,5 +1,6 @@
 #include <cuda.h>
 #include <cuda_runtime.h>
+#include <algorithm>
 #include <cstdio>
 #include <cstdlib>
 #include "devcfg.cuh"
@@ -440,6 +441,201 @@
     if (warp == 0) tmem_dealloc(tmem_base, TCN_TMEM_COLS);
 }
 
+constexpr int TCN2P_NS = 4;
+constexpr int TCN2P_WB = TCN_PLANES * TCN2_MT * 32;
+constexpr int TCN2P_WSLOT = TCN_PLANES * TCN2P_WB;
+constexpr int TCN2P_X = TCN2_CB * 32;
+constexpr int TCN2P_STAGES = 7;
+constexpr int TCN2P_ACC = TCN_PLANES * TCN2_MT;
+template <bool STAGED> __host__ __device__ constexpr int tcn2p_gpw() { return STAGED ? 2 : (TCN2_MT / 4 + TCN2_EPI_WARPS / 4 - 1) / (TCN2_EPI_WARPS / 4); }
+constexpr int TCN2P_STAGED_MAX_M = 4 * 2 * (TCN2_EPI_WARPS / 4);
+constexpr size_t TCN2P_SMEM = 1024 + (size_t)TCN2P_NS * TCN2P_WSLOT + (size_t)TCN2P_STAGES * TCN2P_X + 8 * (2 * TCN2P_STAGES + 6) + 16;
+
+template <bool FOLD, bool STAGED>
+__global__ void __launch_bounds__(TCN2_THREADS, 1)
+tcn2p_mac_kernel(const __grid_constant__ CUtensorMap tmW, const __grid_constant__ CUtensorMap tmX,
+                 const DeviceParams *__restrict__ P, TcnMacArgs a) {
+    constexpr int NS = TCN2P_NS, STAGES = TCN2P_STAGES, GPW = tcn2p_gpw<STAGED>();
+    constexpr uint32_t ID = (2u << 4) | ((uint32_t)(TCN2_CB >> 4) << 24) | ((uint32_t)(TCN2P_ACC >> 3) << 17);
+
+    extern __shared__ uint8_t smem_raw[];
+    const uint32_t base = (smem_u32(smem_raw) + 1023u) & ~1023u;
+    uint8_t *base_ptr = smem_raw + (base - smem_u32(smem_raw));
+    const uint32_t sW = base, sX = base + NS * TCN2P_WSLOT;
+    const uint32_t off_bar = NS * TCN2P_WSLOT + STAGES * TCN2P_X;
+    const uint32_t bar_full = base + off_bar, bar_empty = bar_full + 8 * STAGES;
+    const uint32_t bar_wfull = bar_empty + 8 * STAGES, bar_wempty = bar_wfull + 8;
+    const uint32_t bar_tfull = bar_wempty + 8, bar_tempty = bar_tfull + 16;
+    const uint32_t tmem_slot = bar_tempty + 16;
+    volatile uint32_t *tmem_slot_ptr = reinterpret_cast<volatile uint32_t *>(base_ptr + off_bar + 8 * (2 * STAGES + 6));
+
+    const int warp = threadIdx.x >> 5, lane = threadIdx.x & 31;
+    const int n = a.n;
+    const int m_tiles = (a.M + TCN2_MT - 1) / TCN2_MT;
+    const long groups = a.nslots / NS;
+    const long items = (groups > blockIdx.x ? (groups - blockIdx.x + gridDim.x - 1) / gridDim.x : 0) * m_tiles;
+    auto item_group = [&](long it) { return (long)blockIdx.x + (it / m_tiles) * gridDim.x; };
+    const int chunks = (a.ncols + TCN2_CB - 1) / TCN2_CB;
+
+    if (threadIdx.x == 0) {
+        for (int s = 0; s < STAGES; s++) { mbar_init(bar_full + 8 * s, 1); mbar_init(bar_empty + 8 * s, 1); }
+        mbar_init(bar_wfull, 1);
+        mbar_init(bar_wempty, 1);
+        for (int b = 0; b < 2; b++) { mbar_init(bar_tfull + 8 * b, 1); mbar_init(bar_tempty + 8 * b, TCN2_EPI_WARPS); }
+        fence_barrier_init();
+        prefetch_tmap(&tmW);
+        prefetch_tmap(&tmX);
+    }
+    if (warp == 0) tmem_alloc(tmem_slot, TCN_TMEM_COLS);
+    tc_fence_before();
+    __syncthreads();
+    tc_fence_after();
+    const uint32_t tmem_base = *tmem_slot_ptr;
+
+    if (warp == 0) {
+        if (lane == 0) {
+            int stage = 0;
+            uint32_t phase = 0, wphase = 0;
+            for (long item = 0; item < items; item++) {
+                const int sl = (int)item_group(item) * NS, mt = (int)(item % m_tiles);
+                mbar_wait(bar_wempty, wphase ^ 1);
+                mbar_expect_tx(bar_wfull, NS * TCN2P_WSLOT);
+                for (int s = 0; s < NS; s++) tma_load_5d(sW + s * TCN2P_WSLOT, &tmW, bar_wfull, 0, mt * TCN2_MT, 0, a.slot0 + sl + s, 0);
+                wphase ^= 1;
+                for (int ch = 0; ch < chunks; ch++)
+                    for (int s = 0; s < NS; s++)
+                        for (int b = 0; b < TCN_PLANES; b++) {
+                            mbar_wait(bar_empty + 8 * stage, phase ^ 1);
+                            TCN2_TR(0, b);
+                            mbar_expect_tx(bar_full + 8 * stage, TCN2P_X);
+                            tma_load_4d(sX + stage * TCN2P_X, &tmX, bar_full + 8 * stage, 0, ch * TCN2_CB, b, sl + s);
+                            if (++stage == STAGES) { stage = 0; phase ^= 1; }
+                        }
+            }
+        }
+        __syncwarp();
+    } else if (warp == 1) {
+        if (lane == 0) {
+            int stage = 0;
+            uint32_t phase = 0, wphase = 0, use = 0;
+            for (long item = 0; item < items; item++) {
+                mbar_wait(bar_wfull, wphase);
+                wphase ^= 1;
+                tc_fence_after();
+                for (int chs = 0; chs < chunks * NS; chs++, use++) {
+                    const int s = chs % NS;
+                    const uint32_t buf = use & 1;
+                    TCN2_TR(1, 100);
+                    mbar_wait(bar_tempty + 8 * buf, ((use >> 1) & 1) ^ 1);
+                    TCN2_TR(1, 101);
+                    tc_fence_after();
+                    const uint32_t acc = tmem_base + buf * TCN2P_ACC;
+                    for (int b = 0; b < TCN_PLANES; b++) {
+                        mbar_wait(bar_full + 8 * stage, phase);
+                        TCN2_TR(1, b);
+                        tc_fence_after();
+                        umma_i8(acc, umma_desc_sw32(sX + stage * TCN2P_X), umma_desc_sw32(sW + s * TCN2P_WSLOT + b * TCN2P_WB), ID, b ? 1u : 0u);
+                        umma_commit(bar_empty + 8 * stage);
+                        if (++stage == STAGES) { stage = 0; phase ^= 1; }
+                    }
+                    umma_commit(bar_tfull + 8 * buf);
+                    TCN2_TR(1, 102);
+                }
+                umma_commit(bar_wempty);
+            }
+        }
+        __syncwarp();
+    } else {
+        const int qd = warp & 3, sub = (warp - 2) >> 2;
+        const long pw = (long)a.K * n;
+        const long m_stride = 2L * a.Pimg * pw;
+        uint32_t use = 0;
+        for (long item = 0; item < items; item++) {
+            const int sl = (int)item_group(item) * NS, mt = (int)(item % m_tiles);
+            const int slot = a.slot0 + sl, j = slot / n, c = slot - j * n;
+            const Mod mod = P->tab[j].mod;
+            const TcnFold fold = a.fold[FOLD ? j : 0];
+            const long slot_off = (long)j * n + c;
+            const int m_valid = min(TCN2_MT, a.M - mt * TCN2_MT);
+            const int groups = (m_valid + 3) >> 2;
+            uint64_t bias_lane[NS];
+#pragma unroll
+            for (int s = 0; s < NS; s++)
+                bias_lane[s] = (a.bias && lane < m_valid) ? __ldg(a.bias + (long)(mt * TCN2_MT + lane) * pw + slot_off + s) : 0;
+            for (int ch = 0; ch < chunks; ch++) {
+                const int col = ch * TCN2_CB + qd * 32 + lane;
+                const bool valid = col < a.ncols;
+                const int p = col >> 1, poly = col & 1;
+                const long colbase = (long)(p / a.Pimg) * ((long)a.Mtotal * a.Pimg) + p % a.Pimg;
+                uint64_t *out_col = a.out + (colbase * 2 + poly) * pw + slot_off + (long)(a.m0 + mt * TCN2_MT) * m_stride;
+                const bool add_bias = poly == 0 && a.bias != nullptr;
+                uint64_t keep[GPW][4][NS - 1];
+#pragma unroll
+                for (int s = 0; s < NS; s++, use++) {
+                    const uint32_t buf = use & 1;
+                    if (warp == 2 && lane == 0) TCN2_TR(2, 200);
+                    mbar_wait(bar_tfull + 8 * buf, (use >> 1) & 1);
+                    if (warp == 2 && lane == 0) TCN2_TR(2, 201);
+                    tc_fence_after();
+#pragma unroll
+                    for (int gi = 0; gi < GPW; gi++) {
+                        const int g = sub + gi * (TCN2_EPI_WARPS / 4);
+                        if (g >= groups) break;
+                        const int mloc = g * 4;
+                        uint32_t C[TCN_PLANES][4];
+#pragma unroll
+                        for (int w = 0; w < TCN_PLANES; w++)
+                            tmem_ld4(tmem_base + ((uint32_t)(qd * 32) << 16) + buf * TCN2P_ACC + w * TCN2_MT + mloc, C[w]);
+                        tmem_ld_wait();
+                        uint64_t *op = out_col + (long)mloc * m_stride + s;
+#pragma unroll
+                        for (int i = 0; i < 4; i++) {
+                            if (mloc + i < m_valid) {
+                                const uint64_t bias_m = __shfl_sync(0xffffffffu, bias_lane[s], mloc + i);
+                                uint32_t Ci[TCN_PLANES];
+#pragma unroll
+                                for (int w = 0; w < TCN_PLANES; w++) Ci[w] = C[w][i];
+                                uint64_t r;
+                                if constexpr (FOLD) {
+                                    r = tcn7_fold_reduce(Ci, add_bias ? bias_m : 0, fold, mod.q);
+                                } else {
+                                    r = barrett128(tcn7_combine(Ci), mod);
+                                    if (add_bias) r = addmod(r, bias_m, mod.q);
+                                }
+                                if constexpr (STAGED) {
+                                    if (s < NS - 1) keep[gi][i][s < NS - 1 ? s : 0] = r;
+                                    else if (valid) tcn_store_sector(op - (NS - 1), keep[gi][i][0], keep[gi][i][1], keep[gi][i][2], r);
+                                } else if (valid) {
+                                    *op = r;
+                                }
+                            }
+                            op += m_stride;
+                        }
+                    }
+                    tc_fence_before();
+                    __syncwarp();
+                    if (lane == 0) mbar_arrive(bar_tempty + 8 * buf);
+                    if (warp == 2 && lane == 0) TCN2_TR(2, 202);
+                }
+            }
+        }
+    }
+    tc_fence_before();
+    __syncthreads();
+    if (warp == 0) tmem_dealloc(tmem_base, TCN_TMEM_COLS);
+}
+
+struct TcnShift { uint64_t q[MAXK], w[MAXK], wp[MAXK]; };
+__global__ void tcn_preshift_kernel(const uint64_t *__restrict__ src, uint64_t *__restrict__ dst, long words, int n, int K, TcnShift c) {
+    const long pw = (long)K * n;
+    for (long i = (long)blockIdx.x * blockDim.x + threadIdx.x; i < words; i += (long)gridDim.x * blockDim.x) {
+        const int j = (int)((i % pw) / n);
+        const uint64_t q = c.q[j];
+        const uint64_t r = mulshoup_lazy(__ldg(src + i), c.w[j], c.wp[j], q);
+        dst[i] = r >= q ? r - q : r;
+    }
+}
+
 __global__ void __launch_bounds__(256)
 tcn_split_kernel(TcnSplitArgs a) {
     __shared__ uint64_t tile[32][133];
@@ -566,6 +762,59 @@
     return cudaGetLastError();
 }
 
+template <bool FOLD, bool STAGED>
+cudaError_t launch_tcn2p_mac_t(const DeviceParams *P, const TcnMacArgs &a, int sm_count, cudaStream_t stream) {
+    EncodeTiledFn enc = encode_tiled();
+    if (!enc) return cudaErrorNotSupported;
+    CUtensorMap tmW, tmX;
+    {
+        const cuuint64_t rowsW = (cuuint64_t)a.Mall * a.Kpad, slotW = rowsW * TCN_PLANES;
+        cuuint64_t dims[5] = {(cuuint64_t)a.Kpad, (cuuint64_t)a.M, (cuuint64_t)TCN_PLANES, (cuuint64_t)a.K * a.n, (cuuint64_t)TCN_PLANES};
+        cuuint64_t strides[4] = {(cuuint64_t)a.Kpad, rowsW, slotW, slotW * a.K * a.n};
+        cuuint32_t box[5] = {32, TCN2_MT, TCN_PLANES, 1, TCN_PLANES}, es[5] = {1, 1, 1, 1, 1};
+        if (enc(&tmW, CU_TENSOR_MAP_DATA_TYPE_UINT8, 5, (void *)(a.W + (size_t)a.m_first * a.Kpad), dims, strides, box, es,
+                CU_TENSOR_MAP_INTERLEAVE_NONE, CU_TENSOR_MAP_SWIZZLE_32B, CU_TENSOR_MAP_L2_PROMOTION_L2_256B, CU_TENSOR_MAP_FLOAT_OOB_FILL_NONE) != CUDA_SUCCESS)
+            return cudaErrorInvalidValue;
+    }
+    {
+        const cuuint64_t rowsX = (cuuint64_t)a.ncols * a.Kpad;
+        cuuint64_t dims[4] = {(cuuint64_t)a.Kpad, (cuuint64_t)a.ncols, (cuuint64_t)TCN_PLANES, (cuuint64_t)a.nslots};
+        cuuint64_t strides[3] = {(cuuint64_t)a.Kpad, rowsX, rowsX * TCN_PLANES};
+        cuuint32_t box[4] = {32, TCN2_CB, 1, 1}, es[4] = {1, 1, 1, 1};
+        if (enc(&tmX, CU_TENSOR_MAP_DATA_TYPE_UINT8, 4, (void *)a.X, dims, strides, box, es, CU_TENSOR_MAP_INTERLEAVE_NONE, CU_TENSOR_MAP_SWIZZLE_32B,
+                CU_TENSOR_MAP_L2_PROMOTION_L2_256B, CU_TENSOR_MAP_FLOAT_OOB_FILL_NONE) != CUDA_SUCCESS)
+            return cudaErrorInvalidValue;
+    }
+    auto k = tcn2p_mac_kernel<FOLD, STAGED>;
+    static DeviceOnce once;
+    if (once.first()) {
+        cudaError_t e = cudaFuncSetAttribute(k, cudaFuncAttributeMaxDynamicSharedMemorySize, (int)TCN2P_SMEM);
+        if (e != cudaSuccess) return e;
+    }
+    const long groups = a.nslots / TCN2P_NS;
+    const unsigned grid = (unsigned)(groups < sm_count ? groups : sm_count);
+    k<<<grid, TCN2_THREADS, TCN2P_SMEM, stream>>>(tmW, tmX, P, a);
+    return cudaGetLastError();
+}
+
+}
+
+bool tcn_preshift_shape(int R, int ncols, int M, int variant) {
+    return R >= 1 && R <= 32 && variant != 1 && (variant == 2 || ncols >= 4 * M);
+}
+
+cudaError_t launch_tcn_preshift(const uint64_t *q, const uint64_t *src, uint64_t *dst, long words, int b, int n, int K, cudaStream_t stream) {
+    if (words <= 0) return cudaSuccess;
+    if (b < 1 || b >= TCN_PLANES || K > MAXK) return cudaErrorInvalidValue;
+    TcnShift c{};
+    for (int j = 0; j < K; j++) {
+        c.q[j] = q[j];
+        c.w[j] = (uint64_t)(((unsigned __int128)1 << (8 * b)) % q[j]);
+        c.wp[j] = (uint64_t)(((unsigned __int128)c.w[j] << 64) / q[j]);
+    }
+    const long blocks = std::min<long>((words + 255) / 256, 148L * 16);
+    tcn_preshift_kernel<<<(unsigned)blocks, 256, 0, stream>>>(src, dst, words, n, K, c);
+    return cudaGetLastError();
 }
 
 size_t tcn_x_bytes_per_slot(int planes, int ncols, int Kpad) { return (size_t)planes * ncols * Kpad; }
@@ -592,8 +841,16 @@
     static const int bias_env = [] { const char *e = getenv("CRCNN_TCN2_BIAS"); return e ? atoi(e) : -1; }();
     static const int ns_env = [] { const char *e = getenv("CRCNN_TCN2_NS"); return e ? atoi(e) : 4; }();
     static const int stage_env = [] { const char *e = getenv("CRCNN_TCN2_STAGE"); return e ? atoi(e) : 1; }();
+    if (a.preshift) {
+        if (!tcn_preshift_shape(a.R, a.ncols, a.M, forced) || a.nslots % TCN2P_NS || a.slot0 % TCN2P_NS || a.n % TCN2P_NS) return cudaErrorInvalidValue;
+        bool fold7 = a.use_fold != 0;
+        for (int j = 0; j < a.K && fold7; j++) fold7 = a.fold[j].ok7 != 0;
+        if (stage_env && a.M <= TCN2P_STAGED_MAX_M && (reinterpret_cast<uintptr_t>(a.out) & 31) == 0)
+            return fold7 ? launch_tcn2p_mac_t<true, true>(P, a, sm_count, stream) : launch_tcn2p_mac_t<false, true>(P, a, sm_count, stream);
+        return fold7 ? launch_tcn2p_mac_t<true, false>(P, a, sm_count, stream) : launch_tcn2p_mac_t<false, false>(P, a, sm_count, stream);
+    }
     if (use2 && ns_env == 4 && bk == 32 && a.nslots % 4 == 0 && a.slot0 % 4 == 0 && a.n % 4 == 0) {
-        if (stage_env && (reinterpret_cast<uintptr_t>(a.out) & 31) == 0)
+        if (stage_env && a.M <= TCN2P_STAGED_MAX_M && (reinterpret_cast<uintptr_t>(a.out) & 31) == 0)
             return fold ? launch_tcn2_mac_t<32, true, 1, 4, true>(P, a, sm_count, stream) : launch_tcn2_mac_t<32, false, 1, 4, true>(P, a, sm_count, stream);
         return fold ? launch_tcn2_mac_t<32, true, 1, 4>(P, a, sm_count, stream) : launch_tcn2_mac_t<32, false, 1, 4>(P, a, sm_count, stream);
     }
diff --git a/crcnn_b200/csrc/tcn_mac.cuh b/crcnn_b200/csrc/tcn_mac.cuh
--- a/crcnn_b200/csrc/tcn_mac.cuh
+++ b/crcnn_b200/csrc/tcn_mac.cuh
@@ -45,11 +45,14 @@
     int use_fold;
     TcnFold fold[MAXK];
     int variant;
+    int preshift;
 };
 
 size_t tcn_x_bytes_per_slot(int planes, int ncols, int Kpad);
 size_t tcn_w_bytes(int planes, int Mall, int Kpad, int K, int n);
 cudaError_t launch_tcn_split(const TcnSplitArgs &a, cudaStream_t stream);
+bool tcn_preshift_shape(int R, int ncols, int M, int variant);
+cudaError_t launch_tcn_preshift(const uint64_t *q, const uint64_t *src, uint64_t *dst, long words, int b, int n, int K, cudaStream_t stream);
 cudaError_t launch_tcn_mac(const DeviceParams *P, const TcnMacArgs &a, int sm_count, cudaStream_t stream);
 
 }
```

Measured after the change: 40.48 (median of 6 runs). 1.03x the previous value.
